# Rita-zi/WavTokenizer

Measured on AMD Instinct MI355X. Metric: audio-seconds/sec encode+decode, 24 kHz 3 s clips, higher is better.
Workload: dtype f32 (split-f16 x3 products)

## Files before the change

### include/wavtokenizer_amd.h

```cpp
#ifndef WAVTOKENIZER_AMD_H
#define WAVTOKENIZER_AMD_H

#include <stddef.h>
#include <stdint.h>

#ifdef __cplusplus
extern "C" {
#endif

typedef enum {
    WT_OK = 0,
    WT_ERR_INVALID = -1,
    WT_ERR_MISSING_TENSOR = -2,
    WT_ERR_SHAPE = -3,
    WT_ERR_HIP = -4,
    WT_ERR_NOT_INITED = -5,
    WT_ERR_RANGE = -6,
    WT_ERR_LSTM_SYNC = -7,
    WT_ERR_INDEX = -8
} wt_status;

enum wt_status_bits {
    WT_STATUS_BIT_LSTM = 1,
    WT_STATUS_BIT_RANGE = 2
};

typedef struct {
    int32_t n_ratios;
    int32_t ratios[8];
    int32_t vq_bins;
    int32_t num_quantizers;
    int32_t input_channels;
    int32_t dim;
    int32_t intermediate_dim;
    int32_t num_layers;
    int32_t adanorm_num_embeddings;
    int32_t n_fft;
    int32_t hop_length;
    int32_t padding_same;
} wt_arch;

typedef struct {
    const char*  name;
    const float* data;
    int64_t      numel;
} wt_tensor;

typedef struct wt_model wt_model;
typedef struct wt_plan  wt_plan;

typedef enum {
    WT_PLAN_ENCODE = 0,
    WT_PLAN_DECODE = 1,
    WT_PLAN_SEANET_DECODER = 2,
    WT_PLAN_HEAD = 3,
    WT_PLAN_UNIT_LSTM = 4
} wt_plan_kind;

enum {
    WT_PLAN_FLAG_KEEP_STAGES = 1,
    WT_PLAN_FLAG_UNFUSED = 16,
    WT_PLAN_FLAG_STEP_LSTM = 4,
    WT_PLAN_FLAG_GRAPH = 8,
    WT_PLAN_FLAG_FP32_GEMM = 2,
    WT_PLAN_FLAG_RANGE_REPORT = 32,
    WT_PLAN_FLAG_MIXED_LENGTH = 64
};

enum wt_range_site {
    WT_SITE_ENCODER = 0,
    WT_SITE_BB_EMBED = 1,
    WT_SITE_RES0 = 2, WT_SITE_RES1 = 3,
    WT_SITE_ATTN = 4,
    WT_SITE_RES2 = 5, WT_SITE_RES3 = 6,
    WT_SITE_CNX0 = 7,
    WT_SITE_HEAD = 40,
    WT_SITE_SEANET_DECODER = 41
};

const char* wt_last_error(void);
const char* wt_version(void);

int  wt_model_create(const wt_arch* arch, const wt_tensor* tensors, int32_t n_tensors, int32_t device,
                     wt_model** out);
void wt_model_destroy(wt_model* m);

size_t wt_model_export_bytes(const wt_model* m);
int  wt_model_export(const wt_model* m, void* buf, size_t n);
int  wt_packed_info(const void* buf, size_t n, wt_arch* arch, int32_t* version, uint64_t* arch_hash);
int  wt_packed_verify(const void* buf, size_t n);
size_t wt_packed_bytes(const void* buf, size_t n);
int  wt_model_create_packed(const void* buf, size_t n, int32_t device, wt_model** out);
int  wt_model_hop(const wt_model* m);
int  wt_model_persistent_lstm(const wt_model* m);
int  wt_device_info(int32_t device, int32_t* compute_units, int32_t* is_gfx950, int32_t* persistent_lstm);
int64_t wt_model_weight_bytes(const wt_model* m);

int    wt_plan_create(const wt_model* m, int32_t kind, int32_t B, int64_t len, int32_t flags, wt_plan** out);
int    wt_plan_create_ex(const wt_model* m, int32_t kind, int32_t B, int64_t len, int32_t flags, uint64_t fp32_sites,
                         wt_plan** out);
void   wt_plan_destroy(wt_plan* p);
size_t wt_plan_workspace_bytes(const wt_plan* p);
int64_t wt_plan_frames(const wt_plan* p);
int    wt_plan_num_launches(const wt_plan* p);
int64_t wt_plan_graph_replays(const wt_plan* p);
int    wt_plan_find_buffer(const wt_plan* p, const char* name, size_t* offset, size_t* numel);
int    wt_plan_buffer_info(const wt_plan* p, const char* name, size_t* offset, size_t* numel, int32_t* format);
int    wt_plan_status(const wt_plan* p, int32_t* bits, int32_t clear);
int    wt_plan_range_sites(const wt_plan* p, uint64_t* sites, int32_t clear);
int    wt_plan_range_report(const wt_plan* p, int32_t index, const char** step, const char** buffer, float* amax);
int    wt_model_status(const wt_model* m, int32_t* bits, int32_t clear);
int    wt_model_split_ok(const wt_model* m);
int    wt_plan_buffer_name(const wt_plan* p, int32_t index, const char** name);

int wt_plan_num_steps(const wt_plan* p);
int wt_plan_step_name(const wt_plan* p, int32_t index, const char** name);
int wt_plan_set_timing(const wt_plan* p, const char* name_substr);
int wt_plan_read_timing(const wt_plan* p, double* total_ms, int64_t* launches, int32_t reset);

int wt_encode(const wt_plan* p, const float* wav, float* features, int64_t* codes, float* emb_out,
              void* workspace, void* stream);

int wt_encode_mixed(const wt_plan* p, const float* wav, const int32_t* lengths, float* features, int64_t* codes, float* emb_out,
                    void* workspace, void* stream);
int64_t wt_plan_min_clip_length(const wt_plan* p);
int wt_sconv_geometry(int64_t T, int32_t k, int32_t stride, int32_t dilation, int32_t out[4]);

int wt_codes_to_features(const wt_model* m, const int64_t* codes, int32_t K, int32_t B, int64_t L,
                         float* features, void* stream);

int wt_decode(const wt_plan* p, const float* features, int32_t bandwidth_id, float* wav_out,
              float* backbone_out, void* workspace, void* stream);

int wt_head(const wt_plan* p, const float* x, float* wav_out, void* workspace, void* stream);

int wt_seanet_decode(const wt_plan* p, const float* features, float* wav_out, void* workspace, void* stream);


int wt_sconv1d(const float* x, const float* w, const float* bias, float* y, int32_t B, int64_t T,
               int32_t Cin, int32_t Cout, int32_t k, int32_t stride, int32_t dilation, int32_t elu_input,
               void* stream);

int wt_linear(const float* x, const float* w, const float* bias, float* y, int64_t M, int32_t N, int32_t K,
              int32_t f16x3, void* workspace, void* stream);

int wt_conv1d_s32(const float* x, const float* w, const float* bias, float* y, int32_t B, int64_t T, int32_t Cin,
                  int32_t Cout, int32_t k, int32_t stride, int32_t zero_same, void* workspace, void* stream);

size_t wt_vq_workspace_bytes(int64_t N, int32_t D, int32_t bins);
int wt_vq_nearest(const float* x, const float* embed, int64_t N, int32_t D, int32_t bins, int64_t* codes_out,
                  void* workspace, void* stream);
int wt_vq_nearest_f32(const float* x, const float* embed, int64_t N, int32_t D, int32_t bins, int64_t* codes_out,
                      void* workspace, void* stream);

typedef struct {
    int32_t size;
    int32_t engine, epi, out, pro, b_is_act;
    int32_t M, N, K;
    int32_t T_in, T_out, Cin, taps, stride, dil, pad_left, pad_mode, Tp;
    int32_t K1, nz, tap_pair, head_kb;
    float alpha;
    int64_t a_bstride, a_rstride, a2_bstride, a2_rstride, w_rstride, c_rstride, r_rstride, zA, zW, zC;
    const float* A;
    const float* A2;
    const float* B;
    const float* bias;
    const float* R;
    const float* gamma;
    float* C;
    float* C2;
    uint32_t* status;
} wt_gemm_desc;
typedef struct {
    int32_t BM, BN, waves_m, waves_n, stages, ks, prod, staged, bias_cache, G, tiles;
} wt_launch_form;
size_t wt_gemm_probe_workspace_bytes(const wt_gemm_desc* d);
int wt_gemm_probe(const wt_gemm_desc* d, wt_launch_form* form, void* workspace, void* stream);

enum { WT_OP_GN_APPLY = 0, WT_OP_GN_STATS = 1, WT_OP_ROWNORM = 2, WT_OP_SOFTMAX = 3, WT_OP_ISTFT_OLA = 4, WT_OP_CONV_FIRST = 5,
       WT_OP_CONV_LAST = 6, WT_OP_TRANSPOSE = 7, WT_OP_CONVTR = 8, WT_OP_ROW_SUMSQ = 9, WT_OP_S32_AMAX = 10 };
enum { WT_OPK_GN_TILE = 1, WT_OPK_GN_CHUNK = 2, WT_OPK_GN_STATS = 3, WT_OPK_ROWNORM = 4, WT_OPK_DWCONV_LN = 5,
       WT_OPK_SOFTMAX_REG = 6, WT_OPK_SOFTMAX_RMW = 7, WT_OPK_ISTFT_OLA = 8, WT_OPK_CONV_FIRST = 9, WT_OPK_CONV_LAST32 = 10,
       WT_OPK_CONV_LAST = 11, WT_OPK_TRANSPOSE = 12, WT_OPK_CONVTR = 13, WT_OPK_ROW_SUMSQ = 14, WT_OPK_S32_AMAX = 15 };
typedef struct {
    int32_t size;
    int32_t op;
    int32_t B, L, C;
    int32_t groups, mode, flag, out_s32;
    int32_t ld, k, stride, Cout, n_fft, hop, Kq;
    float eps;
    int64_t n;
    const void* x;
    const void *p0, *p1, *p2, *p3, *p4, *p5;
    void *y, *y2, *y3;
    uint32_t* status;
} wt_op_desc;
typedef struct {
    int32_t kernel;
    int32_t variant;
    int32_t variant2;
    int32_t grid_x, grid_y, grid_z, block, lds;
} wt_op_form;
int wt_op_probe(const wt_op_desc* d, wt_op_form* form, void* stream);

int wt_resblock(const float* x, const float* wav, const float* e0_w, const float* e0_b, const float* w3, const float* b3,
                const float* w1, const float* b1, const float* ws, const float* bs, float* y, int32_t B, int64_t T,
                int32_t C, int32_t elu_out, int32_t out_s32, int32_t fp32_chain, void* stream);
int wt_resblock_down(const float* wav, const float* e0_w, const float* e0_b, const float* w3, const float* b3, const float* w1,
                     const float* b1, const float* ws, const float* bs, const float* wd, const float* bd, float* y_down,
                     int32_t B, int64_t T, int32_t r, void* stream);

int wt_unit_run(const wt_plan* p, const float* x, float* y, void* workspace, void* stream);

int wt_model_take_bad_codes(const wt_model* m);


typedef struct wt_resampler wt_resampler;
int     wt_resampler_create(int32_t orig_sr, int32_t new_sr, int32_t device, wt_resampler** out);
void    wt_resampler_destroy(wt_resampler* r);
int64_t wt_resampler_out_length(const wt_resampler* r, int64_t T);
int     wt_convert_audio(const wt_resampler* r, const float* wav, int32_t B, int32_t C, int64_t T, float* out, void* stream);

int wt_pcm16(const float* x, int64_t n, float limit, int32_t rescale, int16_t* out, void* workspace, void* stream);

int wt_linear_overlap_add(const float* frames, const float* weight, int32_t n_frames, int64_t rows, int64_t frame_len,
                          int64_t last_len, int64_t stride, float* out, void* stream);

#ifdef __cplusplus
}
#endif
#endif
```

### wavtokenizer_amd/_capi.py

```python
from __future__ import annotations

import ctypes
import os
from ctypes import POINTER, c_char_p, c_float, c_int32, c_int64, c_size_t, c_void_p

_HERE = os.path.dirname(os.path.abspath(__file__))
LIB_PATH = os.environ.get("WAVTOK_HIP_LIB") or os.path.join(_HERE, "libwavtok_hip.so")

EXPORTS = [
    "wt_last_error", "wt_version", "wt_model_create", "wt_model_destroy", "wt_model_export_bytes", "wt_model_export", "wt_packed_info", "wt_packed_verify", "wt_packed_bytes",
    "wt_model_create_packed", "wt_model_hop", "wt_model_weight_bytes",
    "wt_plan_create", "wt_plan_create_ex", "wt_plan_range_sites", "wt_plan_range_report", "wt_model_persistent_lstm", "wt_device_info", "wt_plan_destroy", "wt_plan_workspace_bytes", "wt_plan_frames", "wt_plan_num_launches", "wt_plan_graph_replays",
    "wt_plan_find_buffer", "wt_plan_buffer_info", "wt_plan_buffer_name", "wt_plan_status", "wt_plan_num_steps", "wt_plan_step_name",
    "wt_plan_set_timing", "wt_plan_read_timing", "wt_model_split_ok", "wt_model_status", "wt_model_take_bad_codes", "wt_encode", "wt_codes_to_features",
    "wt_decode", "wt_seanet_decode", "wt_head", "wt_unit_run", "wt_sconv1d", "wt_linear", "wt_conv1d_s32", "wt_vq_workspace_bytes",
    "wt_vq_nearest", "wt_vq_nearest_f32", "wt_resblock", "wt_resblock_down", "wt_gemm_probe_workspace_bytes", "wt_gemm_probe", "wt_op_probe",
    "wt_resampler_create", "wt_resampler_destroy", "wt_resampler_out_length", "wt_convert_audio", "wt_pcm16",
    "wt_linear_overlap_add", "wt_encode_mixed", "wt_plan_min_clip_length", "wt_sconv_geometry",
]

WT_PLAN_ENCODE, WT_PLAN_DECODE, WT_PLAN_SEANET_DECODER, WT_PLAN_HEAD, WT_PLAN_UNIT_LSTM = 0, 1, 2, 3, 4
WT_PLAN_FLAG_KEEP_STAGES = 1
WT_PLAN_FLAG_FP32_GEMM = 2
WT_PLAN_FLAG_STEP_LSTM = 4
WT_PLAN_FLAG_GRAPH = 8
WT_PLAN_FLAG_UNFUSED = 16
WT_PLAN_FLAG_RANGE_REPORT = 32
WT_PLAN_FLAG_MIXED_LENGTH = 64
WT_SITE_ENCODER, WT_SITE_BB_EMBED, WT_SITE_RES0, WT_SITE_RES1, WT_SITE_ATTN, WT_SITE_RES2, WT_SITE_RES3 = 0, 1, 2, 3, 4, 5, 6
WT_SITE_CNX0, WT_SITE_HEAD, WT_SITE_SEANET_DECODER = 7, 40, 41
WT_ERR_INVALID = -1
WT_ERR_RANGE, WT_ERR_LSTM_SYNC, WT_ERR_INDEX = -6, -7, -8
WT_STATUS_BIT_LSTM, WT_STATUS_BIT_RANGE = 1, 2
BUF_S32, BUF_ELU = 1, 2


class WtArch(ctypes.Structure):
    _fields_ = [("n_ratios", c_int32), ("ratios", c_int32 * 8), ("vq_bins", c_int32), ("num_quantizers", c_int32),
                ("input_channels", c_int32), ("dim", c_int32), ("intermediate_dim", c_int32),
                ("num_layers", c_int32), ("adanorm_num_embeddings", c_int32), ("n_fft", c_int32),
                ("hop_length", c_int32), ("padding_same", c_int32)]


class WtTensor(ctypes.Structure):
    _fields_ = [("name", c_char_p), ("data", POINTER(c_float)), ("numel", c_int64)]


class WtGemmDesc(ctypes.Structure):
    _fields_ = ([("size", c_int32), ("engine", c_int32), ("epi", c_int32), ("out", c_int32), ("pro", c_int32), ("b_is_act", c_int32),
                 ("M", c_int32), ("N", c_int32), ("K", c_int32)]
                + [(n, c_int32) for n in ("T_in", "T_out", "Cin", "taps", "stride", "dil", "pad_left", "pad_mode", "Tp",
                                         "K1", "nz", "tap_pair", "head_kb")]
                + [("alpha", c_float)]
                + [(n, c_int64) for n in ("a_bstride", "a_rstride", "a2_bstride", "a2_rstride", "w_rstride", "c_rstride",
                                         "r_rstride", "zA", "zW", "zC")]
                + [(n, c_void_p) for n in ("A", "A2", "B", "bias", "R", "gamma", "C", "C2", "status")])


class WtLaunchForm(ctypes.Structure):
    _fields_ = [(n, c_int32) for n in ("BM", "BN", "waves_m", "waves_n", "stages", "ks", "prod", "staged", "bias_cache", "G", "tiles")]


WT_OP_GN_APPLY, WT_OP_GN_STATS, WT_OP_ROWNORM, WT_OP_SOFTMAX, WT_OP_ISTFT_OLA, WT_OP_CONV_FIRST = 0, 1, 2, 3, 4, 5
WT_OP_CONV_LAST, WT_OP_TRANSPOSE, WT_OP_CONVTR, WT_OP_ROW_SUMSQ, WT_OP_S32_AMAX = 6, 7, 8, 9, 10
WT_OPK_NAMES = {1: "gn_tile", 2: "gn_chunk", 3: "gn_stats", 4: "rownorm", 5: "dwconv_ln", 6: "softmax_reg", 7: "softmax_rmw",
                8: "istft_ola", 9: "conv_first", 10: "conv_last32", 11: "conv_last", 12: "transpose", 13: "convtr",
                14: "row_sumsq", 15: "s32_amax"}


class WtOpDesc(ctypes.Structure):
    _fields_ = ([(n, c_int32) for n in ("size", "op", "B", "L", "C", "groups", "mode", "flag", "out_s32", "ld", "k", "stride",
                                        "Cout", "n_fft", "hop", "Kq")]
                + [("eps", c_float), ("n", c_int64)]
                + [(n, c_void_p) for n in ("x", "p0", "p1", "p2", "p3", "p4", "p5", "y", "y2", "y3", "status")])


class WtOpForm(ctypes.Structure):
    _fields_ = [(n, c_int32) for n in ("kernel", "variant", "variant2", "grid_x", "grid_y", "grid_z", "block", "lds")]


class WavTokError(RuntimeError):
    def __init__(self, msg, status=0):
        super().__init__(msg)
        self.status = status


def _load() -> ctypes.CDLL:
    if not os.path.exists(LIB_PATH):
        raise ImportError(
            f"{LIB_PATH} not found: build the HIP extension first (python -c 'import __graft_entry__ as g; g.build()' "
            "or make -C wavtokenizer_amd/csrc). There is no CPU fallback for the product path.")
    lib = ctypes.CDLL(LIB_PATH)
    if os.environ.get("WAVTOK_HIP_LIB"):
        class _Missing:
            def __init__(self, name):
                self.name, self.argtypes, self.restype = name, None, None

            def __call__(self, *a):
                raise WavTokError(f"{LIB_PATH} has no {self.name}")
        for sym in EXPORTS:
            try:
                getattr(lib, sym)
            except AttributeError:
                setattr(lib, sym, _Missing(sym))
    lib.wt_last_error.restype = c_char_p
    lib.wt_version.restype = c_char_p
    lib.wt_model_create.argtypes = [POINTER(WtArch), POINTER(WtTensor), c_int32, c_int32, POINTER(c_void_p)]
    lib.wt_model_destroy.argtypes = [c_void_p]
    lib.wt_model_destroy.restype = None
    lib.wt_model_export_bytes.argtypes = [c_void_p]
    lib.wt_model_export_bytes.restype = c_size_t
    lib.wt_model_export.argtypes = [c_void_p, c_void_p, c_size_t]
    lib.wt_packed_info.argtypes = [c_void_p, c_size_t, POINTER(WtArch), POINTER(c_int32), POINTER(ctypes.c_uint64)]
    lib.wt_packed_verify.argtypes = [c_void_p, c_size_t]
    lib.wt_packed_bytes.argtypes = [c_void_p, c_size_t]
    lib.wt_packed_bytes.restype = c_size_t
    lib.wt_model_create_packed.argtypes = [c_void_p, c_size_t, c_int32, POINTER(c_void_p)]
    lib.wt_model_hop.argtypes = [c_void_p]
    lib.wt_model_weight_bytes.argtypes = [c_void_p]
    lib.wt_model_weight_bytes.restype = c_int64
    lib.wt_plan_create.argtypes = [c_void_p, c_int32, c_int32, c_int64, c_int32, POINTER(c_void_p)]
    lib.wt_plan_create_ex.argtypes = [c_void_p, c_int32, c_int32, c_int64, c_int32, ctypes.c_uint64, POINTER(c_void_p)]
    lib.wt_plan_range_sites.argtypes = [c_void_p, POINTER(ctypes.c_uint64), c_int32]
    lib.wt_plan_range_report.argtypes = [c_void_p, c_int32, POINTER(c_char_p), POINTER(c_char_p), POINTER(c_float)]
    lib.wt_model_persistent_lstm.argtypes = [c_void_p]
    lib.wt_device_info.argtypes = [c_int32, POINTER(c_int32), POINTER(c_int32), POINTER(c_int32)]
    lib.wt_plan_destroy.argtypes = [c_void_p]
    lib.wt_plan_destroy.restype = None
    lib.wt_plan_workspace_bytes.argtypes = [c_void_p]
    lib.wt_plan_workspace_bytes.restype = c_size_t
    lib.wt_plan_frames.argtypes = [c_void_p]
    lib.wt_plan_frames.restype = c_int64
    lib.wt_plan_num_launches.argtypes = [c_void_p]
    lib.wt_plan_graph_replays.argtypes = [c_void_p]
    lib.wt_plan_graph_replays.restype = c_int64
    lib.wt_plan_find_buffer.argtypes = [c_void_p, c_char_p, POINTER(c_size_t), POINTER(c_size_t)]
    lib.wt_plan_buffer_info.argtypes = [c_void_p, c_char_p, POINTER(c_size_t), POINTER(c_size_t), POINTER(c_int32)]
    lib.wt_plan_status.argtypes = [c_void_p, POINTER(c_int32), c_int32]
    lib.wt_model_split_ok.argtypes = [c_void_p]
    lib.wt_model_status.argtypes = [c_void_p, POINTER(c_int32), c_int32]
    lib.wt_model_take_bad_codes.argtypes = [c_void_p]
    lib.wt_unit_run.argtypes = [c_void_p, c_void_p, c_void_p, c_void_p, c_void_p]
    lib.wt_plan_buffer_name.argtypes = [c_void_p, c_int32, POINTER(c_char_p)]
    lib.wt_plan_num_steps.argtypes = [c_void_p]
    lib.wt_plan_step_name.argtypes = [c_void_p, c_int32, POINTER(c_char_p)]
    lib.wt_plan_set_timing.argtypes = [c_void_p, c_char_p]
    lib.wt_plan_read_timing.argtypes = [c_void_p, POINTER(ctypes.c_double), POINTER(c_int64), c_int32]
    lib.wt_encode.argtypes = [c_void_p, c_void_p, c_void_p, c_void_p, c_void_p, c_void_p, c_void_p]
    lib.wt_encode_mixed.argtypes = [c_void_p, c_void_p, c_void_p, c_void_p, c_void_p, c_void_p, c_void_p, c_void_p]
    lib.wt_plan_min_clip_length.argtypes = [c_void_p]
    lib.wt_plan_min_clip_length.restype = c_int64
    lib.wt_sconv_geometry.argtypes = [c_int64, c_int32, c_int32, c_int32, POINTER(c_int32)]
    lib.wt_codes_to_features.argtypes = [c_void_p, c_void_p, c_int32, c_int32, c_int64, c_void_p, c_void_p]
    lib.wt_decode.argtypes = [c_void_p, c_void_p, c_int32, c_void_p, c_void_p, c_void_p, c_void_p]
    lib.wt_seanet_decode.argtypes = [c_void_p, c_void_p, c_void_p, c_void_p, c_void_p]
    lib.wt_head.argtypes = [c_void_p, c_void_p, c_void_p, c_void_p, c_void_p]
    lib.wt_sconv1d.argtypes = [c_void_p, c_void_p, c_void_p, c_void_p, c_int32, c_int64, c_int32, c_int32, c_int32,
                               c_int32, c_int32, c_int32, c_void_p]
    lib.wt_linear.argtypes = [c_void_p, c_void_p, c_void_p, c_void_p, c_int64, c_int32, c_int32, c_int32, c_void_p, c_void_p]
    lib.wt_conv1d_s32.argtypes = [c_void_p, c_void_p, c_void_p, c_void_p, c_int32, c_int64, c_int32, c_int32, c_int32,
                                  c_int32, c_int32, c_void_p, c_void_p]
    lib.wt_vq_workspace_bytes.argtypes = [c_int64, c_int32, c_int32]
    lib.wt_vq_workspace_bytes.restype = c_size_t
    lib.wt_vq_nearest.argtypes = [c_void_p, c_void_p, c_int64, c_int32, c_int32, c_void_p, c_void_p, c_void_p]
    lib.wt_vq_nearest_f32.argtypes = [c_void_p, c_void_p, c_int64, c_int32, c_int32, c_void_p, c_void_p, c_void_p]
    lib.wt_resblock.argtypes = [c_void_p] * 11 + [c_int32, c_int64, c_int32, c_int32, c_int32, c_int32, c_void_p]
    lib.wt_resblock_down.argtypes = [c_void_p] * 12 + [c_int32, c_int64, c_int32, c_void_p]
    lib.wt_gemm_probe_workspace_bytes.argtypes = [POINTER(WtGemmDesc)]
    lib.wt_gemm_probe_workspace_bytes.restype = c_size_t
    lib.wt_gemm_probe.argtypes = [POINTER(WtGemmDesc), POINTER(WtLaunchForm), c_void_p, c_void_p]
    lib.wt_op_probe.argtypes = [POINTER(WtOpDesc), POINTER(WtOpForm), c_void_p]
    lib.wt_resampler_create.argtypes = [c_int32, c_int32, c_int32, POINTER(c_void_p)]
    lib.wt_resampler_destroy.argtypes = [c_void_p]
    lib.wt_resampler_destroy.restype = None
    lib.wt_resampler_out_length.argtypes = [c_void_p, c_int64]
    lib.wt_resampler_out_length.restype = c_int64
    lib.wt_convert_audio.argtypes = [c_void_p, c_void_p, c_int32, c_int32, c_int64, c_void_p, c_void_p]
    lib.wt_pcm16.argtypes = [c_void_p, c_int64, ctypes.c_float, c_int32, c_void_p, c_void_p, c_void_p]
    lib.wt_linear_overlap_add.argtypes = [c_void_p, c_void_p, c_int32, c_int64, c_int64, c_int64, c_int64, c_void_p, c_void_p]
    return lib


lib = _load()


def check(rc: int, what: str = "") -> None:
    if rc != 0:
        msg = lib.wt_last_error()
        raise WavTokError(f"{what} failed (status {rc}): {msg.decode() if msg else ''}", rc)
```

### wavtokenizer_amd/csrc/common.h

```cpp
#pragma once
#include <hip/hip_runtime.h>
#include <stdint.h>
#include <stdio.h>
#include <stdlib.h>
#include <mutex>
#include <string>

namespace wt {

void set_error(const std::string& msg);

#define WT_HIP_CHECK(expr)                                                                      \
    do {                                                                                        \
        hipError_t _e = (expr);                                                                 \
        if (_e != hipSuccess) {                                                                 \
            ::wt::set_error(std::string(#expr) + ": " + hipGetErrorString(_e));                 \
            return -4;                                                                          \
        }                                                                                       \
    } while (0)

struct PerDeviceOnce {
    std::mutex mu;
    bool seen[64] = {};
    template <class F> int run(F&& f) {
        int d = 0;
        (void)hipGetDevice(&d);
        d &= 63;
        std::lock_guard<std::mutex> g(mu);
        if (seen[d]) return 0;
        if (int rc = f()) return rc;
        seen[d] = true;
        return 0;
    }
};

enum : unsigned { WT_STATUS_LSTM = 1u, WT_STATUS_RANGE = 2u };
enum OpKernel : int {
    OPK_NONE = 0, OPK_GN_TILE, OPK_GN_CHUNK, OPK_GN_STATS, OPK_ROWNORM, OPK_DWCONV_LN, OPK_SOFTMAX_REG, OPK_SOFTMAX_RMW,
    OPK_ISTFT_OLA, OPK_CONV_FIRST, OPK_CONV_LAST32, OPK_CONV_LAST, OPK_TRANSPOSE, OPK_CONVTR, OPK_ROW_SUMSQ, OPK_S32_AMAX
};
struct OpForm {
    int kernel = OPK_NONE;
    int variant = 0;
    int variant2 = 0;
    unsigned grid[3] = {0, 0, 0};
    unsigned block = 0;
    unsigned lds = 0;
};
struct LaunchCtx {
    unsigned* status = nullptr;
    OpForm* form = nullptr;
    unsigned long long* stamp_start = nullptr;
    unsigned long long* stamp_end = nullptr;
    bool stamp_used = false;
};
extern thread_local LaunchCtx g_launch;

int device_cus();

#ifdef WT_LAB
inline const char* lab_env(const char* name) { return getenv(name); }
#else
inline const char* lab_env(const char*) { return nullptr; }
#endif

#if defined(__HIPCC__)
#ifdef WT_NO_RANGE_TRACK
__device__ __forceinline__ float amax1(float m, float) { return m; }
__device__ __forceinline__ float amax4(float m, float, float, float, float) { return m; }
#else
__device__ __forceinline__ float amax1(float m, float v) { return fmaxf(m, fabsf(v)); }
__device__ __forceinline__ float amax4(float m, float a, float b, float c, float d) {
    m = fmaxf(fmaxf(m, fabsf(a)), fabsf(b));
    return fmaxf(fmaxf(m, fabsf(c)), fabsf(d));
}
#endif
__device__ __forceinline__ void split2_f16(float a, float b, unsigned& hi_pk, unsigned& lo_pk) {
    typedef float f32x2_t __attribute__((ext_vector_type(2)));
    typedef _Float16 f16x2_t __attribute__((ext_vector_type(2)));
    const f32x2_t ab = {a, b};
    hi_pk = __builtin_bit_cast(unsigned, __builtin_convertvector(ab, f16x2_t));
    const f32x2_t s = ab * 2048.f;
    const float m = -2048.f;
    asm("v_fma_mixlo_f16 %0, %1, %2, %3 op_sel_hi:[1,0,0]" : "=v"(lo_pk) : "v"(hi_pk), "s"(m), "v"(s[0]));
    asm("v_fma_mixhi_f16 %0, %1, %2, %3 op_sel:[1,0,0] op_sel_hi:[1,0,0]" : "+v"(lo_pk) : "v"(hi_pk), "s"(m), "v"(s[1]));
}
typedef _Float16 wt_f16x4 __attribute__((ext_vector_type(4)));
__device__ __forceinline__ void split4_f16(float a, float b, float c, float d, wt_f16x4& hi, wt_f16x4& lo) {
    typedef unsigned u32x2_t __attribute__((ext_vector_type(2)));
    unsigned h0, l0, h1, l1;
    split2_f16(a, b, h0, l0);
    split2_f16(c, d, h1, l1);
    hi = __builtin_bit_cast(wt_f16x4, (u32x2_t){h0, h1});
    lo = __builtin_bit_cast(wt_f16x4, (u32x2_t){l0, l1});
}
__device__ __forceinline__ float elu_med3(float x) { return __builtin_amdgcn_fmed3f(x, __expf(x) - 1.f, 0.f); }
typedef float wt_f32x4 __attribute__((ext_vector_type(4)));
__device__ __forceinline__ wt_f32x4 elu_med3_x4(wt_f32x4 x) {
    const wt_f32x4 t = x * 1.44269504088896340736f;
    wt_f32x4 e;
#pragma unroll
    for (int i = 0; i < 4; ++i) e[i] = __builtin_amdgcn_exp2f(t[i]);
    e = e - 1.f;
#pragma unroll
    for (int i = 0; i < 4; ++i) e[i] = __builtin_amdgcn_fmed3f(x[i], e[i], 0.f);
    return e;
}
__device__ __forceinline__ void range_report(unsigned* status, float amax) {
    if (status && amax >= 65504.f) __hip_atomic_fetch_or(status, (unsigned)WT_STATUS_RANGE, __ATOMIC_RELAXED, __HIP_MEMORY_SCOPE_AGENT);
}
#endif

struct SConvGeom { int pl, pr_total, Tout, Tp; };
__host__ __device__ inline SConvGeom sconv_geom(long T, int k, int stride, int dil) {
    const int keff = (k - 1) * dil + 1;
    const int pt = keff - stride;
    const long nfr_num = T - keff + pt;
    const long nfr = (nfr_num + stride - 1) / stride + 1;
    const long ideal = (nfr - 1) * stride + (keff - pt);
    const int extra = (int)(ideal - T);
    SConvGeom g;
    const int pr = pt / 2;
    g.pl = pt - pr;
    g.pr_total = pr + extra;
    g.Tout = (int)((T + pt + extra - keff) / stride + 1);
    const int maxpad = g.pl > g.pr_total ? g.pl : g.pr_total;
    g.Tp = T > maxpad ? (int)T : maxpad + 1;
    return g;
}

enum : int {
    GEOM_WORDS = 64, GEOM_VALID = 0, GEOM_T = 1, GEOM_TREAD = 2, GEOM_STAGE0 = 3, GEOM_STAGE_WORDS = 9,
    GEOM_C3 = 0, GEOM_SC = 3, GEOM_DOWN = 6, GEOM_MAX_STAGES = 6
};
inline int geom_final(int n_stages) { return GEOM_STAGE0 + n_stages * GEOM_STAGE_WORDS; }
inline int geom_L(int n_stages) { return geom_final(n_stages) + 3; }

enum Pro : int { PRO_NONE = 0, PRO_ELU = 1 };
enum Epi : int {
    EPI_BIAS = 0,
    EPI_BIAS_RES = 1,
    EPI_BIAS_GELU = 2,
    EPI_BIAS_GAMMA_RES = 3,
    EPI_HEAD = 4,
    EPI_ARGMAX = 6,
    EPI_SCALE = 7,
    EPI_BIAS_ROW = 8,
    EPI_BIAS_RES_ELU = 9,
    EPI_BIAS_ELU = 10
};
enum Out16s : int {
    OUT_F32 = 0,
    OUT_S32 = 1,
    OUT_S32_DUAL_ELU = 2,
    OUT_F32_AND_S32 = 3
};
enum PadMode : int { PAD_ZERO = 0, PAD_REFLECT = 1 };

struct LaunchForm {
    int BM = 0, BN = 0, waves_m = 0, waves_n = 0, stages = 0;
    int ks = 1, prod = 0;
    int staged = 0, bias_cache = 0;
    int G = 0, tiles = 0;
};

struct GemmArgs {
    const float* A = nullptr;
    long a_bstride = 0;
    long a_rstride = 0;
    int T_in = 0, T_out = 0;
    int Cin = 0, taps = 1, stride = 1, dil = 1, pad_left = 0, pad_mode = PAD_ZERO;
    int Tp = 0;
    const float* A2 = nullptr;
    long a2_bstride = 0, a2_rstride = 0;
    int K1 = 0;
    const float* W = nullptr;
    long w_rstride = 0;
    const void* W_hi = nullptr;
    const float* bias = nullptr;
    int M = 0, N = 0, K = 0;
    float* C = nullptr;
    long c_rstride = 0;
    float* C2 = nullptr;
    const float* R = nullptr;
    long r_rstride = 0;
    const float* gamma = nullptr;
    float alpha = 1.f;
    int nz = 1;
    long zA = 0, zW = 0, zC = 0;
    int head_kb = 0;
    const float* vq_xx = nullptr;
    const float* vq_ee = nullptr;
    float* vq_pval = nullptr;
    int*   vq_pidx = nullptr;
    int vq_nparts = 0;
    int group_m = 8;
    int group_n = 0;
    int tap_pair = 0;
    unsigned long long* stamp_start = nullptr;
    unsigned long long* stamp_end = nullptr;
    int stage_epi = 0;
    int stage_off = 0;
    int pc_off = 0;
    float acc_scale = 1.f;
    const float* acc_scale_dev = nullptr;
    unsigned* status = nullptr;
    unsigned long long* dbg_stamps = nullptr;
    LaunchForm* form = nullptr;
};

int gemm_vq_parts(int N);
int check_gemm(const GemmArgs& a, int pro, int epi);
int check_gemm16s(const GemmArgs& a, int epi, int out, const int* mix_geom = nullptr);
int launch_gemm(const GemmArgs& a, int pro, int epi, hipStream_t s);
int launch_gemm16s(const GemmArgs& a, int epi, int out, hipStream_t s, const int* mix_geom = nullptr);
int gemm16s_vq_parts(int N);
int launch_split_s32(const float* x, void* out, long n, hipStream_t s, const float* scale_dev = nullptr);
int launch_unsplit_s32(const void* s32, float* out, long n, float inv_scale, hipStream_t s);
int launch_pow2_scales(const float* a, long na, const float* b, long nb, unsigned* bits2, float* out3, hipStream_t s);

int launch_conv_first(const float* wav, const float* w , const float* bias, float* y, int B, long T,
                      int k, int Cout, hipStream_t s);
int launch_conv_last(const float* x , const float* w , const float* bias, float* y ,
                     int B, long T, int Cin, int k, int elu_in, hipStream_t s);
int launch_transpose(const float* in, float* out, int B, int R, int C, hipStream_t s, int out_s32 = 0);
size_t gn_part_floats(int B, int L, int groups);
int launch_gn_stats(const float* x, const float* gamma, const float* beta, float* scale, float* shift, int B, int L,
                    int C, int groups, float eps, hipStream_t s, float* part = nullptr);
int launch_gn_apply(const float* x, const float* gamma, const float* beta, float* scale, float* shift, float* y,
                    int swish, int B, int L, int C, int groups, float eps, hipStream_t s, int out_s32 = 0, float* part = nullptr);
enum RowNormMode : int { RN_DWCONV = 0, RN_PLAIN = 1, RN_AFFINE_IN = 2 };
int launch_rownorm(int mode, const float* x, float* y, int B, int L, int C, const float* dw_w ,
                   const float* dw_b, const float* in_scale, const float* in_shift, const float* out_scale,
                   const float* out_shift, float eps, hipStream_t s, int out_s32 = 0);
int launch_istft_ola(const float* parts, const float* win, const float* wsq, float* out, int B, int L, int n_fft, int hop,
                     int Kq, int center, hipStream_t s);
int launch_softmax(float* S, int rows, int L, int ld, hipStream_t s, float* P_s32 = nullptr);
int launch_row_sumsq(const float* x, float* out, long rows, int D, hipStream_t s);
int launch_vq_finalize(const float* pval, const int* pidx, int nparts, const float* embed, int64_t* codes,
                       float* feat_ncl, int B, int L, int D, int bins, hipStream_t s);
int launch_codes_to_features(const int64_t* codes, const float* embed, int K, int bins, int B, long L, int D,
                             float* feat_ncl, hipStream_t s, unsigned* bad = nullptr);
int launch_fill_u32(void* p, unsigned value, size_t n_bytes, hipStream_t s);
int launch_plan_guard(const unsigned* status, int nwords, int site0, unsigned* host_status, unsigned* model_status, int64_t* codes,
                      long n_codes, float* f0, long n0, float* f1, long n1, float* f2, long n2, hipStream_t s);
int launch_s32_amax(const void* s32, long numel, unsigned* out_bits, hipStream_t s);
struct LstmArgs {
    const float* xg0;
    const float* W0;
    const float* W1;
    const float* b1;
    float* h0;
    float* h1;
    float* c0;
    float* c1;
    const float* x;
    float* y;
    int B, L, H;
    int elu_out;
    int out_s32;
    int f16x3;
    unsigned* status = nullptr;
};
int launch_lstm_step(const LstmArgs& a, int s, hipStream_t stream);
struct LstmPersistArgs {
    const float* xg0;
    const void* Wp;
    const float* b1;
    const float* x;
    float* y;
    void* hx;
    unsigned* ctl;
    unsigned* status = nullptr;
    int dbg_spin_shift = 0;
    int B, L, H, Bx;
    int elu_out, out_s32;
    int data_flag;
};
size_t lstm_persist_hx_bytes();
size_t lstm_persist_ctl_bytes();
int launch_lstm_persist(const LstmPersistArgs& a, hipStream_t stream);
struct ResblockArgs {
    const float* x;
    const float* wav;
    const float* e0_w;
    const float* e0_b;
    const float* W3;
    const float* b3;
    const float* W1;
    const float* b1;
    const float* Ws;
    const float* bs;
    float* y;
    int B, T, C;
    long x_bstride;
    int elu_out;
    int out_s32;
    int dbg;
    unsigned* status;
    const float* Wd;
    const float* bd;
    float* y_down;
    int R;
};
struct ResblockMix {
    const int* T = nullptr;
    const int* Tread = nullptr;
};
bool resblock_fusable(int C);
int launch_resblock(const ResblockArgs& a, hipStream_t s);
int launch_resblock16(const ResblockArgs& a, hipStream_t s, const ResblockMix* mix = nullptr);
bool resblock16_down_fusable(int C, long T, int r, int k);
int launch_resblock16_down(const ResblockArgs& a, hipStream_t s, const ResblockMix* mix = nullptr);
int launch_mixed_geometry(const int* lengths, int* geom, int B, long Tpad, int tmin, int n_st, const int* kd, const int* rd,
                          int kf, hipStream_t s);
int launch_mixed_pad(const int* geom, int l_word, int64_t* codes, float* feat_ncl, float* emb_ncl, int B, int L, int D,
                     hipStream_t s);
int launch_convtr(const float* x, const float* w , const float* bias, float* y, int B, int Tin,
                  int Cin, int Cout, int k, int stride, int elu_in, hipStream_t s);

}
```

### wavtokenizer_amd/csrc/model.h

```cpp
#pragma once
#include "../../include/wavtokenizer_amd.h"
#include "common.h"

#include <algorithm>
#include <atomic>
#include <climits>
#include <cmath>
#include <cstring>
#include <functional>
#include <map>
#include <memory>
#include <mutex>
#include <string>
#include <vector>

namespace wt {

struct S32Copy {
    const void* p = nullptr;
    float acc_scale = 1.f;
    bool tap_pair = false;
};
struct ConvW {
    float* w = nullptr;
    float* b = nullptr;
    int cout = 0, cin = 0, k = 0;
    S32Copy s32;
};
struct GemmW {
    float* w = nullptr;
    int rows = 0, cols = 0;
    S32Copy s32;
};
struct LstmW {
    GemmW Wih0;
    float* b0 = nullptr;
    float* W0 = nullptr;
    float* W1 = nullptr;
    float* b1 = nullptr;
    float* W0h = nullptr;
    float* W1h = nullptr;
    float* Wp = nullptr;
};
struct ResStage {
    ConvW c3, c1, sc, down;
    ConvW cat;
    int C = 0, r = 0;
};
struct PosRes {
    float *n1w, *n1b, *n2w, *n2b;
    ConvW c1, c2;
};
struct CnxBlock {
    float *dw_w, *dw_b, *ada_s, *ada_h, *b1, *b2, *gamma;
    GemmW W1, W2;
};
struct SeaDecStage {
    float* tr_w = nullptr;
    GemmW tr_wp;
    float* tr_b = nullptr;
    int cin = 0, cout = 0, k = 0, r = 0;
    ConvW c3, c1, sc;
    ConvW cat;
};

}

struct wt_model {
    wt_arch arch{};
    int device = 0;
    int hop = 1;
    int H = 512;
    std::vector<int> enc_ratios;
    std::vector<void*> allocs;
    std::vector<size_t> alloc_bytes;
    int64_t weight_bytes = 0;
    float *e0_w = nullptr, *e0_b = nullptr;
    int e0_k = 7, e0_c = 32;
    std::vector<wt::ResStage> stages;
    wt::LstmW enc_lstm;
    wt::ConvW enc_final;
    wt::GemmW embed;
    float* ee = nullptr;
    wt::ConvW bb_embed;
    wt::PosRes res[4];
    float *at_nw, *at_nb, *at_bqk, *at_bv, *at_bp;
    wt::GemmW at_Wqk, at_Wv, at_Wp;
    float *gn5w, *gn5b, *ada_s, *ada_h;
    std::vector<wt::CnxBlock> cnx;
    float *fln_w, *fln_b;
    wt::GemmW head_W, istft_W;
    float *head_b = nullptr, *wsq = nullptr, *win = nullptr;
    int Kb = 0, Kq = 0, bins_f = 0, R = 0;
    bool has_seadec = false;
    wt::ConvW sd_first;
    wt::LstmW sd_lstm;
    std::vector<wt::SeaDecStage> sd_stages;
    float *sd_last_w = nullptr, *sd_last_b = nullptr;
    bool s32_ok = true;
    bool sd_s32_ok = true;
    float w_amax = 0.f;
    struct LazyF32 { const float* w; const void* s32; int64_t n; float scale; };
    std::vector<LazyF32> lazy_f32;
    mutable std::atomic<bool> f32_stale{false};
    mutable std::mutex f32_mu;
    unsigned* bad_codes_host = nullptr;
    unsigned* bad_codes_dev = nullptr;
    unsigned* status_host = nullptr;
    unsigned* status_dev = nullptr;
    mutable std::atomic<bool> persist_ok{true};
};

namespace wt {

struct TensorMap {
    std::map<std::string, std::pair<const float*, int64_t>> m;
    std::string missing;
    const float* get(const std::string& k, int64_t numel) {
        auto it = m.find(k);
        if (it == m.end()) { if (missing.empty()) missing = k; return nullptr; }
        if (it->second.second != numel) {
            if (missing.empty()) missing = k + " (numel " + std::to_string(it->second.second) + ", expected " + std::to_string(numel) + ")";
            return nullptr;
        }
        return it->second.first;
    }
    bool has(const std::string& k) const { return m.count(k) != 0; }
};

struct RunCtx {
    char* ws;
    hipStream_t stream;
    const float* in_f;
    float* out_f;
    int64_t* codes;
    float* aux;
    int bw_id;
    const int* lengths = nullptr;
};
enum Site : int {
    SITE_ENC = 0,
    SITE_BB_EMBED = 1,
    SITE_RES0 = 2, SITE_RES1 = 3, SITE_ATTN = 4, SITE_RES2 = 5, SITE_RES3 = 6,
    SITE_CNX0 = 7,
    SITE_HEAD = 40,
    SITE_SEADEC = 41,
    SITE_COUNT = 64
};
constexpr int CTL_SITE0 = 16;
constexpr int CTL_WORDS = CTL_SITE0 + SITE_COUNT + 48;

enum BufFmt : int { BUF_F32 = 0, BUF_S32 = 1, BUF_ELU = 2 };
struct BufSpec {
    std::string name;
    size_t bytes = 0, numel = 0, off = 0;
    int first = INT_MAX, last = -1;
    int fmt = BUF_F32;
    bool holds_s32 = false;
};

struct DeviceGuard {
    int prev = -1;
    bool ok = true;
    explicit DeviceGuard(int dev) {
        if (hipGetDevice(&prev) != hipSuccess) prev = -1;
        if (prev != dev) ok = hipSetDevice(dev) == hipSuccess; else prev = -1;
    }
    ~DeviceGuard() { if (prev >= 0) (void)hipSetDevice(prev); }
};

}

struct wt_plan {
    const wt_model* model = nullptr;
    int kind = 0, B = 0, flags = 0;
    int64_t len = 0, L = 0, T = 0;
    uint64_t fp32_sites = 0;
    int whole_site = -1;
    int cur_site = 0;
    long n_codes = 0, n_out = 0, n_aux = 0;
    int build_rc = 0;
    std::vector<wt::BufSpec> bufs;
    std::vector<std::function<int(const wt::RunCtx&)>> steps;
    std::vector<std::string> step_names;
    std::vector<int> step_sites;
    struct RangeEntry { int step, buf; };
    std::vector<RangeEntry> range_entries;
    unsigned* range_dev = nullptr;
    mutable std::vector<float> range_host;
    mutable bool range_fresh = false;
    size_t ws_bytes = 0;
    int n_launches = 0;
    mutable std::string timing_filter;
    mutable std::vector<std::pair<hipEvent_t, hipEvent_t>> ev_pending, ev_free;
    static constexpr int STAMP_SLOTS = 8192;
    mutable unsigned long long* stamps = nullptr;
    mutable int stamp_next = 0;
    mutable double timing_ms = 0.0;
    mutable long timing_n = 0;
    unsigned* status_host = nullptr;
    unsigned* status_dev = nullptr;
    int ctl = -1;
    bool uses_persist = false;
    int mix_geom = -1;
    int64_t min_clip = 0;
    mutable bool graph_persist = false;
    mutable std::mutex mu;
    struct GraphKey {
        const void *ws = nullptr, *in = nullptr, *out = nullptr, *codes = nullptr, *aux = nullptr, *lengths = nullptr;
        int bw = -1;
        bool operator==(const GraphKey& o) const {
            return ws == o.ws && in == o.in && out == o.out && codes == o.codes && aux == o.aux && lengths == o.lengths && bw == o.bw;
        }
    };
    mutable GraphKey graph_key, last_key;
    mutable bool graph_failed = false;
    mutable hipGraphExec_t graph_exec = nullptr;
    mutable hipStream_t cap_stream = nullptr;
    mutable long graph_replays = 0;

    wt_plan() = default;
    wt_plan(const wt_plan&) = delete;
    ~wt_plan() {
        if (status_host) (void)hipHostFree(status_host);
        if (range_dev) (void)hipFree(range_dev);
        if (stamps) (void)hipFree(stamps);
        if (graph_exec) (void)hipGraphExecDestroy(graph_exec);
        if (cap_stream) (void)hipStreamDestroy(cap_stream);
        for (auto& ev : ev_pending) { (void)hipEventDestroy(ev.first); (void)hipEventDestroy(ev.second); }
        for (auto& ev : ev_free) { (void)hipEventDestroy(ev.first); (void)hipEventDestroy(ev.second); }
    }

    int buf(const std::string& name, size_t numel, int fmt = wt::BUF_F32) {
        wt::BufSpec b;
        b.name = name; b.numel = numel; b.bytes = (numel * sizeof(float) + 255) / 256 * 256; b.fmt = fmt;
        bufs.push_back(b);
        return (int)bufs.size() - 1;
    }
    void step(std::initializer_list<int> used, std::function<int(const wt::RunCtx&)> fn, int launches = 1,
              const std::string& name = "") {
        const int s = (int)steps.size();
        std::string nm = name;
        for (int id : used) {
            if (id < 0) continue;
            bufs[id].first = std::min(bufs[id].first, s);
            bufs[id].last = std::max(bufs[id].last, s);
            if (name.empty()) nm = bufs[id].name;
        }
        if (flags & WT_PLAN_FLAG_RANGE_REPORT)
            for (int id : used)
                if (id >= 0 && (bufs[id].fmt & wt::BUF_S32)) range_entries.push_back({s, id});
        steps.push_back(std::move(fn));
        step_names.push_back(nm);
        step_sites.push_back(cur_site);
        n_launches += launches;
    }
    float* ptr(const wt::RunCtx& c, int id) const { return reinterpret_cast<float*>(c.ws + bufs[id].off); }
    void layout() {
        const bool keep = flags & WT_PLAN_FLAG_KEEP_STAGES;
        std::vector<int> order(bufs.size());
        for (size_t i = 0; i < order.size(); ++i) order[i] = (int)i;
        std::stable_sort(order.begin(), order.end(), [&](int x, int y) { return bufs[x].first < bufs[y].first; });
        std::vector<int> placed;
        ws_bytes = 0;
        for (int id : order) {
            wt::BufSpec& b = bufs[id];
            if (b.last < 0) { b.off = 0; continue; }
            if (keep) b.last = INT_MAX;
            size_t off = 0;
            bool moved = true;
            while (moved) {
                moved = false;
                for (int pid : placed) {
                    const wt::BufSpec& q = bufs[pid];
                    const bool live = !(q.last < b.first || b.last < q.first);
                    const bool overlap = off < q.off + q.bytes && q.off < off + b.bytes;
                    if (live && overlap) { off = q.off + q.bytes; moved = true; }
                }
            }
            b.off = off;
            placed.push_back(id);
            ws_bytes = std::max(ws_bytes, off + b.bytes);
        }
        ws_bytes = std::max<size_t>(ws_bytes, 256);
    }
};

namespace wt {

int build_model(wt_model* M, TensorMap& tm);
int build_splits(wt_model* M);
float s32_weight_scale(float amax);
size_t model_export_bytes(const wt_model* M);
int model_export(const wt_model* M, void* buf, size_t n);
int model_import(wt_model* M, const void* buf, size_t n);
int packed_info(const void* buf, size_t n, wt_arch* arch, int32_t* version, uint64_t* arch_hash);
int ensure_f32_weights(const wt_model* M);
size_t packed_bytes(const void* buf, size_t n);
int packed_verify(const void* buf, size_t n);
bool full_chip(int device);
GemmArgs sconv_args(const ConvW& w, int B, long T, int stride, int dil);
GemmArgs zconv_args(const ConvW& w, int B, int L);
GemmArgs linear_args(const float* W, const float* bias, long M, int N, int K);
GemmArgs linear_args(const GemmW& W, const float* bias, long M, int N, int K);
int build_encode(wt_plan* P);
int build_decode(wt_plan* P);
int build_head(wt_plan* P);
int build_seanet_decoder(wt_plan* P);
int build_unit_lstm(wt_plan* P);
void plan_begin(wt_plan* P);
void plan_end(wt_plan* P);
inline long wave_samples(const wt_model* M, long L) {
    return M->arch.padding_same ? L * (long)M->arch.hop_length : (L - 1) * (long)M->arch.hop_length;
}

}
```

### wavtokenizer_amd/csrc/plan.cpp

```cpp
#include "model.h"

namespace wt {

static bool site_fp32(const wt_plan* P, int site) { return (P->fp32_sites >> site) & 1u; }
static bool plan_fp32(const wt_plan* P) {
    if ((P->flags & WT_PLAN_FLAG_FP32_GEMM) || !P->model->s32_ok) return true;
    if (P->whole_site == SITE_SEADEC && !P->model->sd_s32_ok) return true;
    return P->whole_site >= 0 && site_fp32(P, P->whole_site);
}
static bool plan_unfused(const wt_plan* P) { return P->flags & WT_PLAN_FLAG_UNFUSED; }
static bool plan_s32(const wt_plan* P) { return !plan_unfused(P) && !plan_fp32(P); }

static int gemm_auto(const wt_plan* P, const GemmArgs& a, int pro, int epi, hipStream_t s) {
    if (P->model->f32_stale.load()) if (int rc = ensure_f32_weights(P->model)) return rc;
    return launch_gemm(a, pro, epi, s);
}

static void set_s32(GemmArgs& a, const S32Copy& c) {
    a.W_hi = c.p; a.acc_scale = c.acc_scale; a.tap_pair = c.tap_pair ? 1 : 0;
}

static int gemm_s32(const GemmArgs& a, int epi, int out, hipStream_t s, const int* mix = nullptr) {
    if (!a.W_hi) { set_error("internal: no S32 copy of this weight"); return WT_ERR_INVALID; }
    return launch_gemm16s(a, epi, out, s, mix);
}

static int dense(const wt_plan* P, bool s32, const GemmArgs& a, int pro, int epi, int out, hipStream_t s, const int* mix = nullptr) {
    if (mix && !s32) { set_error("internal: a mixed-length conv off the S32 route"); return WT_ERR_INVALID; }
    return s32 ? gemm_s32(a, epi, out, s, mix) : gemm_auto(P, a, pro, epi, s);
}

static int dense_act(const wt_plan* P, bool s32, GemmArgs a, const float* b_op, int epi, int out, hipStream_t s) {
    if (s32) { a.W_hi = b_op; return launch_gemm16s(a, epi, out, s); }
    a.W = b_op;
    return gemm_auto(P, a, PRO_NONE, epi, s);
}

struct GemmBufs {
    int A, A2, C, C2 = -1;
    bool r_is_c = false;
    long x_off = 0;
    int mix_word = -1;
};
static void gemm_step(wt_plan* P, bool s32, const GemmArgs& proto, const GemmBufs& b, int pro, int epi, int out,
                      const std::string& name = "") {
    auto is_s32 = [&](int id) { return (P->bufs[id].fmt & BUF_S32) != 0 || P->bufs[id].holds_s32; };
    const int eff = s32 ? out : OUT_F32;
    const bool c_s32 = eff == OUT_S32 || eff == OUT_S32_DUAL_ELU, dual = eff == OUT_S32_DUAL_ELU || eff == OUT_F32_AND_S32;
    const char* why = nullptr;
    if (dual && b.C2 < 0) why = "a dual output without a second buffer";
    else if (s32 && (!is_s32(b.A) || (b.A2 >= 0 && !is_s32(b.A2)))) why = "an S32 GEMM reads a buffer declared fp32";
    else if ((is_s32(b.C) != c_s32 || (dual && !is_s32(b.C2)))) why = "the output format disagrees with the buffer's declaration";
    if (why && !P->build_rc) {
        set_error("internal: GEMM step into '" + P->bufs[b.C].name + "': " + why);
        P->build_rc = WT_ERR_INVALID;
    }
    const int geom = b.mix_word >= 0 ? P->mix_geom : -1;
    P->step({geom, b.A, b.A2, b.C, b.C2}, [=](const RunCtx& c) {
        GemmArgs a = proto;
        a.A = P->ptr(c, b.A) + b.x_off; a.C = P->ptr(c, b.C);
        if (b.A2 >= 0) a.A2 = P->ptr(c, b.A2);
        if (b.C2 >= 0) a.C2 = P->ptr(c, b.C2);
        if (b.r_is_c) a.R = a.C;
        return dense(P, s32, a, pro, epi, out, c.stream, geom >= 0 ? reinterpret_cast<const int*>(P->ptr(c, geom)) + b.mix_word : nullptr);
    }, 1, name);
}

static GemmBufs in_place(int A, int C) { GemmBufs b{A, -1, C}; b.r_is_c = true; return b; }

static int copy_f32(float* dst, const float* src, size_t numel, hipStream_t s) {
    WT_HIP_CHECK(hipMemcpyAsync(dst, src, numel * sizeof(float), hipMemcpyDeviceToDevice, s));
    return 0;
}
constexpr int CALLER = -1;
static void copy_step(wt_plan* P, int src, int dst, size_t numel, const std::string& name = "") {
    P->step({src, dst}, [=](const RunCtx& c) {
        return copy_f32(dst == CALLER ? c.out_f : P->ptr(c, dst), src == CALLER ? c.in_f : P->ptr(c, src), numel, c.stream);
    }, 1, name);
}


GemmArgs sconv_args(const ConvW& w, int B, long T, int stride, int dil) {
    const SConvGeom g = sconv_geom(T, w.k, stride, dil);
    GemmArgs a;
    a.a_bstride = T * w.cin; a.a_rstride = w.cin;
    a.T_in = (int)T; a.T_out = g.Tout; a.Cin = w.cin; a.taps = w.k; a.stride = stride; a.dil = dil;
    a.pad_left = g.pl; a.pad_mode = PAD_REFLECT; a.Tp = g.Tp;
    a.W = w.w; a.w_rstride = (long)w.k * w.cin; a.bias = w.b;
    a.M = B * g.Tout; a.N = w.cout; a.K = w.k * w.cin;
    a.c_rstride = w.cout;
    set_s32(a, w.s32);
    return a;
}
GemmArgs zconv_args(const ConvW& w, int B, int L) {
    GemmArgs a;
    a.a_bstride = (long)L * w.cin; a.a_rstride = w.cin;
    a.T_in = L; a.T_out = L; a.Cin = w.cin; a.taps = w.k; a.pad_left = (w.k - 1) / 2; a.pad_mode = PAD_ZERO;
    a.W = w.w; a.w_rstride = (long)w.k * w.cin; a.bias = w.b;
    a.M = B * L; a.N = w.cout; a.K = w.k * w.cin; a.c_rstride = w.cout;
    set_s32(a, w.s32);
    return a;
}
GemmArgs linear_args(const float* W, const float* bias, long M, int N, int K) {
    GemmArgs a;
    a.a_bstride = 0; a.a_rstride = K; a.T_in = (int)M; a.T_out = (int)M; a.Cin = K; a.taps = 1;
    a.W = W; a.w_rstride = K; a.bias = bias; a.M = (int)M; a.N = N; a.K = K; a.c_rstride = N;
    return a;
}
GemmArgs linear_args(const GemmW& W, const float* bias, long M, int N, int K) {
    GemmArgs a = linear_args(W.w, bias, M, N, K); set_s32(a, W.s32); return a;
}

static int plan_resblock(wt_plan* P, const ConvW& c3, const ConvW& c1, const ConvW& sc, int B, long T, int xin,
                         const std::string& name, bool elu_out = false, const wt_model* e0 = nullptr, long x_off = 0,
                         long x_bstride = 0, bool out_s32 = false, int mix_word = -1) {
    const int C = sc.cout;
    if (resblock_fusable(C) && !plan_unfused(P)) {
        const int y = P->buf(name, (size_t)B * T * C, (out_s32 && !plan_fp32(P) ? BUF_S32 : BUF_F32) | (elu_out ? BUF_ELU : 0));
        const int geom = mix_word >= 0 ? P->mix_geom : -1;
        P->step({e0 ? -1 : xin, y, geom}, [=](const RunCtx& c) {
            ResblockArgs a{};
            ResblockMix mix;
            if (geom >= 0) mix.T = mix.Tread = reinterpret_cast<const int*>(P->ptr(c, geom)) + mix_word;
            a.x = e0 ? nullptr : P->ptr(c, xin) + x_off;
            a.x_bstride = x_bstride;
            a.wav = e0 ? c.in_f : nullptr;
            a.e0_w = e0 ? e0->e0_w : nullptr; a.e0_b = e0 ? e0->e0_b : nullptr;
            a.W3 = c3.w; a.b3 = c3.b; a.W1 = c1.w; a.b1 = c1.b; a.Ws = sc.w; a.bs = sc.b;
            a.y = P->ptr(c, y); a.B = B; a.T = (int)T; a.C = C; a.elu_out = elu_out ? 1 : 0;
            if (plan_fp32(P)) return launch_resblock(a, c.stream);
            a.out_s32 = out_s32 ? 1 : 0;
            return launch_resblock16(a, c.stream, geom >= 0 ? &mix : nullptr);
        }, 1, "resblock.fused");
        return y;
    }
    const int h = P->buf(name + ".h", (size_t)B * T * (C / 2));
    const int y = P->buf(name, (size_t)B * T * C, elu_out ? BUF_ELU : BUF_F32);
    GemmArgs a3 = sconv_args(c3, B, T, 1, 1), as = sconv_args(sc, B, T, 1, 1), a1 = sconv_args(c1, B, T, 1, 1);
    if (x_bstride) a3.a_bstride = as.a_bstride = x_bstride;
    a1.r_rstride = C;
    GemmBufs bx{xin, -1, h};
    bx.x_off = x_off;
    gemm_step(P, false, a3, bx, PRO_ELU, EPI_BIAS, OUT_F32);
    bx.C = y;
    gemm_step(P, false, as, bx, PRO_NONE, EPI_BIAS, OUT_F32);
    gemm_step(P, false, a1, in_place(h, y), PRO_ELU, elu_out ? EPI_BIAS_RES_ELU : EPI_BIAS_RES, OUT_F32);
    return y;
}

static int plan_lstm(wt_plan* P, const LstmW& w, int B, int L, int H, int xin, const std::string& name,
                     bool elu_out = false, int xin_s32 = -1, bool y_s32 = false) {
    const int xg = P->buf(name + ".xg", (size_t)B * L * 4 * H);
    const int Bp = (B + 63) / 64 * 64;
    const size_t st_numel = (size_t)4 * H * Bp + (size_t)2 * B * H;
    const int st = P->buf(name + ".state", st_numel);
    const int y = P->buf(name, (size_t)B * L * H, (y_s32 ? BUF_S32 : BUF_F32) | (elu_out ? BUF_ELU : 0));
    GemmArgs ax = linear_args(w.Wih0, w.b0, (long)B * L, 4 * H, H);
    ax.T_in = B; ax.T_out = B; ax.a_bstride = H; ax.a_rstride = (long)L * H;
    const int xsrc = xin_s32 >= 0 ? xin_s32 : xin;
    gemm_step(P, xin_s32 >= 0, ax, {xsrc, -1, xg}, PRO_NONE, EPI_BIAS, OUT_F32);
    const bool persist_env = [] { const char* e = lab_env("WT_LSTM_PERSIST"); return !e || e[0] != '0'; }();
    const bool persist = persist_env && !plan_fp32(P) && !(P->flags & WT_PLAN_FLAG_STEP_LSTM) && w.Wp && H == 512 && B <= 128 && L < 65536 &&
                         full_chip(P->model->device);
    if (persist) P->uses_persist = true;
    const size_t hxn = lstm_persist_hx_bytes() / sizeof(float), ctn = lstm_persist_ctl_bytes() / sizeof(float);
    const int hx = persist ? P->buf(name + ".hx", hxn + ctn) : -1;
    P->step({xin, xg, st, hx, y}, [=](const RunCtx& c) {
        if (persist && P->model->persist_ok.load()) {
            float* hb = P->ptr(c, hx);
            if (int rc = launch_fill_u32(hb, 0xFFFFFFFFu, (hxn + ctn) * sizeof(float), c.stream)) return rc;
            LstmPersistArgs pa;
            const int df_trace = [] { const char* e = lab_env("WT_LSTM_TRACE"); return e ? atoi(e) : 0; }();
            pa.data_flag = 1 | (df_trace ? 4 : 0);
            pa.xg0 = P->ptr(c, xg); pa.Wp = w.Wp; pa.b1 = w.b1; pa.x = P->ptr(c, xin); pa.y = P->ptr(c, y);
            pa.hx = hb; pa.ctl = reinterpret_cast<unsigned*>(hb + hxn);
            pa.B = B; pa.L = L; pa.H = H; pa.Bx = (B + 7) / 8; pa.elu_out = elu_out ? 1 : 0; pa.out_s32 = y_s32 ? 1 : 0;
            return launch_lstm_persist(pa, c.stream);
        }
        float* s = P->ptr(c, st);
        if (int rc = launch_fill_u32(s, 0u, (st_numel * sizeof(float) + 15) / 16 * 16, c.stream)) return rc;
        LstmArgs la;
        la.f16x3 = plan_fp32(P) ? 0 : 1;
        la.xg0 = P->ptr(c, xg); la.W0 = la.f16x3 ? w.W0h : w.W0; la.W1 = la.f16x3 ? w.W1h : w.W1; la.b1 = w.b1;
        la.h0 = s; la.h1 = s + (size_t)2 * H * Bp; la.c0 = s + (size_t)4 * H * Bp; la.c1 = la.c0 + (size_t)B * H;
        la.x = P->ptr(c, xin); la.y = P->ptr(c, y); la.B = B; la.L = L; la.H = H; la.elu_out = elu_out ? 1 : 0;
        la.out_s32 = y_s32 ? 1 : 0;
        for (int t = 0; t <= L; ++t)
            if (int rc = launch_lstm_step(la, t, c.stream)) return rc;
        return 0;
    }, L + 2);
    return y;
}

static int plan_resblock_s32(wt_plan* P, const ConvW& c3, const ConvW& sc, const ConvW& cat, int B, long T, int x_raw,
                             int x_elu, const std::string& name, long x_off = 0, long x_bstride = 0, int mix_word = -1) {
    if (!cat.s32.p) { set_error("internal: unfused S32 resblock without an S32 shortcut + conv1 weight"); return -1; }
    const int C = sc.cout;
    const int h = P->buf(name + ".h", (size_t)B * T * (C / 2), BUF_S32 | BUF_ELU);
    GemmArgs a3 = sconv_args(c3, B, T, 1, 1);
    GemmBufs b3{x_elu, -1, h};
    b3.x_off = x_off; b3.mix_word = mix_word >= 0 ? mix_word + GEOM_C3 : -1;
    if (x_bstride) a3.a_bstride = x_bstride;
    gemm_step(P, true, a3, b3, PRO_NONE, EPI_BIAS_ELU, OUT_S32);
    const int o = P->buf(name, (size_t)B * T * C, BUF_S32 | BUF_ELU);
    GemmArgs ac = sconv_args(sc, B, T, 1, 1);
    ac.W = cat.w; ac.w_rstride = cat.cin; ac.bias = cat.b; ac.K = cat.cin; ac.Cin = cat.cin;
    set_s32(ac, cat.s32);
    ac.K1 = C; ac.a2_bstride = T * (C / 2); ac.a2_rstride = C / 2;
    if (x_bstride) ac.a_bstride = x_bstride;
    GemmBufs bc{x_raw, h, o};
    bc.x_off = x_off; bc.mix_word = mix_word >= 0 ? mix_word + GEOM_SC : -1;
    gemm_step(P, true, ac, bc, PRO_NONE, EPI_BIAS_ELU, OUT_S32);
    return o;
}

int build_encode(wt_plan* P) {
    const wt_model* M = P->model;
    const int B = P->B;
    const long T = P->T;
    const bool fold_e0 = !plan_unfused(P) && !M->stages.empty() && M->stages[0].C == 32 &&
                         M->e0_k == 7 && resblock_fusable(32);
    int x = -1;
    if (!fold_e0) {
        x = P->buf("enc.0", (size_t)B * T * M->e0_c);
        const int x0 = x;
        P->step({x0}, [=](const RunCtx& c) {
            return launch_conv_first(c.in_f, M->e0_w, M->e0_b, P->ptr(c, x0), B, T, M->e0_k, M->e0_c, c.stream);
        });
    }
    const bool fuse_elu = !plan_unfused(P);
    const bool s32 = plan_s32(P);
    struct Route { bool fused, down, s32; };
    std::vector<Route> route(M->stages.size());
    for (size_t si = 0; si < route.size(); ++si) {
        const ResStage& st = M->stages[si];
        Route& r = route[si];
        r.fused = resblock_fusable(st.C) && !plan_unfused(P);
        r.s32 = s32 && st.C % 32 == 0 && st.down.s32.p &&
                (r.fused || (si > 0 && route[si - 1].s32 && st.c3.s32.p && st.c1.s32.p && st.sc.s32.p));
        r.down = si == 0 && fold_e0 && r.fused && r.s32 && route.size() > 1 && resblock_fusable(M->stages[1].C) &&
                 st.down.cin == 32 && st.down.cout == 64 && resblock16_down_fusable(st.C, T, st.r, st.down.k);
    }
    const bool lstm_s32 = !route.empty() && route.back().s32 && M->enc_lstm.Wih0.s32.p;
    const bool tail_s32 = lstm_s32 && M->enc_final.s32.p && M->embed.s32.p;
    const bool mixed = P->flags & WT_PLAN_FLAG_MIXED_LENGTH;
    const int n_st = (int)route.size();
    int geom = -1;
    if (mixed) {
        bool ok = s32 && !(P->flags & (WT_PLAN_FLAG_KEEP_STAGES | WT_PLAN_FLAG_RANGE_REPORT)) && tail_s32 &&
                  n_st >= 2 && n_st <= GEOM_MAX_STAGES && route[0].down;
        for (int si = 1; si < n_st && ok; ++si)
            ok = route[si].s32 && (route[si].fused ? M->stages[si].C == 64 : M->stages[si].cat.s32.p != nullptr);
        for (const ResStage& st : M->stages) ok = ok && st.c3.k == 3 && st.sc.k == 1;
        if (!ok) {
            set_error("mixed-length plans run only the shipped split-f16 encoder route: not with WT_PLAN_FLAG_UNFUSED, "
                      "FP32_GEMM, KEEP_STAGES or RANGE_REPORT, an encoder range site on fp32, or weights without S32 copies");
            return WT_ERR_INVALID;
        }
        P->min_clip = 1024;
        if (T < P->min_clip) { set_error("mixed-length plans need a padded length of at least 1024 samples"); return WT_ERR_INVALID; }
        geom = P->mix_geom = P->buf("mix.geom", (size_t)B * GEOM_WORDS);
        std::vector<int> kd, rd;
        for (const ResStage& st : M->stages) { kd.push_back(st.down.k); rd.push_back(st.r); }
        const int kf = M->enc_final.k;
        const int tmin = (int)P->min_clip;
        P->step({geom}, [=](const RunCtx& c) {
            return launch_mixed_geometry(c.lengths, reinterpret_cast<int*>(P->ptr(c, geom)), B, T, tmin, n_st, kd.data(),
                                         rd.data(), kf, c.stream);
        }, 1, "mix.geom");
    }
    auto mix_ptr = [=](const RunCtx& c, int word) { return reinterpret_cast<const int*>(P->ptr(c, geom)) + word; };
    long Tc = T;
    int idx = 1;
    int x_elu = -1;
    int x_s32 = -1;
    for (size_t si = 0; si < route.size(); ++si) {
        const ResStage& st = M->stages[si];
        const Route r = route[si];
        const bool last = si + 1 == route.size();
        GemmArgs ad = sconv_args(st.down, B, Tc, st.r, 1);
        const size_t ynum = (size_t)B * ad.T_out * st.down.cout;
        const std::string out = "enc." + std::to_string(idx + 2);
        if (r.down) {
            const int y = P->buf(out, ynum);
            P->step({-1, y, geom}, [=](const RunCtx& c) {
                ResblockArgs a{};
                ResblockMix mix;
                if (geom >= 0) { mix.T = mix_ptr(c, GEOM_T); mix.Tread = mix_ptr(c, GEOM_TREAD); }
                a.wav = c.in_f; a.e0_w = M->e0_w; a.e0_b = M->e0_b;
                a.W3 = st.c3.w; a.b3 = st.c3.b; a.W1 = st.c1.w; a.b1 = st.c1.b; a.Ws = st.sc.w; a.bs = st.sc.b;
                a.Wd = st.down.w; a.bd = st.down.b; a.y_down = P->ptr(c, y); a.R = st.r;
                a.B = B; a.T = (int)Tc; a.C = st.C;
                return launch_resblock16_down(a, c.stream, geom >= 0 ? &mix : nullptr);
            }, 1, "resblock.fused_down");
            x = y; Tc = ad.T_out; idx += 3;
            continue;
        }
        const std::string name = "enc." + std::to_string(idx);
        const int stage_word = GEOM_STAGE0 + (int)si * GEOM_STAGE_WORDS;
        if (r.fused)
            x = plan_resblock(P, st.c3, st.c1, st.sc, B, Tc, x, name, fuse_elu, (si == 0 && fold_e0) ? M : nullptr, 0, 0, r.s32,
                              mixed ? stage_word + GEOM_C3 : -1);
        else if (r.s32)
            x = plan_resblock_s32(P, st.c3, st.sc, st.cat, B, Tc, x, x_elu, name, 0, 0, mixed ? stage_word : -1);
        else
            x = plan_resblock(P, st.c3, st.c1, st.sc, B, Tc, x, name, fuse_elu);
        if (x < 0) return WT_ERR_INVALID;
        const bool next_s32 = !last && !route[si + 1].fused && route[si + 1].s32;
        const int y = P->buf(out, ynum, next_s32 ? BUF_S32 : BUF_F32);
        const int y2 = (next_s32 || (last && lstm_s32)) ? P->buf(out + ".s32", ynum, BUF_S32 | (next_s32 ? BUF_ELU : 0)) : -1;
        GemmBufs bd{x, -1, y, y2};
        bd.mix_word = mixed ? stage_word + GEOM_DOWN : -1;
        gemm_step(P, r.s32, ad, bd, fuse_elu ? PRO_NONE : PRO_ELU, EPI_BIAS,
                  next_s32 ? OUT_S32_DUAL_ELU : (y2 >= 0 ? OUT_F32_AND_S32 : OUT_F32));
        if (next_s32) x_elu = y2;
        if (last) x_s32 = y2;
        x = y; Tc = ad.T_out; idx += 3;
    }
    const int L = (int)Tc;
    if (L != P->L) { set_error("internal: frame count mismatch"); return WT_ERR_INVALID; }
    P->n_codes = (long)B * L; P->n_out = P->n_aux = (long)B * 512 * L;
    const int H = M->H;
    x = plan_lstm(P, M->enc_lstm, B, L, H, x, "enc." + std::to_string(idx), fuse_elu, x_s32, tail_s32);
    GemmArgs af = sconv_args(M->enc_final, B, L, 1, 1);
    const int emb = P->buf("enc." + std::to_string(idx + 2), (size_t)B * L * 512);
    const int emb_s32 = tail_s32 ? P->buf("enc." + std::to_string(idx + 2) + ".s32", (size_t)B * L * 512, BUF_S32) : -1;
    GemmBufs bf{x, -1, emb, emb_s32};
    bf.mix_word = mixed ? geom_final(n_st) : -1;
    gemm_step(P, tail_s32, af, bf, fuse_elu ? PRO_NONE : PRO_ELU, EPI_BIAS, OUT_F32_AND_S32);
    const int bins = M->arch.vq_bins;
    GemmArgs av = linear_args(M->embed, nullptr, (long)B * L, bins, 512);
    const int np = tail_s32 ? gemm16s_vq_parts(bins) : gemm_vq_parts(bins);
    const int xx = P->buf("vq.xx", (size_t)B * L);
    const int pv = P->buf("vq.pval", (size_t)B * L * np);
    const int pi = P->buf("vq.pidx", (size_t)B * L * np);
    P->step({emb, xx}, [=](const RunCtx& c) { return launch_row_sumsq(P->ptr(c, emb), P->ptr(c, xx), (long)B * L, 512, c.stream); });
    P->step({emb, emb_s32, xx, pv, pi}, [=](const RunCtx& c) {
        GemmArgs a = av; a.A = P->ptr(c, tail_s32 ? emb_s32 : emb);
        a.vq_xx = P->ptr(c, xx); a.vq_ee = M->ee; a.vq_pval = P->ptr(c, pv);
        a.vq_pidx = reinterpret_cast<int*>(P->ptr(c, pi)); a.vq_nparts = np;
        return dense(P, tail_s32, a, PRO_NONE, EPI_ARGMAX, OUT_F32, c.stream);
    }, 1, "vq.argmin");
    P->step({geom, pv, pi, emb}, [=](const RunCtx& c) {
        if (int rc = launch_vq_finalize(P->ptr(c, pv), reinterpret_cast<int*>(P->ptr(c, pi)), np, M->embed.w, c.codes,
                                        c.out_f, B, L, 512, bins, c.stream)) return rc;
        if (c.aux) if (int rc = launch_transpose(P->ptr(c, emb), c.aux, B, L, 512, c.stream)) return rc;
        if (geom >= 0) return launch_mixed_pad(mix_ptr(c, 0), geom_L(n_st), c.codes, c.out_f, c.aux, B, L, 512, c.stream);
        return 0;
    }, mixed ? 3 : 2);
    return 0;
}

static void plan_head(wt_plan* P, int xo, bool s32) {
    const wt_model* M = P->model;
    const wt_arch& ar = M->arch;
    const int B = P->B, L = (int)P->L, D = ar.dim;
    const long Mrows = (long)B * L;
    const int Kb = M->Kb, hop = ar.hop_length;
    const int spec = P->buf("head.spec", (size_t)Mrows * 2 * Kb, s32 ? BUF_S32 : BUF_F32);
    GemmArgs ah = linear_args(M->head_W, M->head_b, Mrows, 2 * Kb, D);
    ah.c_rstride = 2 * Kb; ah.head_kb = Kb;
    gemm_step(P, s32, ah, {xo, -1, spec}, PRO_NONE, EPI_HEAD, OUT_S32, "head.out");
    const int Kq = M->Kq;
    const int parts = P->buf("head.parts", (size_t)4 * Mrows * Kq);
    GemmArgs ai = linear_args(M->istft_W, nullptr, Mrows, Kq, Kq);
    ai.a_rstride = 2 * Kb; ai.zA = Kq;
    ai.zW = (long)Kq * Kq; ai.nz = 4;
    ai.c_rstride = Kq; ai.zC = (long)Mrows * Kq;
    gemm_step(P, s32, ai, {spec, -1, parts}, PRO_NONE, EPI_BIAS, OUT_F32, "head.istft");
    P->step({parts}, [=](const RunCtx& c) {
        return launch_istft_ola(P->ptr(c, parts), M->win, M->wsq, c.out_f, B, L, ar.n_fft, hop, Kq, ar.padding_same ? 0 : 1, c.stream);
    }, 1, "head.ola");
}

int build_decode(wt_plan* P) {
    const wt_model* M = P->model;
    const wt_arch& ar = M->arch;
    const int B = P->B, L = (int)P->L, D = ar.dim, I = ar.intermediate_dim, Cin = ar.input_channels;
    const long Mrows = (long)B * L;
    const int Lp = ((L + 31) / 32) * 32;
    P->n_out = B * wave_samples(M, L); P->n_aux = Mrows * D;
    const bool s32_plan = plan_s32(P) && (Cin % 32 == 0) && (D % 32 == 0) && (I % 32 == 0);
    auto s32_at = [&](int site) { return s32_plan && !site_fp32(P, site); };
    P->cur_site = SITE_BB_EMBED;
    const bool s32_e = s32_at(SITE_BB_EMBED);
    const int x0 = P->buf("bb.in", (size_t)Mrows * Cin, s32_e ? BUF_S32 : BUF_F32);
    P->step({x0}, [=](const RunCtx& c) { return launch_transpose(c.in_f, P->ptr(c, x0), B, Cin, L, c.stream, s32_e); });
    const int x = P->buf("bb.x", (size_t)Mrows * D);
    gemm_step(P, s32_e, zconv_args(M->bb_embed, B, L), {x0, -1, x}, PRO_NONE, EPI_BIAS, OUT_F32);
    const bool keep = P->flags & WT_PLAN_FLAG_KEEP_STAGES;
    auto snapshot = [&](int src, const std::string& name) {
        if (keep) copy_step(P, src, P->buf(name, (size_t)Mrows * D), (size_t)Mrows * D);
    };
    snapshot(x, "bb.embed");
    const int sc = P->buf("bb.gn_scale", (size_t)B * D), sh = P->buf("bb.gn_shift", (size_t)B * D);
    const int gp = P->buf("bb.gn_part", gn_part_floats(B, L, 32));
    const int h1 = P->buf("bb.h1", (size_t)Mrows * D, s32_plan ? BUF_S32 : BUF_F32);
    const int h2 = P->buf("bb.h2", (size_t)Mrows * D);

    auto resnet = [&](const PosRes& r, const std::string& name, int site) {
        P->cur_site = site;
        const bool s32 = s32_at(site);
        P->bufs[h1].fmt = s32 ? BUF_S32 : BUF_F32;
        P->step({x, sc, sh, h1, gp}, [=](const RunCtx& c) {
            return launch_gn_apply(P->ptr(c, x), r.n1w, r.n1b, P->ptr(c, sc), P->ptr(c, sh), P->ptr(c, h1), 1, B, L, D, 32, 1e-6f, c.stream, s32, P->ptr(c, gp));
        }, 1, "res.gn1");
        gemm_step(P, s32, zconv_args(r.c1, B, L), {h1, -1, h2}, PRO_NONE, EPI_BIAS, OUT_F32, "res.conv1");
        P->step({h2, sc, sh, h1, gp}, [=](const RunCtx& c) {
            return launch_gn_apply(P->ptr(c, h2), r.n2w, r.n2b, P->ptr(c, sc), P->ptr(c, sh), P->ptr(c, h1), 1, B, L, D, 32, 1e-6f, c.stream, s32, P->ptr(c, gp));
        }, 1, "res.gn2");
        GemmArgs a2 = zconv_args(r.c2, B, L);
        a2.r_rstride = D;
        gemm_step(P, s32, a2, in_place(h1, x), PRO_NONE, EPI_BIAS_RES, OUT_F32, "res.conv2");
        snapshot(x, name);
    };
    resnet(M->res[0], "bb.pos_net.0", SITE_RES0);
    resnet(M->res[1], "bb.pos_net.1", SITE_RES1);
    {
        P->cur_site = SITE_ATTN;
        const bool s32 = s32_at(SITE_ATTN) && M->at_Wqk.s32.p && M->at_Wv.s32.p && M->at_Wp.s32.p;
        const int fmt = s32 ? BUF_S32 : BUF_F32;
        P->bufs[h1].fmt = fmt;
        const int qk = P->buf("bb.attn.qk", (size_t)Mrows * 2 * D, fmt);
        const int vt = P->buf("bb.attn.vt", (size_t)B * D * Lp, fmt);
        const int S = P->buf("bb.attn.s", (size_t)Mrows * Lp);
        const int Ps = s32 ? P->buf("bb.attn.p", (size_t)Mrows * Lp, BUF_S32) : S;
        const int o = P->buf("bb.attn.o", (size_t)Mrows * D, fmt);
        P->step({x, sc, sh, gp, h1}, [=](const RunCtx& c) {
            return launch_gn_apply(P->ptr(c, x), M->at_nw, M->at_nb, P->ptr(c, sc), P->ptr(c, sh), P->ptr(c, h1), 0, B, L, D, 32, 1e-6f, c.stream, s32, P->ptr(c, gp));
        }, 1, "attn.gn");
        gemm_step(P, s32, linear_args(M->at_Wqk, M->at_bqk, Mrows, 2 * D, D), {h1, -1, qk}, PRO_NONE, EPI_BIAS, OUT_S32, "attn.qk");
        P->step({h1, vt}, [=](const RunCtx& c) {
            if (int rc = launch_fill_u32(P->ptr(c, vt), 0u, (size_t)B * D * Lp * sizeof(float), c.stream)) return rc;
            GemmArgs a = linear_args(nullptr, M->at_bv, D, L, D);
            a.A = s32 ? static_cast<const float*>(M->at_Wv.s32.p) : M->at_Wv.w; a.acc_scale = M->at_Wv.s32.acc_scale; a.zA = 0;
            a.zW = (long)L * D; a.nz = B;
            a.C = P->ptr(c, vt); a.c_rstride = Lp; a.zC = (long)D * Lp;
            return dense_act(P, s32, a, P->ptr(c, h1), EPI_BIAS_ROW, OUT_S32, c.stream);
        }, 2, "attn.vt");
        P->step({qk, S}, [=](const RunCtx& c) {
            GemmArgs a = linear_args(nullptr, nullptr, L, L, D);
            a.A = P->ptr(c, qk); a.a_rstride = 2 * D; a.zA = (long)L * 2 * D;
            a.w_rstride = 2 * D; a.zW = (long)L * 2 * D; a.nz = B;
            a.C = P->ptr(c, S); a.c_rstride = Lp; a.zC = (long)L * Lp;
            a.alpha = (float)std::pow((double)D, -0.5);
            return dense_act(P, s32, a, P->ptr(c, qk) + D, EPI_SCALE, OUT_F32, c.stream);
        }, 1, "attn.s");
        P->step({S, Ps}, [=](const RunCtx& c) { return launch_softmax(P->ptr(c, S), (int)Mrows, L, Lp, c.stream, s32 ? P->ptr(c, Ps) : nullptr); });
        P->step({Ps, vt, o}, [=](const RunCtx& c) {
            GemmArgs a = linear_args(nullptr, nullptr, L, D, Lp);
            a.A = P->ptr(c, Ps); a.zA = (long)L * Lp;
            a.zW = (long)D * Lp; a.nz = B;
            a.C = P->ptr(c, o); a.c_rstride = D; a.zC = (long)L * D;
            return dense_act(P, s32, a, P->ptr(c, vt), EPI_BIAS, OUT_S32, c.stream);
        }, 1, "attn.o");
        GemmArgs ap = linear_args(M->at_Wp, M->at_bp, Mrows, D, D);
        ap.r_rstride = D;
        gemm_step(P, s32, ap, in_place(o, x), PRO_NONE, EPI_BIAS_RES, OUT_F32, "attn.proj");
        snapshot(x, "bb.pos_net.2");
    }
    resnet(M->res[2], "bb.pos_net.3", SITE_RES2);
    resnet(M->res[3], "bb.pos_net.4", SITE_RES3);
    P->cur_site = SITE_CNX0;
    const int xc = P->buf(keep ? "bb.x2" : "bb.norm", (size_t)Mrows * D);
    P->step({x, gp, sc, sh}, [=](const RunCtx& c) {
        return launch_gn_stats(P->ptr(c, x), M->gn5w, M->gn5b, P->ptr(c, sc), P->ptr(c, sh), B, L, D, 32, 1e-6f, c.stream, P->ptr(c, gp));
    });
    P->step({x, sc, sh, xc}, [=](const RunCtx& c) {
        return launch_rownorm(RN_AFFINE_IN, P->ptr(c, x), P->ptr(c, xc), B, L, D, nullptr, nullptr, P->ptr(c, sc),
                              P->ptr(c, sh), M->ada_s + (size_t)c.bw_id * D, M->ada_h + (size_t)c.bw_id * D, 1e-6f, c.stream);
    });
    snapshot(xc, "bb.norm");
    const int nrm = P->buf("bb.cnx.norm", (size_t)Mrows * D, s32_plan ? BUF_S32 : BUF_F32);
    const int mid = P->buf("bb.cnx.mid", (size_t)Mrows * I, s32_plan ? BUF_S32 : BUF_F32);
    for (int i = 0; i < ar.num_layers; ++i) {
        const CnxBlock cb = M->cnx[i];
        P->cur_site = SITE_CNX0 + i;
        const bool s32 = s32_at(SITE_CNX0 + i);
        P->bufs[nrm].fmt = P->bufs[mid].fmt = s32 ? BUF_S32 : BUF_F32;
        P->step({xc, nrm}, [=](const RunCtx& c) {
            return launch_rownorm(RN_DWCONV, P->ptr(c, xc), P->ptr(c, nrm), B, L, D, cb.dw_w, cb.dw_b, nullptr, nullptr,
                                  cb.ada_s + (size_t)c.bw_id * D, cb.ada_h + (size_t)c.bw_id * D, 1e-6f, c.stream, s32);
        });
        gemm_step(P, s32, linear_args(cb.W1, cb.b1, Mrows, I, D), {nrm, -1, mid}, PRO_NONE, EPI_BIAS_GELU, OUT_S32, "cnx.pwconv1");
        GemmArgs a2 = linear_args(cb.W2, cb.b2, Mrows, D, I);
        a2.r_rstride = D; a2.gamma = cb.gamma;
        gemm_step(P, s32, a2, in_place(mid, xc), PRO_NONE, EPI_BIAS_GAMMA_RES, OUT_F32, "cnx.pwconv2");
        if (i == 0 || i == ar.num_layers / 2 - 1 || i == ar.num_layers - 1) snapshot(xc, "bb.convnext." + std::to_string(i));
    }
    P->cur_site = SITE_HEAD;
    const bool s32 = s32_at(SITE_HEAD);
    const int xo = P->buf("bb.out", (size_t)Mrows * D, s32 ? BUF_S32 : BUF_F32);
    P->step({xc, xo}, [=](const RunCtx& c) {
        if (int rc = launch_rownorm(RN_PLAIN, P->ptr(c, xc), P->ptr(c, xo), B, L, D, nullptr, nullptr, nullptr, nullptr,
                                    M->fln_w, M->fln_b, 1e-6f, c.stream, s32)) return rc;
        if (c.aux && s32)
            return launch_rownorm(RN_PLAIN, P->ptr(c, xc), c.aux, B, L, D, nullptr, nullptr, nullptr, nullptr, M->fln_w,
                                  M->fln_b, 1e-6f, c.stream, 0);
        return c.aux ? copy_f32(c.aux, P->ptr(c, xo), (size_t)Mrows * D, c.stream) : 0;
    });
    plan_head(P, xo, s32);
    return 0;
}

int build_head(wt_plan* P) {
    const wt_model* M = P->model;
    const int B = P->B, L = (int)P->L, D = M->arch.dim;
    const long Mrows = (long)B * L;
    const bool s32 = plan_s32(P) && (D % 32 == 0) && M->head_W.s32.p && M->istft_W.s32.p;
    const int xo = P->buf("head.in", (size_t)Mrows * D, s32 ? BUF_S32 : BUF_F32);
    if (s32) P->step({xo}, [=](const RunCtx& c) { return launch_split_s32(c.in_f, P->ptr(c, xo), Mrows * D, c.stream); });
    else copy_step(P, CALLER, xo, (size_t)Mrows * D);
    P->n_out = P->B * wave_samples(M, L);
    plan_head(P, xo, s32);
    return 0;
}

static bool seadec_s32_ok(const wt_plan* P) {
    const wt_model* M = P->model;
    if (!plan_s32(P) || M->sd_stages.empty() || !M->sd_first.s32.p || !M->sd_lstm.Wih0.s32.p) return false;
    for (const SeaDecStage& st : M->sd_stages) {
        if (!st.tr_wp.s32.p || st.cout % 32) return false;
        if (!resblock_fusable(st.cout) && !(st.c3.s32.p && st.c1.s32.p && st.sc.s32.p)) return false;
    }
    return resblock_fusable(M->sd_stages.back().cout);
}

int build_seanet_decoder(wt_plan* P) {
    const wt_model* M = P->model;
    if (!M->has_seadec) { set_error("checkpoint holds no SEANetDecoder weights"); return WT_ERR_MISSING_TENSOR; }
    const int B = P->B, L = (int)P->L, H = M->H;
    P->n_out = (long)B * L * M->hop;
    const bool s32 = seadec_s32_ok(P);
    const bool fuse_elu = !plan_unfused(P);
    const int x0 = P->buf("sdec.in", (size_t)B * L * 512);
    P->step({x0}, [=](const RunCtx& c) { return launch_transpose(c.in_f, P->ptr(c, x0), B, 512, L, c.stream, s32); });
    const int xf = P->buf("sdec.0", (size_t)B * L * H);
    const int xs = s32 ? P->buf("sdec.0.s32", (size_t)B * L * H) : -1;
    P->bufs[x0].holds_s32 = s32;
    if (xs >= 0) P->bufs[xs].holds_s32 = true;
    gemm_step(P, s32, sconv_args(M->sd_first, B, L, 1, 1), {x0, -1, xf, xs}, PRO_NONE, EPI_BIAS, OUT_F32_AND_S32);
    int x = plan_lstm(P, M->sd_lstm, B, L, H, xf, "sdec.1", fuse_elu, xs, s32);
    long Tc = L;
    int di = 2;
    for (size_t si = 0; si < M->sd_stages.size(); ++si) {
        const SeaDecStage st = M->sd_stages[si];
        const long To = Tc * st.r;
        const int xin = x;
        const int Tin = (int)Tc;
        const bool unfused_s32 = s32 && !resblock_fusable(st.cout);
        const bool last = si + 1 == M->sd_stages.size();
        const std::string name = "sdec." + std::to_string(di + 1);
        int y, y2 = -1;
        long y_off = 0, y_bs = 0;
        if (st.tr_wp.w) {
            const int trim_l = (st.k - st.r) - (st.k - st.r) / 2;
            const size_t ynum = (size_t)B * (Tin + 1) * st.r * st.cout;
            y = P->buf(name, ynum);
            if (unfused_s32) { y2 = P->buf(name + ".elu", ynum); P->bufs[y].holds_s32 = P->bufs[y2].holds_s32 = true; }
            y_off = (long)trim_l * st.cout;
            y_bs = (long)(Tin + 1) * st.r * st.cout;
            GemmArgs a;
            a.a_bstride = (long)Tin * st.cin; a.a_rstride = st.cin;
            a.T_in = Tin; a.T_out = Tin + 1; a.Cin = st.cin; a.taps = 2; a.pad_left = 1; a.pad_mode = PAD_ZERO;
            a.W = st.tr_wp.w; a.w_rstride = 2L * st.cin; a.zW = (long)st.cout * 2 * st.cin; a.bias = st.tr_b;
            a.M = B * (Tin + 1); a.N = st.cout; a.K = 2 * st.cin;
            a.c_rstride = (long)st.r * st.cout; a.zC = st.cout; a.nz = st.r;
            set_s32(a, st.tr_wp.s32);
            gemm_step(P, s32, a, {xin, -1, y, y2}, fuse_elu ? PRO_NONE : PRO_ELU, EPI_BIAS, y2 >= 0 ? OUT_S32_DUAL_ELU : OUT_F32, "sdec.convtr");
        } else {
            y = P->buf(name, (size_t)B * To * st.cout);
            P->step({xin, y}, [=](const RunCtx& c) {
                return launch_convtr(P->ptr(c, xin), st.tr_w, st.tr_b, P->ptr(c, y), B, Tin, st.cin, st.cout, st.k, st.r,
                                     fuse_elu ? 0 : 1, c.stream);
            }, 1, "sdec.convtr");
        }
        const std::string rname = "sdec." + std::to_string(di + 2);
        if (unfused_s32)
            x = plan_resblock_s32(P, st.c3, st.sc, st.cat, B, To, y, y2, rname, y_off, y_bs);
        else
            x = plan_resblock(P, st.c3, st.c1, st.sc, B, To, y, rname, fuse_elu, nullptr, y_off, y_bs, s32 && !last);
        if (x < 0) return WT_ERR_INVALID;
        Tc = To; di += 3;
    }
    const int xin = x;
    const long Tf = Tc;
    P->step({xin}, [=](const RunCtx& c) {
        return launch_conv_last(P->ptr(c, xin), M->sd_last_w, M->sd_last_b, c.out_f, B, Tf, 32, 7, fuse_elu ? 0 : 1, c.stream);
    }, 1, "sdec.last");
    return 0;
}


void plan_begin(wt_plan* P) {
    P->ctl = P->buf("ctl", CTL_WORDS);
    const int ctl = P->ctl;
    P->step({ctl}, [=](const RunCtx& c) {
        return launch_fill_u32(P->ptr(c, ctl), 0u, CTL_WORDS * sizeof(unsigned), c.stream);
    }, 1, "ctl.clear");
}

void plan_end(wt_plan* P) {
    const wt_model* M = P->model;
    const int ctl = P->ctl;
    const long nc = P->n_codes, n0 = P->n_out, n1 = P->n_aux;
    P->step({ctl}, [=](const RunCtx& c) {
        return launch_plan_guard(reinterpret_cast<const unsigned*>(P->ptr(c, ctl)), CTL_WORDS, CTL_SITE0, P->status_dev, M->status_dev,
                                 nc ? c.codes : nullptr, nc, c.out_f, n0, n1 ? c.aux : nullptr, n1, nullptr, 0, c.stream);
    }, 1, "guard");
}

int build_unit_lstm(wt_plan* P) {
    const wt_model* M = P->model;
    const int B = P->B, L = (int)P->L, H = M->H;
    const bool s32 = plan_s32(P) && M->enc_lstm.Wih0.s32.p;
    const int x = P->buf("lstm.in", (size_t)B * L * H);
    const int xs = s32 ? P->buf("lstm.in.s32", (size_t)B * L * H, BUF_S32) : -1;
    P->n_out = (long)B * L * 512;
    P->step({x, xs}, [=](const RunCtx& c) {
        if (int rc = copy_f32(P->ptr(c, x), c.in_f, (size_t)B * L * H, c.stream)) return rc;
        return s32 ? launch_split_s32(c.in_f, P->ptr(c, xs), (long)B * L * H, c.stream) : 0;
    }, 2, "lstm.in");
    const int y = plan_lstm(P, M->enc_lstm, B, L, H, x, "lstm.out", false, xs, false);
    copy_step(P, y, CALLER, (size_t)B * L * H, "lstm.copy");
    return 0;
}

}
```

### wavtokenizer_amd/csrc/probe.cpp

```cpp
#include "model.h"

using namespace wt;

extern "C" {

int wt_codes_to_features(const wt_model* m, const int64_t* codes, int32_t K, int32_t B, int64_t L, float* features,
                         void* stream) {
    if (!m || !codes || !features) { set_error("wt_codes_to_features: null argument"); return WT_ERR_INVALID; }
    if (K < 1 || K > m->arch.num_quantizers) { set_error("wt_codes_to_features: K exceeds the number of codebooks"); return WT_ERR_INVALID; }
    DeviceGuard dg(m->device);
    if (!dg.ok) { set_error("hipSetDevice failed"); return WT_ERR_HIP; }
    return launch_codes_to_features(codes, m->embed.w, K, m->arch.vq_bins, B, L, 512, features, static_cast<hipStream_t>(stream),
                                    m->bad_codes_dev);
}

int wt_sconv1d(const float* x, const float* w, const float* bias, float* y, int32_t B, int64_t T, int32_t Cin,
               int32_t Cout, int32_t k, int32_t stride, int32_t dilation, int32_t elu_input, void* stream) {
    ConvW cw; cw.w = const_cast<float*>(w); cw.b = const_cast<float*>(bias); cw.cout = Cout; cw.cin = Cin; cw.k = k;
    GemmArgs a = sconv_args(cw, B, T, stride, dilation);
    a.A = x; a.C = y;
    return launch_gemm(a, elu_input ? PRO_ELU : PRO_NONE, EPI_BIAS, static_cast<hipStream_t>(stream));
}

static int split_pair(const float* w, long nw, const float* x, long nx, char* ws_w, char* ws_x, char* tail, GemmArgs& a,
                      hipStream_t s) {
    unsigned* bits = reinterpret_cast<unsigned*>(tail);
    float* sc = reinterpret_cast<float*>(tail + 16);
    if (int rc = launch_pow2_scales(w, nw, x, nx, bits, sc, s)) return rc;
    if (int rc = launch_split_s32(w, ws_w, nw, s, sc)) return rc;
    if (int rc = launch_split_s32(x, ws_x, nx, s, sc + 1)) return rc;
    a.W_hi = ws_w;
    a.A = reinterpret_cast<const float*>(ws_x);
    a.acc_scale_dev = sc + 2;
    return 0;
}

int wt_linear(const float* x, const float* w, const float* bias, float* y, int64_t M, int32_t N, int32_t K,
              int32_t f16x3, void* workspace, void* stream) {
    if (!x || !w || !y) { set_error("wt_linear: null argument"); return WT_ERR_INVALID; }
    hipStream_t s = static_cast<hipStream_t>(stream);
    GemmArgs a = linear_args(w, bias, M, N, K);
    a.A = x; a.C = y;
    if (!f16x3) return launch_gemm(a, PRO_NONE, EPI_BIAS, s);
    if (!workspace) { set_error("wt_linear: the f16x3 modes need a workspace"); return WT_ERR_INVALID; }
    char* hi = static_cast<char*>(workspace);
    if (f16x3 == 1) { set_error("wt_linear: mode 1 (the in-loop split kernel of round 1) was removed; use 2, 3 or 4"); return WT_ERR_INVALID; }
    char* xs = hi + (size_t)N * K * 4;
    if (int rc = split_pair(w, (long)N * K, x, (long)M * K, hi, xs, xs + (size_t)M * K * 4, a, s)) return rc;
    a.dbg_stamps = reinterpret_cast<unsigned long long*>(xs + (size_t)M * K * 4 + 256);
    if (f16x3 == 4) return launch_gemm16s(a, EPI_BIAS_GELU, OUT_S32, s);
    return launch_gemm16s(a, EPI_BIAS, f16x3 == 3 ? 1 : 0, s);
}

int wt_conv1d_s32(const float* x, const float* w, const float* bias, float* y, int32_t B, int64_t T, int32_t Cin,
                  int32_t Cout, int32_t k, int32_t stride, int32_t zero_same, void* workspace, void* stream) {
    if (!x || !w || !y || !workspace) { set_error("wt_conv1d_s32: null argument"); return WT_ERR_INVALID; }
    hipStream_t s = static_cast<hipStream_t>(stream);
    ConvW cw; cw.w = const_cast<float*>(w); cw.b = const_cast<float*>(bias); cw.cout = Cout; cw.cin = Cin; cw.k = k;
    GemmArgs a = zero_same ? zconv_args(cw, B, (int)T) : sconv_args(cw, B, T, stride, 1);
    char* ws = static_cast<char*>(workspace);
    char* xs = ws + (size_t)Cout * k * Cin * 4;
    if (int rc = split_pair(w, (long)Cout * k * Cin, x, (long)B * T * Cin, ws, xs, xs + (size_t)B * T * Cin * 4, a, s)) return rc;
    a.C = y;
    return launch_gemm16s(a, EPI_BIAS, 0, s);
}

static size_t al256(size_t b) { return (b + 255) / 256 * 256; }

struct ProbeLayout { long nA = 0, nA2 = 0, nB = 0; size_t oA2 = 0, oB = 0, oScale = 0, total = 0; };
static ProbeLayout probe_layout(const wt_gemm_desc& d) {
    ProbeLayout L;
    const long clips = d.M / d.T_out;
    const long a_cols = d.A2 ? d.K1 : d.Cin;
    L.nA = (d.nz - 1) * d.zA + (clips - 1) * d.a_bstride + (long)(d.T_in - 1) * d.a_rstride + a_cols;
    if (d.A2) L.nA2 = (clips - 1) * d.a2_bstride + (long)(d.T_in - 1) * d.a2_rstride + (d.K - d.K1);
    L.nB = (d.nz - 1) * d.zW + (long)(d.N - 1) * d.w_rstride + d.K;
    L.oA2 = al256((size_t)L.nA * 4);
    L.oB = L.oA2 + al256((size_t)L.nA2 * 4);
    L.oScale = L.oB + al256((size_t)L.nB * 4);
    L.total = L.oScale + 256;
    return L;
}
static int probe_args(const wt_gemm_desc* d, char* ws, GemmArgs& a) {
    if (!d || d->size != (int32_t)sizeof(wt_gemm_desc)) { set_error("wt_gemm_probe: descriptor missing or of another size"); return WT_ERR_INVALID; }
    if (d->engine != 0 && d->engine != 1) { set_error("wt_gemm_probe: engine is 0 (gemm16s) or 1 (gemm)"); return WT_ERR_INVALID; }
    if (!d->A || !d->B || !d->C) { set_error("wt_gemm_probe: A, B and C are required"); return WT_ERR_INVALID; }
    if (d->epi == EPI_ARGMAX) { set_error("wt_gemm_probe: the argmax epilogue is reached through wt_vq_nearest"); return WT_ERR_INVALID; }
    if (d->M <= 0 || d->N <= 0 || d->K <= 0 || d->T_out <= 0 || d->T_in <= 0 || d->M % d->T_out || d->nz < 1 || d->taps < 1 ||
        d->stride < 1 || d->dil < 1 || d->pad_left < 0 || (d->pad_mode != PAD_ZERO && d->pad_mode != PAD_REFLECT) ||
        d->a_bstride < 0 || d->a_rstride < 0 || d->a2_bstride < 0 || d->a2_rstride < 0 || d->w_rstride < d->K ||
        d->c_rstride < d->N || d->r_rstride < 0 || d->zA < 0 || d->zW < 0 || d->zC < 0 || (d->nz > 1 && d->zC <= 0)) {
        set_error("wt_gemm_probe: bad extents or strides"); return WT_ERR_INVALID;
    }
    if (d->engine == 1 && (d->out != OUT_F32 || d->A2 || d->tap_pair)) {
        set_error("wt_gemm_probe: gemm.hip writes fp32 and has no second K source or tap pairing"); return WT_ERR_INVALID;
    }
    if (d->engine == 0 && d->pro != PRO_NONE) { set_error("wt_gemm_probe: gemm16s has no operand prologue"); return WT_ERR_INVALID; }
    if (d->tap_pair && (d->taps != 2 * d->stride || d->dil != 1)) { set_error("wt_gemm_probe: tap pairing needs k = 2 * stride, dilation 1"); return WT_ERR_INVALID; }
    if (d->engine == 0 && (!ws || (reinterpret_cast<uintptr_t>(ws) & 255))) { set_error("wt_gemm_probe: gemm16s needs a 256-byte aligned workspace"); return WT_ERR_INVALID; }
    a = GemmArgs{};
    a.a_bstride = d->a_bstride; a.a_rstride = d->a_rstride; a.T_in = d->T_in; a.T_out = d->T_out; a.Cin = d->Cin; a.taps = d->taps;
    a.stride = d->stride; a.dil = d->dil; a.pad_left = d->pad_left; a.pad_mode = d->pad_mode; a.Tp = d->Tp;
    a.a2_bstride = d->a2_bstride; a.a2_rstride = d->a2_rstride; a.K1 = d->K1;
    a.w_rstride = d->w_rstride; a.bias = d->bias; a.M = d->M; a.N = d->N; a.K = d->K;
    a.C = d->C; a.c_rstride = d->c_rstride; a.C2 = d->C2; a.R = d->R; a.r_rstride = d->r_rstride; a.gamma = d->gamma;
    a.alpha = d->alpha; a.nz = d->nz; a.zA = d->zA; a.zW = d->zW; a.zC = d->zC; a.head_kb = d->head_kb; a.tap_pair = d->tap_pair ? 1 : 0;
    if (d->engine == 1) {
        a.A = d->A; a.W = d->B;
        return check_gemm(a, d->pro, d->epi) ? WT_ERR_INVALID : WT_OK;
    }
    const ProbeLayout L = probe_layout(*d);
    a.A = reinterpret_cast<const float*>(ws);
    a.A2 = d->A2 ? reinterpret_cast<const float*>(ws + L.oA2) : nullptr;
    a.W = d->B; a.W_hi = ws + L.oB;
    a.status = reinterpret_cast<unsigned*>(d->status);
    return check_gemm16s(a, d->epi, d->out) ? WT_ERR_INVALID : WT_OK;
}

size_t wt_gemm_probe_workspace_bytes(const wt_gemm_desc* d) {
    if (!d || d->size != (int32_t)sizeof(wt_gemm_desc) || d->engine != 0 || d->M <= 0 || d->T_out <= 0 || d->nz < 1) return 0;
    return probe_layout(*d).total;
}

int wt_gemm_probe(const wt_gemm_desc* d, wt_launch_form* form, void* workspace, void* stream) {
    char* ws = static_cast<char*>(workspace);
    GemmArgs a;
    if (int rc = probe_args(d, ws, a)) return rc;
    hipStream_t s = static_cast<hipStream_t>(stream);
    LaunchForm lf;
    a.form = &lf;
    if (d->engine == 1) {
        if (int rc = launch_gemm(a, d->pro, d->epi, s)) return rc;
    } else {
        const ProbeLayout L = probe_layout(*d);
        float* scale_dev = reinterpret_cast<float*>(ws + L.oScale);
        float scale = 1.f;
        if (!d->b_is_act) {
            std::vector<float> h((size_t)L.nB);
            WT_HIP_CHECK(hipMemcpyAsync(h.data(), d->B, (size_t)L.nB * 4, hipMemcpyDeviceToHost, s));
            WT_HIP_CHECK(hipStreamSynchronize(s));
            float amax = 0.f;
            for (long z = 0; z < d->nz; ++z)
                for (long n = 0; n < d->N; ++n)
                    for (long k = 0; k < d->K; ++k) {
                        const float v = std::fabs(h[(size_t)(z * d->zW + n * d->w_rstride + k)]);
                        if (!(v <= 3.0e38f)) { set_error("wt_gemm_probe: a non-finite weight has no S32 copy"); return WT_ERR_INVALID; }
                        amax = std::max(amax, v);
                    }
            scale = s32_weight_scale(amax);
            uint32_t bits;
            memcpy(&bits, &scale, 4);
            if (int rc = launch_fill_u32(scale_dev, bits, 16, s)) return rc;
            a.acc_scale = 1.f / scale;
        }
        if (int rc = launch_split_s32(d->B, ws + L.oB, L.nB, s, scale != 1.f ? scale_dev : nullptr)) return rc;
        if (int rc = launch_split_s32(d->A, ws, L.nA, s)) return rc;
        if (d->A2) if (int rc = launch_split_s32(d->A2, ws + L.oA2, L.nA2, s)) return rc;
        if (int rc = launch_gemm16s(a, d->epi, d->out, s)) return rc;
    }
    if (form) *form = wt_launch_form{lf.BM, lf.BN, lf.waves_m, lf.waves_n, lf.stages, lf.ks, lf.prod, lf.staged, lf.bias_cache, lf.G, lf.tiles};
    return WT_OK;
}

static int op_probe_check(const wt_op_desc* d) {
    auto bad = [](const char* m) { set_error(std::string("wt_op_probe: ") + m); return (int)WT_ERR_INVALID; };
    if (!d || d->size != (int32_t)sizeof(wt_op_desc)) return bad("descriptor missing or of another size");
    if (d->op < WT_OP_GN_APPLY || d->op > WT_OP_S32_AMAX) return bad("unknown op");
    auto al16 = [](const void* p) { return !(reinterpret_cast<uintptr_t>(p) & 15); };
    const void* ptrs[] = {d->p0, d->p1, d->p2, d->p3, d->p4, d->p5, d->y, d->y2, d->y3};
    for (const void* p : ptrs) if (!al16(p)) return bad("arrays must be 16-byte aligned");
    if (!d->x || (reinterpret_cast<uintptr_t>(d->x) & (d->op == WT_OP_SOFTMAX ? 3 : 15))) return bad("x missing or misaligned");
    if (reinterpret_cast<uintptr_t>(d->status) & 3) return bad("status misaligned");
    const bool shaped = d->op != WT_OP_SOFTMAX && d->op != WT_OP_ROW_SUMSQ && d->op != WT_OP_S32_AMAX;
    if (shaped && (d->B <= 0 || d->L <= 0)) return bad("extents must be positive");
    if (shaped && d->op != WT_OP_CONV_FIRST && d->op != WT_OP_ISTFT_OLA && (d->C <= 0 || (long)d->L * d->C >= (long)INT_MAX)) return bad("extents must be positive (and L * C < 2^31)");
    switch (d->op) {
    case WT_OP_GN_APPLY: case WT_OP_GN_STATS:
        if (!d->p0 || !d->p1 || !d->y2 || !d->y3 || (d->op == WT_OP_GN_APPLY && !d->y)) return bad("null argument");
        if (d->groups <= 0 || d->C % d->groups || d->C / d->groups > 256 || d->B > 65535) return bad("GroupNorm needs C % groups == 0, at most 256 channels per group, B <= 65535");
        break;
    case WT_OP_ROWNORM:
        if (!d->y || !d->p4 || !d->p5) return bad("null argument");
        if (d->mode < RN_DWCONV || d->mode > RN_AFFINE_IN) return bad("rownorm mode is 0, 1 or 2");
        if (d->mode == RN_DWCONV && (!d->p0 || !d->p1)) return bad("null argument");
        if (d->mode == RN_AFFINE_IN && (!d->p2 || !d->p3)) return bad("null argument");
        break;
    case WT_OP_SOFTMAX:
        if (d->n <= 0 || d->n > INT_MAX || d->L <= 0 || d->ld < d->L) return bad("softmax needs rows > 0 and 0 < L <= ld");
        break;
    case WT_OP_ISTFT_OLA:
        if (!d->p0 || !d->p1 || !d->y) return bad("null argument");
        if (d->n_fft <= 0 || d->hop <= 0 || d->n_fft % 4 || d->n_fft % d->hop || (d->n_fft - d->hop) % 2 || d->Kq < d->n_fft / 4 + 1)
            return bad("the ISTFT tail needs n_fft % 4 == 0, n_fft % hop == 0 and Kq > n_fft / 4");
        break;
    case WT_OP_CONV_FIRST:
        if (!d->p0 || !d->p1 || !d->y) return bad("null argument");
        if (d->k <= 0 || d->Cout <= 0 || d->Cout % 4) return bad("conv_first needs k > 0 and Cout % 4 == 0");
        break;
    case WT_OP_CONV_LAST:
        if (!d->p0 || !d->p1 || !d->y) return bad("null argument");
        if (d->k <= 0) return bad("conv_last needs k > 0");
        break;
    case WT_OP_TRANSPOSE:
        if (!d->y) return bad("null argument");
        if (d->B > 65535 || (d->L + 31) / 32 > 65535) return bad("transpose: too many tiles for one launch");
        break;
    case WT_OP_CONVTR:
        if (!d->p0 || !d->p1 || !d->y) return bad("null argument");
        if (d->stride <= 0 || d->k < d->stride || d->Cout <= 0 || d->Cout % 4) return bad("convtr needs k >= stride > 0 and Cout % 4 == 0");
        break;
    case WT_OP_ROW_SUMSQ:
        if (!d->y) return bad("null argument");
        if (d->n <= 0 || d->C <= 0 || d->C % 4) return bad("row_sumsq needs rows > 0 and C % 4 == 0");
        break;
    case WT_OP_S32_AMAX:
        if (!d->y) return bad("null argument");
        if (d->n <= 0 || d->n % 32) return bad("s32_amax needs whole S32 groups of 32 values");
        break;
    }
    return WT_OK;
}

int wt_op_probe(const wt_op_desc* d, wt_op_form* form, void* stream) {
    if (int rc = op_probe_check(d)) return rc;
    hipStream_t s = static_cast<hipStream_t>(stream);
    auto F = [](const void* p) { return static_cast<const float*>(p); };
    auto W = [](void* p) { return static_cast<float*>(p); };
    OpForm lf;
    const LaunchCtx saved = g_launch;
    g_launch.status = reinterpret_cast<unsigned*>(d->status);
    g_launch.form = &lf;
    int rc = 0;
    switch (d->op) {
    case WT_OP_GN_APPLY:
        rc = launch_gn_apply(F(d->x), F(d->p0), F(d->p1), W(d->y2), W(d->y3), W(d->y), d->flag ? 1 : 0, d->B, d->L, d->C, d->groups, d->eps, s,
                             d->out_s32 ? 1 : 0, const_cast<float*>(F(d->p2)));
        break;
    case WT_OP_GN_STATS:
        rc = launch_gn_stats(F(d->x), F(d->p0), F(d->p1), W(d->y2), W(d->y3), d->B, d->L, d->C, d->groups, d->eps, s, const_cast<float*>(F(d->p2)));
        break;
    case WT_OP_ROWNORM:
        rc = launch_rownorm(d->mode, F(d->x), W(d->y), d->B, d->L, d->C, F(d->p0), F(d->p1), F(d->p2), F(d->p3), F(d->p4), F(d->p5), d->eps, s,
                            d->out_s32 ? 1 : 0);
        break;
    case WT_OP_SOFTMAX:
        rc = launch_softmax(const_cast<float*>(F(d->x)), (int)d->n, d->L, d->ld, s, W(d->y));
        break;
    case WT_OP_ISTFT_OLA:
        rc = launch_istft_ola(F(d->x), F(d->p0), F(d->p1), W(d->y), d->B, d->L, d->n_fft, d->hop, d->Kq, d->flag ? 1 : 0, s);
        break;
    case WT_OP_CONV_FIRST:
        rc = launch_conv_first(F(d->x), F(d->p0), F(d->p1), W(d->y), d->B, d->L, d->k, d->Cout, s);
        break;
    case WT_OP_CONV_LAST:
        rc = launch_conv_last(F(d->x), F(d->p0), F(d->p1), W(d->y), d->B, d->L, d->C, d->k, d->flag ? 1 : 0, s);
        break;
    case WT_OP_TRANSPOSE:
        rc = launch_transpose(F(d->x), W(d->y), d->B, d->L, d->C, s, d->out_s32 ? 1 : 0);
        break;
    case WT_OP_CONVTR:
        rc = launch_convtr(F(d->x), F(d->p0), F(d->p1), W(d->y), d->B, d->L, d->C, d->Cout, d->k, d->stride, d->flag ? 1 : 0, s);
        break;
    case WT_OP_ROW_SUMSQ:
        rc = launch_row_sumsq(F(d->x), W(d->y), d->n, d->C, s);
        break;
    case WT_OP_S32_AMAX:
        rc = launch_s32_amax(d->x, d->n, static_cast<unsigned*>(d->y), s);
        break;
    }
    g_launch = saved;
    if (rc) return rc;
    if (form) *form = wt_op_form{lf.kernel, lf.variant, lf.variant2, (int32_t)lf.grid[0], (int32_t)lf.grid[1], (int32_t)lf.grid[2], (int32_t)lf.block, (int32_t)lf.lds};
    return WT_OK;
}

size_t wt_vq_workspace_bytes(int64_t N, int32_t D, int32_t bins) {
    const size_t np = std::max(gemm_vq_parts(bins), gemm16s_vq_parts(bins));
    return al256((size_t)N * D * 4) + al256((size_t)bins * D * 4) + al256((size_t)N * sizeof(float)) +
           2 * al256((size_t)N * np * sizeof(float)) + al256((size_t)bins * sizeof(float)) + 512;
}

static int vq_nearest(const float* x, const float* embed, int64_t N, int32_t D, int32_t bins, int64_t* codes_out,
                      void* workspace, void* stream, bool s32) {
    if (!x || !embed || !codes_out || !workspace) { set_error("wt_vq_nearest: null argument"); return WT_ERR_INVALID; }
    if (s32 && (D % 32)) { set_error("wt_vq_nearest: the split-f16 kernel needs D % 32 == 0"); return WT_ERR_INVALID; }
    hipStream_t s = static_cast<hipStream_t>(stream);
    const int np = s32 ? gemm16s_vq_parts(bins) : gemm_vq_parts(bins);
    char* ws = static_cast<char*>(workspace);
    char* xs = ws; ws += al256((size_t)N * D * 4);
    char* es = ws; ws += al256((size_t)bins * D * 4);
    float* xx = reinterpret_cast<float*>(ws); ws += al256((size_t)N * sizeof(float));
    float* pv = reinterpret_cast<float*>(ws); ws += al256((size_t)N * np * sizeof(float));
    int* pi = reinterpret_cast<int*>(ws); ws += al256((size_t)N * np * sizeof(float));
    float* ee = reinterpret_cast<float*>(ws); ws += al256((size_t)bins * sizeof(float));
    if (int rc = launch_row_sumsq(x, xx, N, D, s)) return rc;
    if (int rc = launch_row_sumsq(embed, ee, bins, D, s)) return rc;
    GemmArgs a = linear_args(embed, nullptr, N, bins, D);
    a.A = x; a.vq_xx = xx; a.vq_ee = ee; a.vq_pval = pv; a.vq_pidx = pi; a.vq_nparts = np;
    if (s32) {
        if (int rc = split_pair(embed, (long)bins * D, x, (long)N * D, es, xs, ws, a, s)) return rc;
        if (int rc = launch_gemm16s(a, EPI_ARGMAX, OUT_F32, s)) return rc;
    } else {
        if (int rc = launch_gemm(a, PRO_NONE, EPI_ARGMAX, s)) return rc;
    }
    for (int64_t r0 = 0; r0 < N; r0 += 8192) {
        const int n = (int)std::min<int64_t>(8192, N - r0);
        if (int rc = launch_vq_finalize(pv + r0 * np, pi + r0 * np, np, embed, codes_out + r0, nullptr, 1, n, D, bins, s)) return rc;
    }
    return WT_OK;
}
int wt_vq_nearest(const float* x, const float* embed, int64_t N, int32_t D, int32_t bins, int64_t* codes_out,
                  void* workspace, void* stream) {
    return vq_nearest(x, embed, N, D, bins, codes_out, workspace, stream, true);
}
int wt_vq_nearest_f32(const float* x, const float* embed, int64_t N, int32_t D, int32_t bins, int64_t* codes_out,
                      void* workspace, void* stream) {
    return vq_nearest(x, embed, N, D, bins, codes_out, workspace, stream, false);
}

int wt_resblock(const float* x, const float* wav, const float* e0_w, const float* e0_b, const float* w3, const float* b3,
                const float* w1, const float* b1, const float* ws, const float* bs, float* y, int32_t B, int64_t T,
                int32_t C, int32_t elu_out, int32_t out_s32, int32_t fp32_chain, void* stream) {
    if ((!x && !wav) || !w3 || !b3 || !w1 || !b1 || !ws || !bs || !y) { set_error("wt_resblock: null argument"); return WT_ERR_INVALID; }
    if (wav && (!e0_w || !e0_b)) { set_error("wt_resblock: the folded first conv needs its weights"); return WT_ERR_INVALID; }
    if (B < 1 || T < 1 || (long)B * T >= (long)INT_MAX) { set_error("wt_resblock: bad shape"); return WT_ERR_INVALID; }
    if (fp32_chain && out_s32) { set_error("wt_resblock: the fp32 kernel writes fp32"); return WT_ERR_INVALID; }
    ResblockArgs a{};
    a.x = wav ? nullptr : x; a.wav = wav; a.e0_w = e0_w; a.e0_b = e0_b;
    a.W3 = w3; a.b3 = b3; a.W1 = w1; a.b1 = b1; a.Ws = ws; a.bs = bs;
    a.y = y; a.B = B; a.T = (int)T; a.C = C; a.elu_out = elu_out ? 1 : 0; a.out_s32 = out_s32 ? 1 : 0;
    hipStream_t s = static_cast<hipStream_t>(stream);
    return fp32_chain ? launch_resblock(a, s) : launch_resblock16(a, s);
}

int wt_resblock_down(const float* wav, const float* e0_w, const float* e0_b, const float* w3, const float* b3, const float* w1,
                     const float* b1, const float* ws, const float* bs, const float* wd, const float* bd, float* y_down,
                     int32_t B, int64_t T, int32_t r, void* stream) {
    if (!wav || !e0_w || !e0_b || !w3 || !b3 || !w1 || !b1 || !ws || !bs || !wd || !bd || !y_down) {
        set_error("wt_resblock_down: null argument"); return WT_ERR_INVALID;
    }
    if (B < 1 || T < 1 || (long)B * T >= (long)INT_MAX) { set_error("wt_resblock_down: bad shape"); return WT_ERR_INVALID; }
    if (!resblock16_down_fusable(32, T, r, 2 * r)) {
        set_error("wt_resblock_down: needs stride 2 or 4 and T >= 1024"); return WT_ERR_INVALID;
    }
    ResblockArgs a{};
    a.wav = wav; a.e0_w = e0_w; a.e0_b = e0_b; a.W3 = w3; a.b3 = b3; a.W1 = w1; a.b1 = b1; a.Ws = ws; a.bs = bs;
    a.Wd = wd; a.bd = bd; a.y_down = y_down; a.R = r; a.B = B; a.T = (int)T; a.C = 32;
    return launch_resblock16_down(a, static_cast<hipStream_t>(stream));
}


}
```

### wavtokenizer_amd/csrc/weights.cpp

```cpp
#include "model.h"

namespace wt {

static int upload(wt_model* M, const std::vector<float>& h, float** out) {
    void* d = nullptr;
    size_t bytes = std::max<size_t>(h.size(), 4) * sizeof(float);
    WT_HIP_CHECK(hipMalloc(&d, bytes));
    M->allocs.push_back(d);
    M->alloc_bytes.push_back(bytes);
    WT_HIP_CHECK(hipMemcpy(d, h.data(), h.size() * sizeof(float), hipMemcpyHostToDevice));
    M->weight_bytes += (int64_t)h.size() * sizeof(float);
    *out = static_cast<float*>(d);
    return 0;
}
static int upload_raw(wt_model* M, const float* src, int64_t n, float** out) {
    std::vector<float> h(src, src + n);
    return upload(M, h, out);
}

static std::vector<float> fold_wn(const float* g, const float* v, int d0, int64_t inner) {
    std::vector<float> w((size_t)d0 * inner);
    for (int o = 0; o < d0; ++o) {
        double ss = 0.0;
        for (int64_t i = 0; i < inner; ++i) { double x = v[o * inner + i]; ss += x * x; }
        const double sc = (double)g[o] / std::sqrt(ss);
        for (int64_t i = 0; i < inner; ++i) w[o * inner + i] = (float)(sc * (double)v[o * inner + i]);
    }
    return w;
}

static std::vector<float> repack_ock(const std::vector<float>& w, int cout, int cin, int k) {
    std::vector<float> o(w.size());
    for (int a = 0; a < cout; ++a)
        for (int c = 0; c < cin; ++c)
            for (int j = 0; j < k; ++j) o[((size_t)a * k + j) * cin + c] = w[((size_t)a * cin + c) * k + j];
    return o;
}

static int load_wn_conv(wt_model* M, TensorMap& tm, const std::string& prefix, int cout, int cin, int k, ConvW* out) {
    const float* g = tm.get(prefix + ".weight_g", cout);
    const float* v = tm.get(prefix + ".weight_v", (int64_t)cout * cin * k);
    const float* b = tm.get(prefix + ".bias", cout);
    if (!g || !v || !b) return WT_ERR_MISSING_TENSOR;
    std::vector<float> w = repack_ock(fold_wn(g, v, cout, (int64_t)cin * k), cout, cin, k);
    out->cout = cout; out->cin = cin; out->k = k;
    if (int rc = upload(M, w, &out->w)) return rc;
    return upload_raw(M, b, cout, &out->b);
}

static int load_plain_conv(wt_model* M, TensorMap& tm, const std::string& prefix, int cout, int cin, int k, ConvW* out) {
    const float* w = tm.get(prefix + ".weight", (int64_t)cout * cin * k);
    const float* b = tm.get(prefix + ".bias", cout);
    if (!w || !b) return WT_ERR_MISSING_TENSOR;
    std::vector<float> wv(w, w + (int64_t)cout * cin * k);
    std::vector<float> p = repack_ock(wv, cout, cin, k);
    out->cout = cout; out->cin = cin; out->k = k;
    if (int rc = upload(M, p, &out->w)) return rc;
    return upload_raw(M, b, cout, &out->b);
}

static int load_vec(wt_model* M, TensorMap& tm, const std::string& key, int64_t n, float** out) {
    const float* p = tm.get(key, n);
    if (!p) return WT_ERR_MISSING_TENSOR;
    return upload_raw(M, p, n, out);
}
static int upload_gemm(wt_model* M, const std::vector<float>& h, int rows, int cols, GemmW* out) {
    out->rows = rows; out->cols = cols; return upload(M, h, &out->w);
}
static int load_gemm(wt_model* M, TensorMap& tm, const std::string& key, int rows, int cols, GemmW* out) {
    out->rows = rows; out->cols = cols; return load_vec(M, tm, key, (int64_t)rows * cols, &out->w);
}

static int load_lstm(wt_model* M, TensorMap& tm, const std::string& prefix, int H, LstmW* out, bool* split_ok) {
    const float* wih0 = tm.get(prefix + ".lstm.weight_ih_l0", 4LL * H * H);
    const float* whh0 = tm.get(prefix + ".lstm.weight_hh_l0", 4LL * H * H);
    const float* bih0 = tm.get(prefix + ".lstm.bias_ih_l0", 4LL * H);
    const float* bhh0 = tm.get(prefix + ".lstm.bias_hh_l0", 4LL * H);
    const float* wih1 = tm.get(prefix + ".lstm.weight_ih_l1", 4LL * H * H);
    const float* whh1 = tm.get(prefix + ".lstm.weight_hh_l1", 4LL * H * H);
    const float* bih1 = tm.get(prefix + ".lstm.bias_ih_l1", 4LL * H);
    const float* bhh1 = tm.get(prefix + ".lstm.bias_hh_l1", 4LL * H);
    if (!wih0 || !whh0 || !bih0 || !bhh0 || !wih1 || !whh1 || !bih1 || !bhh1) return WT_ERR_MISSING_TENSOR;
    std::vector<float> Wih0((size_t)4 * H * H), W0((size_t)4 * H * H), W1((size_t)4 * H * 2 * H), b0(4 * H), b1(4 * H);
    auto put = [&](std::vector<float>& dst, size_t prow, int Ktot, int k, float v) {
        const size_t blk = prow / 16, li = prow % 16;
        const int S = k / 16, e = (k % 16) / 4, lk = k % 4;
        dst[blk * 16 * Ktot + (size_t)S * 256 + (size_t)(lk * 16 + li) * 4 + e] = v;
    };
    std::vector<_Float16> W0h((size_t)4 * H * H * 2), W1h((size_t)4 * H * 2 * H * 2);
    auto put16 = [&](std::vector<_Float16>& dst, size_t prow, int Ktot, int k, float v) {
        const size_t blk = prow / 16, li = prow % 16;
        const int P = k / 32, r = k % 32, pp = (r / 16) * 4 + (r % 16) / 4, lk = r % 4;
        const size_t base = blk * 16 * Ktot * 2 + (size_t)P * 1024 + (size_t)(lk * 16 + li) * 8 + pp;
        const _Float16 h = (_Float16)v;
        dst[base] = h;
        dst[base + 512] = (_Float16)((v - (float)h) * 2048.f);
    };
    std::vector<_Float16> Wp(H == 512 ? (size_t)3 * 2048 * 512 * 2 : 0);
    auto putp = [&](int role, size_t prow, int k, float v) {
        if (Wp.empty()) return;
        const size_t wg = prow / 64, tile = (prow % 64) / 16, li = prow % 16;
        const int blk = k / 32, lk = (k % 32) / 8, pp = k % 8;
        const size_t base = ((((size_t)role * 32 + wg) * 4 + tile) * 16 + blk) * 2 * 64 * 8 + (size_t)(lk * 16 + li) * 8 + pp;
        const _Float16 h = (_Float16)v;
        Wp[base] = h;
        Wp[base + 64 * 8] = (_Float16)((v - (float)h) * 2048.f);
    };
    for (const float* wsrc : {whh0, wih1, whh1})
        for (size_t i = 0; i < (size_t)4 * H * H; ++i)
            if (!(std::fabs(wsrc[i]) < 65504.f)) *split_ok = false;
    for (int g = 0; g < 4; ++g)
        for (int j = 0; j < H; ++j) {
            const size_t src = (size_t)g * H + j;
            const size_t dst = (size_t)(j / 4) * 16 + g * 4 + (j % 4);
            std::memcpy(&Wih0[dst * H], &wih0[src * H], H * sizeof(float));
            for (int k = 0; k < H; ++k) {
                put(W0, dst, H, k, whh0[src * H + k]);
                put(W1, dst, 2 * H, k, wih1[src * H + k]);
                put(W1, dst, 2 * H, H + k, whh1[src * H + k]);
                put16(W0h, dst, H, k, whh0[src * H + k]);
                put16(W1h, dst, 2 * H, k, wih1[src * H + k]);
                put16(W1h, dst, 2 * H, H + k, whh1[src * H + k]);
                putp(0, dst, k, whh0[src * H + k]);
                putp(1, dst, k, wih1[src * H + k]);
                putp(2, dst, k, whh1[src * H + k]);
            }
            b0[dst] = bih0[src] + bhh0[src];
            b1[dst] = bih1[src] + bhh1[src];
        }
    if (int rc = upload_gemm(M, Wih0, 4 * H, H, &out->Wih0)) return rc;
    if (int rc = upload(M, b0, &out->b0)) return rc;
    if (int rc = upload(M, W0, &out->W0)) return rc;
    if (int rc = upload(M, W1, &out->W1)) return rc;
    {
        std::vector<float> t0(W0.size()), t1(W1.size());
        std::memcpy(t0.data(), W0h.data(), t0.size() * sizeof(float));
        std::memcpy(t1.data(), W1h.data(), t1.size() * sizeof(float));
        if (int rc = upload(M, t0, &out->W0h)) return rc;
        if (int rc = upload(M, t1, &out->W1h)) return rc;
        if (!Wp.empty()) {
            std::vector<float> tp(Wp.size() / 2);
            std::memcpy(tp.data(), Wp.data(), tp.size() * sizeof(float));
            if (int rc = upload(M, tp, &out->Wp)) return rc;
        }
    }
    return upload(M, b1, &out->b1);
}

static int build_cat(wt_model* M, const ConvW& sc, const ConvW& c1, ConvW* cat) {
    if (sc.k != 1 || c1.k != 1 || sc.cout != c1.cout) return 0;
    const int C = sc.cout, K1 = sc.cin, K2 = c1.cin;
    std::vector<float> ws((size_t)C * K1), w1((size_t)C * K2), bs(C), b1(C), w((size_t)C * (K1 + K2)), b(C);
    WT_HIP_CHECK(hipMemcpy(ws.data(), sc.w, ws.size() * sizeof(float), hipMemcpyDeviceToHost));
    WT_HIP_CHECK(hipMemcpy(w1.data(), c1.w, w1.size() * sizeof(float), hipMemcpyDeviceToHost));
    WT_HIP_CHECK(hipMemcpy(bs.data(), sc.b, bs.size() * sizeof(float), hipMemcpyDeviceToHost));
    WT_HIP_CHECK(hipMemcpy(b1.data(), c1.b, b1.size() * sizeof(float), hipMemcpyDeviceToHost));
    for (int n = 0; n < C; ++n) {
        std::memcpy(&w[(size_t)n * (K1 + K2)], &ws[(size_t)n * K1], K1 * sizeof(float));
        std::memcpy(&w[(size_t)n * (K1 + K2) + K1], &w1[(size_t)n * K2], K2 * sizeof(float));
        b[n] = bs[n] + b1[n];
    }
    if (int rc = upload(M, w, &cat->w)) return rc;
    if (int rc = upload(M, b, &cat->b)) return rc;
    cat->cout = C; cat->cin = K1 + K2; cat->k = 1;
    return 0;
}

static const char* ENC = "feature_extractor.encodec.encoder.model.";
static const char* DEC = "feature_extractor.encodec.decoder.model.";
static const char* VQK = "feature_extractor.encodec.quantizer.vq.layers.0._codebook.";

int build_model(wt_model* M, TensorMap& tm) {
    const wt_arch& a = M->arch;
    const int nf = 32, H = 512;
    M->H = H;
    {
        const float* g = tm.get(std::string(ENC) + "0.conv.conv.weight_g", nf);
        const float* v = tm.get(std::string(ENC) + "0.conv.conv.weight_v", (int64_t)nf * 7);
        const float* b = tm.get(std::string(ENC) + "0.conv.conv.bias", nf);
        if (!g || !v || !b) return WT_ERR_MISSING_TENSOR;
        std::vector<float> w = fold_wn(g, v, nf, 7);
        std::vector<float> p((size_t)7 * nf);
        for (int c = 0; c < nf; ++c)
            for (int j = 0; j < 7; ++j) p[(size_t)j * nf + c] = w[(size_t)c * 7 + j];
        if (int rc = upload(M, p, &M->e0_w)) return rc;
        if (int rc = upload_raw(M, b, nf, &M->e0_b)) return rc;
    }
    int idx = 1, mult = 1;
    for (int r : M->enc_ratios) {
        ResStage st;
        st.C = mult * nf; st.r = r;
        const std::string p = std::string(ENC) + std::to_string(idx);
        if (int rc = load_wn_conv(M, tm, p + ".block.1.conv.conv", st.C / 2, st.C, 3, &st.c3)) return rc;
        if (int rc = load_wn_conv(M, tm, p + ".block.3.conv.conv", st.C, st.C / 2, 1, &st.c1)) return rc;
        if (int rc = load_wn_conv(M, tm, p + ".shortcut.conv.conv", st.C, st.C, 1, &st.sc)) return rc;
        if (int rc = load_wn_conv(M, tm, std::string(ENC) + std::to_string(idx + 2) + ".conv.conv", 2 * st.C, st.C, 2 * r, &st.down)) return rc;
        if (!resblock_fusable(st.C)) if (int rc = build_cat(M, st.sc, st.c1, &st.cat)) return rc;
        M->stages.push_back(st);
        idx += 3; mult *= 2;
    }
    if (mult * nf != H) { set_error("encoder width after the last ratio must be 512"); return WT_ERR_INVALID; }
    if (int rc = load_lstm(M, tm, std::string(ENC) + std::to_string(idx), H, &M->enc_lstm, &M->s32_ok)) return rc;
    if (int rc = load_wn_conv(M, tm, std::string(ENC) + std::to_string(idx + 2) + ".conv.conv", 512, H, 7, &M->enc_final)) return rc;

    {
        const float* inited = tm.get(std::string(VQK) + "inited", 1);
        const float* e = tm.get(std::string(VQK) + "embed", (int64_t)a.vq_bins * 512);
        if (!inited || !e) return WT_ERR_MISSING_TENSOR;
        if (inited[0] != 1.0f) {
            set_error("codebook buffer `inited` is not 1: the reference would run k-means on the first forward (core_vq.py:140-151)");
            return WT_ERR_NOT_INITED;
        }
        std::vector<float> all((size_t)a.num_quantizers * a.vq_bins * 512);
        std::memcpy(all.data(), e, (size_t)a.vq_bins * 512 * sizeof(float));
        for (int q = 1; q < a.num_quantizers; ++q) {
            const std::string pq = "feature_extractor.encodec.quantizer.vq.layers." + std::to_string(q) + "._codebook.";
            const float* eq = tm.get(pq + "embed", (int64_t)a.vq_bins * 512);
            if (!eq) return WT_ERR_MISSING_TENSOR;
            std::memcpy(all.data() + (size_t)q * a.vq_bins * 512, eq, (size_t)a.vq_bins * 512 * sizeof(float));
        }
        M->embed.rows = a.vq_bins; M->embed.cols = 512;
        if (int rc = upload(M, all, &M->embed.w)) return rc;
        std::vector<float> ee(a.vq_bins);
        for (int n = 0; n < a.vq_bins; ++n) {
            float s = 0.f;
            for (int c = 0; c < 512; ++c) s += e[(size_t)n * 512 + c] * e[(size_t)n * 512 + c];
            ee[n] = s;
        }
        if (int rc = upload(M, ee, &M->ee)) return rc;
    }

    const int D = a.dim, I = a.intermediate_dim, A = a.adanorm_num_embeddings;
    if (int rc = load_plain_conv(M, tm, "backbone.embed", D, a.input_channels, 7, &M->bb_embed)) return rc;
    const int ridx[4] = {0, 1, 3, 4};
    for (int i = 0; i < 4; ++i) {
        const std::string p = "backbone.pos_net." + std::to_string(ridx[i]);
        PosRes& r = M->res[i];
        if (int rc = load_vec(M, tm, p + ".norm1.weight", D, &r.n1w)) return rc;
        if (int rc = load_vec(M, tm, p + ".norm1.bias", D, &r.n1b)) return rc;
        if (int rc = load_vec(M, tm, p + ".norm2.weight", D, &r.n2w)) return rc;
        if (int rc = load_vec(M, tm, p + ".norm2.bias", D, &r.n2b)) return rc;
        if (int rc = load_plain_conv(M, tm, p + ".conv1", D, D, 3, &r.c1)) return rc;
        if (int rc = load_plain_conv(M, tm, p + ".conv2", D, D, 3, &r.c2)) return rc;
    }
    {
        const std::string p = "backbone.pos_net.2";
        if (int rc = load_vec(M, tm, p + ".norm.weight", D, &M->at_nw)) return rc;
        if (int rc = load_vec(M, tm, p + ".norm.bias", D, &M->at_nb)) return rc;
        const float* wq = tm.get(p + ".q.weight", (int64_t)D * D);
        const float* wk = tm.get(p + ".k.weight", (int64_t)D * D);
        const float* bq = tm.get(p + ".q.bias", D);
        const float* bk = tm.get(p + ".k.bias", D);
        if (!wq || !wk || !bq || !bk) return WT_ERR_MISSING_TENSOR;
        std::vector<float> wqk((size_t)2 * D * D), bqk(2 * D);
        std::memcpy(&wqk[0], wq, (size_t)D * D * sizeof(float));
        std::memcpy(&wqk[(size_t)D * D], wk, (size_t)D * D * sizeof(float));
        std::memcpy(&bqk[0], bq, D * sizeof(float));
        std::memcpy(&bqk[D], bk, D * sizeof(float));
        if (int rc = upload_gemm(M, wqk, 2 * D, D, &M->at_Wqk)) return rc;
        if (int rc = upload(M, bqk, &M->at_bqk)) return rc;
        if (int rc = load_gemm(M, tm, p + ".v.weight", D, D, &M->at_Wv)) return rc;
        if (int rc = load_vec(M, tm, p + ".v.bias", D, &M->at_bv)) return rc;
        if (int rc = load_gemm(M, tm, p + ".proj_out.weight", D, D, &M->at_Wp)) return rc;
        if (int rc = load_vec(M, tm, p + ".proj_out.bias", D, &M->at_bp)) return rc;
    }
    if (int rc = load_vec(M, tm, "backbone.pos_net.5.weight", D, &M->gn5w)) return rc;
    if (int rc = load_vec(M, tm, "backbone.pos_net.5.bias", D, &M->gn5b)) return rc;
    if (A <= 0) { set_error("only the AdaLayerNorm (adanorm_num_embeddings > 0) backbone is implemented"); return WT_ERR_INVALID; }
    if (int rc = load_vec(M, tm, "backbone.norm.scale.weight", (int64_t)A * D, &M->ada_s)) return rc;
    if (int rc = load_vec(M, tm, "backbone.norm.shift.weight", (int64_t)A * D, &M->ada_h)) return rc;
    for (int i = 0; i < a.num_layers; ++i) {
        const std::string p = "backbone.convnext." + std::to_string(i);
        CnxBlock c;
        const float* dw = tm.get(p + ".dwconv.weight", (int64_t)D * 7);
        if (!dw) return WT_ERR_MISSING_TENSOR;
        std::vector<float> dwp((size_t)7 * D);
        for (int ch = 0; ch < D; ++ch)
            for (int j = 0; j < 7; ++j) dwp[(size_t)j * D + ch] = dw[(size_t)ch * 7 + j];
        if (int rc = upload(M, dwp, &c.dw_w)) return rc;
        if (int rc = load_vec(M, tm, p + ".dwconv.bias", D, &c.dw_b)) return rc;
        if (int rc = load_vec(M, tm, p + ".norm.scale.weight", (int64_t)A * D, &c.ada_s)) return rc;
        if (int rc = load_vec(M, tm, p + ".norm.shift.weight", (int64_t)A * D, &c.ada_h)) return rc;
        if (int rc = load_gemm(M, tm, p + ".pwconv1.weight", I, D, &c.W1)) return rc;
        if (int rc = load_vec(M, tm, p + ".pwconv1.bias", I, &c.b1)) return rc;
        if (int rc = load_gemm(M, tm, p + ".pwconv2.weight", D, I, &c.W2)) return rc;
        if (int rc = load_vec(M, tm, p + ".pwconv2.bias", D, &c.b2)) return rc;
        if (int rc = load_vec(M, tm, p + ".gamma", D, &c.gamma)) return rc;
        M->cnx.push_back(c);
    }
    if (int rc = load_vec(M, tm, "backbone.final_layer_norm.weight", D, &M->fln_w)) return rc;
    if (int rc = load_vec(M, tm, "backbone.final_layer_norm.bias", D, &M->fln_b)) return rc;

    {
        const int N = a.n_fft, hop = a.hop_length;
        if (N % hop != 0 || N % 2 != 0 || (N - hop) % 2 != 0) {
            set_error("ISTFT kernel needs n_fft to be an even multiple of hop_length"); return WT_ERR_INVALID;
        }
        if (N % 4 != 0) { set_error("ISTFT kernel needs n_fft % 4 == 0"); return WT_ERR_INVALID; }
        const int bins = N / 2 + 1;
        const int Q = N / 4;
        const int Kq = ((Q + 1 + 31) / 32) * 32;
        const int Kb = 2 * Kq;
        const int R = N / hop;
        M->Kb = Kb; M->Kq = Kq; M->bins_f = bins; M->R = R;
        const float* w = tm.get("head.out.weight", (int64_t)(N + 2) * D);
        const float* b = tm.get("head.out.bias", N + 2);
        const float* win = tm.get("head.istft.window", N);
        if (!w || !b || !win) return WT_ERR_MISSING_TENSOR;
        auto slot_bin = [&](int s) { int f = s < Kq ? 2 * s : 2 * (s - Kq) + 1; return f <= N / 2 && (s < Kq || s - Kq < Q) ? f : -1; };
        std::vector<float> wp((size_t)2 * Kb * D, 0.f), bp((size_t)2 * Kb, 0.f);
        for (int sl = 0; sl < Kb; ++sl) {
            const int f = slot_bin(sl);
            if (f < 0) continue;
            const size_t pm = (size_t)(sl / 16) * 32 + (sl % 16), pp = pm + 16;
            std::memcpy(&wp[pm * D], &w[(size_t)f * D], D * sizeof(float));
            std::memcpy(&wp[pp * D], &w[(size_t)(bins + f) * D], D * sizeof(float));
            bp[pm] = b[f];
            bp[pp] = b[bins + f];
        }
        if (int rc = upload_gemm(M, wp, 2 * Kb, D, &M->head_W)) return rc;
        if (int rc = upload(M, bp, &M->head_b)) return rc;
        std::vector<float> basis((size_t)4 * Kq * Kq, 0.f);
        const double two_pi = 6.283185307179586476925286766559;
        for (int n = 0; n <= Q; ++n)
            for (int g = 0; g <= Q; ++g) {
                const int fe = 2 * g, fo = 2 * g + 1;
                const bool edge = (fe == 0) || (fe == N / 2);
                const double ce = (edge ? 1.0 : 2.0) / (double)N, co = 2.0 / (double)N;
                const double the = two_pi * (double)(((long)fe * n) % N) / (double)N;
                const double tho = two_pi * (double)(((long)fo * n) % N) / (double)N;
                basis[((size_t)0 * Kq + n) * Kq + g] = (float)(ce * std::cos(the));
                basis[((size_t)2 * Kq + n) * Kq + g] = edge ? 0.f : (float)(ce * std::sin(the));
                if (g < Q) {
                    basis[((size_t)1 * Kq + n) * Kq + g] = (float)(co * std::cos(tho));
                    basis[((size_t)3 * Kq + n) * Kq + g] = (float)(co * std::sin(tho));
                }
            }
        if (int rc = upload_gemm(M, basis, 4 * Kq, Kq, &M->istft_W)) return rc;
        if (int rc = upload_raw(M, win, N, &M->win)) return rc;
        std::vector<float> wsq(N);
        for (int n = 0; n < N; ++n) wsq[n] = win[n] * win[n];
        if (int rc = upload(M, wsq, &M->wsq)) return rc;
    }

    M->has_seadec = tm.has(std::string(DEC) + "0.conv.conv.weight_v");
    if (M->has_seadec) {
        int m2 = 1 << a.n_ratios;
        if (int rc = load_wn_conv(M, tm, std::string(DEC) + "0.conv.conv", m2 * nf, 512, 7, &M->sd_first)) return rc;
        if (int rc = load_lstm(M, tm, std::string(DEC) + "1", H, &M->sd_lstm, &M->sd_s32_ok)) return rc;
        int di = 2;
        for (int i = 0; i < a.n_ratios; ++i) {
            const int r = a.ratios[i];
            SeaDecStage st;
            st.cin = m2 * nf; st.cout = st.cin / 2; st.k = 2 * r; st.r = r;
            const std::string p = std::string(DEC) + std::to_string(di + 1) + ".convtr.convtr";
            const float* g = tm.get(p + ".weight_g", st.cin);
            const float* v = tm.get(p + ".weight_v", (int64_t)st.cin * st.cout * st.k);
            const float* b = tm.get(p + ".bias", st.cout);
            if (!g || !v || !b) return WT_ERR_MISSING_TENSOR;
            std::vector<float> w = fold_wn(g, v, st.cin, (int64_t)st.cout * st.k);
            std::vector<float> pk((size_t)st.k * st.cin * st.cout);
            for (int ci = 0; ci < st.cin; ++ci)
                for (int co = 0; co < st.cout; ++co)
                    for (int j = 0; j < st.k; ++j)
                        pk[((size_t)j * st.cin + ci) * st.cout + co] = w[((size_t)ci * st.cout + co) * st.k + j];
            if (int rc = upload(M, pk, &st.tr_w)) return rc;
            if (st.k == 2 * r) {
                std::vector<float> pp((size_t)r * st.cout * 2 * st.cin);
                for (int ph = 0; ph < r; ++ph)
                    for (int co = 0; co < st.cout; ++co)
                        for (int ci = 0; ci < st.cin; ++ci) {
                            pp[(((size_t)ph * st.cout + co) * 2 + 0) * st.cin + ci] = w[((size_t)ci * st.cout + co) * st.k + ph + r];
                            pp[(((size_t)ph * st.cout + co) * 2 + 1) * st.cin + ci] = w[((size_t)ci * st.cout + co) * st.k + ph];
                        }
                if (int rc = upload_gemm(M, pp, r * st.cout, 2 * st.cin, &st.tr_wp)) return rc;
            }
            if (int rc = upload_raw(M, b, st.cout, &st.tr_b)) return rc;
            const std::string rp = std::string(DEC) + std::to_string(di + 2);
            const int h = st.cout;
            if (int rc = load_wn_conv(M, tm, rp + ".block.1.conv.conv", h / 2, h, 3, &st.c3)) return rc;
            if (int rc = load_wn_conv(M, tm, rp + ".block.3.conv.conv", h, h / 2, 1, &st.c1)) return rc;
            if (int rc = load_wn_conv(M, tm, rp + ".shortcut.conv.conv", h, h, 1, &st.sc)) return rc;
            if (!resblock_fusable(h)) if (int rc = build_cat(M, st.sc, st.c1, &st.cat)) return rc;
            M->sd_stages.push_back(st);
            di += 3; m2 /= 2;
        }
        const std::string p = std::string(DEC) + std::to_string(di + 1) + ".conv.conv";
        const float* g = tm.get(p + ".weight_g", 1);
        const float* v = tm.get(p + ".weight_v", (int64_t)nf * 7);
        const float* b = tm.get(p + ".bias", 1);
        if (!g || !v || !b) return WT_ERR_MISSING_TENSOR;
        std::vector<float> w = fold_wn(g, v, 1, (int64_t)nf * 7);
        std::vector<float> pk((size_t)7 * nf);
        for (int c = 0; c < nf; ++c)
            for (int j = 0; j < 7; ++j) pk[(size_t)j * nf + c] = w[(size_t)c * 7 + j];
        if (int rc = upload(M, pk, &M->sd_last_w)) return rc;
        if (int rc = upload_raw(M, b, 1, &M->sd_last_b)) return rc;
    }
    return 0;
}

float s32_weight_scale(float amax) {
    if (!(amax > 0.f) || (amax >= 0x1p-6f && amax < 0x1p12f)) return 1.f;
    int e = 0;
    (void)std::frexp(amax, &e);
    return std::ldexp(1.f, 1 - e);
}
static int add_s32(wt_model* M, const float* w, long n, S32Copy* out, bool* split_ok = nullptr, bool gemm_only = false) {
    if (!w || n <= 0 || (n % 32)) return 0;
    if (!split_ok) split_ok = &M->s32_ok;
    std::vector<float> h((size_t)n);
    WT_HIP_CHECK(hipMemcpy(h.data(), w, (size_t)n * sizeof(float), hipMemcpyDeviceToHost));
    float amax = 0.f;
    bool finite = true;
    for (long i = 0; i < n; ++i) {
        const float v = std::fabs(h[i]);
        if (!(v <= 3.0e38f)) finite = false;
        else amax = std::max(amax, v);
    }
    if (!finite) *split_ok = false;
    M->w_amax = std::max(M->w_amax, amax);
    const float scale = finite ? s32_weight_scale(amax) : 1.f;
    float* scale_dev = nullptr;
    if (scale != 1.f) {
        if (int rc = upload(M, std::vector<float>{scale}, &scale_dev)) return rc;
        out->acc_scale = 1.f / scale;
    }
    void* d = nullptr;
    WT_HIP_CHECK(hipMalloc(&d, (size_t)n * 4));
    M->allocs.push_back(d);
    M->alloc_bytes.push_back((size_t)n * 4);
    M->weight_bytes += n * 4;
    if (int rc = launch_split_s32(w, d, n, nullptr, scale_dev)) return rc;
    out->p = d;
    if (gemm_only && finite) M->lazy_f32.push_back({w, d, (int64_t)n, scale});
    return 0;
}

int build_splits(wt_model* M) {
    auto conv32 = [&](ConvW& c, bool gemm_only = true) { return (c.cin % 32) ? 0 : add_s32(M, c.w, (long)c.cout * c.k * c.cin, &c.s32, nullptr, gemm_only); };
    auto gemm32 = [&](GemmW& g, bool* split_ok = nullptr, bool gemm_only = true) { return add_s32(M, g.w, (long)g.rows * g.cols, &g.s32, split_ok, gemm_only); };
    auto conv32sd = [&](ConvW& c) { return (c.cin % 32) ? 0 : add_s32(M, c.w, (long)c.cout * c.k * c.cin, &c.s32, &M->sd_s32_ok, true); };
    for (ResStage& st : M->stages) {
        if (st.down.cin % 32 == 0 && st.down.k == 2 * st.r && st.down.k <= 32) {
            const long n = (long)st.down.cout * st.down.k * st.down.cin;
            std::vector<float> h((size_t)n), pk((size_t)n);
            WT_HIP_CHECK(hipMemcpy(h.data(), st.down.w, (size_t)n * sizeof(float), hipMemcpyDeviceToHost));
            for (int co = 0; co < st.down.cout; ++co)
                for (int q = 0; q < st.down.k; ++q) {
                    const int tap = (q >> 1) + (q & 1) * st.r;
                    std::memcpy(&pk[((size_t)co * st.down.k + q) * st.down.cin], &h[((size_t)co * st.down.k + tap) * st.down.cin],
                                st.down.cin * sizeof(float));
                }
            float* dpk = nullptr;
            if (int rc = upload(M, pk, &dpk)) return rc;
            if (int rc = add_s32(M, dpk, n, &st.down.s32)) return rc;
            M->lazy_f32.push_back({dpk, nullptr, (int64_t)n, 1.f});
            st.down.s32.tap_pair = true;
        } else
        if (int rc = conv32(st.down, false)) return rc;
        const bool fused = resblock_fusable(st.C);
        if (int rc = conv32(st.c3, !fused)) return rc;
        if (int rc = conv32(st.c1, !fused)) return rc;
        if (int rc = conv32(st.sc, !fused)) return rc;
        if (st.cat.w) if (int rc = conv32(st.cat)) return rc;
    }
    if (int rc = gemm32(M->enc_lstm.Wih0)) return rc;
    if (int rc = conv32(M->enc_final)) return rc;
    if (int rc = gemm32(M->embed, nullptr, false)) return rc;
    if (int rc = conv32(M->bb_embed)) return rc;
    for (int i = 0; i < 4; ++i) {
        if (int rc = conv32(M->res[i].c1)) return rc;
        if (int rc = conv32(M->res[i].c2)) return rc;
    }
    for (CnxBlock& c : M->cnx) {
        if (int rc = gemm32(c.W1)) return rc;
        if (int rc = gemm32(c.W2)) return rc;
    }
    if (int rc = gemm32(M->head_W)) return rc;
    if (int rc = gemm32(M->istft_W)) return rc;
    if (int rc = gemm32(M->at_Wqk)) return rc;
    if (int rc = gemm32(M->at_Wv)) return rc;
    if (int rc = gemm32(M->at_Wp)) return rc;
    if (M->has_seadec) {
        if (int rc = conv32sd(M->sd_first)) return rc;
        if (int rc = gemm32(M->sd_lstm.Wih0, &M->sd_s32_ok)) return rc;
        for (SeaDecStage& st : M->sd_stages) {
            if (st.tr_wp.w && st.cin % 16 == 0) if (int rc = gemm32(st.tr_wp, &M->sd_s32_ok)) return rc;
            if (resblock_fusable(st.cout)) continue;
            if (int rc = conv32sd(st.sc)) return rc;
            if (int rc = conv32sd(st.c3)) return rc;
            if (int rc = conv32sd(st.c1)) return rc;
            if (st.cat.w) if (int rc = conv32sd(st.cat)) return rc;
        }
    }
    WT_HIP_CHECK(hipDeviceSynchronize());
    return 0;
}


static constexpr uint32_t PACK_MAGIC = 0x4b505457u;
static constexpr int32_t PACK_VERSION = 7;

static uint64_t arch_hash_of(const wt_arch& a) {
    uint64_t h = 1469598103934665603ull;
    auto mix = [&](const void* p, size_t n) { for (size_t i = 0; i < n; ++i) { h ^= static_cast<const unsigned char*>(p)[i]; h *= 1099511628211ull; } };
    mix(&a, sizeof(a));
    mix(&PACK_VERSION, sizeof(PACK_VERSION));
    return h;
}

struct Archive {
    bool saving;
    std::vector<char>* out = nullptr;
    const char* in = nullptr;
    size_t pos = 0, n = 0;
    bool ok = true;
    const std::map<const void*, int>* index = nullptr;
    const std::vector<void*>* allocs = nullptr;
    const std::vector<size_t>* alloc_bytes = nullptr;
    void raw(void* p, size_t bytes) {
        if (saving) { const char* c = static_cast<const char*>(p); out->insert(out->end(), c, c + bytes); }
        else { if (!ok || bytes > n - pos) { ok = false; std::memset(p, 0, bytes); return; } std::memcpy(p, in + pos, bytes); pos += bytes; }
    }
    int32_t count(size_t have, int32_t limit) {
        int32_t c = (int32_t)have;
        pod(c);
        if (!saving && (c < 0 || c > limit)) { ok = false; c = 0; }
        return c;
    }
    template <class T> void pod(T& v) { raw(&v, sizeof(T)); }
    template <class T> void ptr(T*& p) {
        int32_t idx = -1;
        int64_t off = 0;
        if (saving && p) {
            auto it = index->upper_bound(static_cast<const void*>(p));
            if (it == index->begin()) { ok = false; }
            else { --it; idx = it->second; off = reinterpret_cast<const char*>(p) - static_cast<const char*>(it->first); }
        }
        pod(idx); pod(off);
        if (!saving) {
            if (idx < 0) p = nullptr;
            else if (!ok || idx >= (int)allocs->size() || off < 0 || (size_t)off >= (*alloc_bytes)[idx]) { ok = false; p = nullptr; }
            else p = reinterpret_cast<T*>(static_cast<char*>((*allocs)[idx]) + off);
        }
    }
    void s32(S32Copy& s) { ptr(s.p); pod(s.acc_scale); pod(s.tap_pair); }
    void conv(ConvW& c) { ptr(c.w); ptr(c.b); pod(c.cout); pod(c.cin); pod(c.k); s32(c.s32); }
    void gemm(GemmW& g) { ptr(g.w); pod(g.rows); pod(g.cols); s32(g.s32); }
    void lstm(LstmW& l) { gemm(l.Wih0); ptr(l.b0); ptr(l.W0); ptr(l.W1); ptr(l.b1); ptr(l.W0h); ptr(l.W1h); ptr(l.Wp); }
};

static void archive_model(Archive& ar, wt_model* M) {
    ar.pod(M->hop); ar.pod(M->H); ar.pod(M->weight_bytes); ar.pod(M->s32_ok); ar.pod(M->sd_s32_ok); ar.pod(M->w_amax);
    int32_t n = ar.count(M->enc_ratios.size(), 8);
    M->enc_ratios.resize(n);
    for (int& r : M->enc_ratios) ar.pod(r);
    ar.ptr(M->e0_w); ar.ptr(M->e0_b); ar.pod(M->e0_k); ar.pod(M->e0_c);
    n = ar.count(M->stages.size(), 8); M->stages.resize(n);
    for (ResStage& st : M->stages) { ar.conv(st.c3); ar.conv(st.c1); ar.conv(st.sc); ar.conv(st.down); ar.conv(st.cat); ar.pod(st.C); ar.pod(st.r); }
    ar.lstm(M->enc_lstm); ar.conv(M->enc_final); ar.gemm(M->embed); ar.ptr(M->ee);
    ar.conv(M->bb_embed);
    for (PosRes& r : M->res) { ar.ptr(r.n1w); ar.ptr(r.n1b); ar.ptr(r.n2w); ar.ptr(r.n2b); ar.conv(r.c1); ar.conv(r.c2); }
    ar.ptr(M->at_nw); ar.ptr(M->at_nb); ar.gemm(M->at_Wqk); ar.ptr(M->at_bqk); ar.gemm(M->at_Wv); ar.ptr(M->at_bv); ar.gemm(M->at_Wp); ar.ptr(M->at_bp);
    ar.ptr(M->gn5w); ar.ptr(M->gn5b); ar.ptr(M->ada_s); ar.ptr(M->ada_h);
    n = ar.count(M->cnx.size(), 64); M->cnx.resize(n);
    for (CnxBlock& c : M->cnx) { ar.ptr(c.dw_w); ar.ptr(c.dw_b); ar.ptr(c.ada_s); ar.ptr(c.ada_h); ar.gemm(c.W1); ar.ptr(c.b1); ar.gemm(c.W2); ar.ptr(c.b2); ar.ptr(c.gamma); }
    ar.ptr(M->fln_w); ar.ptr(M->fln_b); ar.gemm(M->head_W); ar.ptr(M->head_b);
    ar.pod(M->Kb); ar.pod(M->Kq); ar.pod(M->bins_f); ar.pod(M->R);
    ar.gemm(M->istft_W); ar.ptr(M->wsq); ar.ptr(M->win);
    ar.pod(M->has_seadec); ar.conv(M->sd_first); ar.lstm(M->sd_lstm);
    n = ar.count(M->sd_stages.size(), 8); M->sd_stages.resize(n);
    for (SeaDecStage& st : M->sd_stages) {
        ar.ptr(st.tr_w); ar.gemm(st.tr_wp); ar.ptr(st.tr_b); ar.pod(st.cin); ar.pod(st.cout); ar.pod(st.k); ar.pod(st.r);
        ar.conv(st.c3); ar.conv(st.c1); ar.conv(st.sc); ar.conv(st.cat);
    }
    ar.ptr(M->sd_last_w); ar.ptr(M->sd_last_b);
    n = ar.count(M->lazy_f32.size(), 1 << 12); M->lazy_f32.resize(n);
    for (wt_model::LazyF32& z : M->lazy_f32) { ar.ptr(z.w); ar.ptr(z.s32); ar.pod(z.n); ar.pod(z.scale); }
}

struct PackHeader {
    uint32_t magic;
    int32_t version;
    wt_arch arch;
    uint64_t arch_hash;
    uint64_t n_allocs, struct_bytes, payload_bytes;
    uint64_t body_hash;
};

static uint64_t body_hash_of(const char* p, size_t n) {
    uint64_t h[4] = {0x9e3779b97f4a7c15ull, 0xc2b2ae3d27d4eb4full, 0x165667b19e3779f9ull, 0x27d4eb2f165667c5ull};
    const uint64_t K = 0x100000001b3ull * 0x9e3779b1ull | 1ull;
    size_t i = 0;
    for (; i + 32 <= n; i += 32) {
        uint64_t w[4];
        std::memcpy(w, p + i, 32);
        for (int l = 0; l < 4; ++l) { h[l] = (h[l] ^ w[l]) * K; h[l] ^= h[l] >> 29; }
    }
    for (; i < n; ++i) { h[0] = (h[0] ^ (unsigned char)p[i]) * K; h[0] ^= h[0] >> 29; }
    h[0] = (h[0] ^ (uint64_t)n) * K;
    return (h[0] ^ (h[1] * 3) ^ (h[2] * 5) ^ (h[3] * 7)) * K;
}

static constexpr uint64_t PACK_NOT_STORED = 1ull << 63;

static std::vector<bool> lazy_allocs(const wt_model* M) {
    std::vector<bool> lazy(M->allocs.size(), false);
    for (const wt_model::LazyF32& z : M->lazy_f32)
        for (size_t i = 0; i < M->allocs.size(); ++i)
            if (M->allocs[i] == static_cast<const void*>(z.w)) lazy[i] = true;
    return lazy;
}

size_t model_export_bytes(const wt_model* M) {
    size_t total = sizeof(PackHeader) + M->allocs.size() * sizeof(uint64_t) + (1u << 17);
    const std::vector<bool> lazy = lazy_allocs(M);
    for (size_t i = 0; i < M->allocs.size(); ++i) if (!lazy[i]) total += (M->alloc_bytes[i] + 255) / 256 * 256;
    return total + 256;
}

int model_export(const wt_model* Mc, void* buf, size_t n) {
    wt_model* M = const_cast<wt_model*>(Mc);
    std::map<const void*, int> index;
    for (size_t i = 0; i < M->allocs.size(); ++i) index[M->allocs[i]] = (int)i;
    std::vector<char> st;
    Archive ar;
    ar.saving = true; ar.out = &st; ar.index = &index;
    archive_model(ar, M);
    if (!ar.ok) { set_error("wt_model_export: a model pointer lies outside the model's allocations"); return WT_ERR_INVALID; }
    PackHeader h{};
    h.magic = PACK_MAGIC; h.version = PACK_VERSION; h.arch = M->arch; h.arch_hash = arch_hash_of(M->arch);
    h.n_allocs = M->allocs.size(); h.struct_bytes = st.size();
    if (M->f32_stale.load()) if (int rc = ensure_f32_weights(M)) return rc;
    const std::vector<bool> lazy = lazy_allocs(M);
    size_t pos = sizeof(PackHeader) + M->allocs.size() * sizeof(uint64_t) + st.size();
    pos = (pos + 255) / 256 * 256;
    const size_t payload0 = pos;
    for (size_t i = 0; i < M->allocs.size(); ++i) if (!lazy[i]) pos += (M->alloc_bytes[i] + 255) / 256 * 256;
    h.payload_bytes = pos - payload0;
    if (pos > n) { set_error("wt_model_export: buffer too small (wt_model_export_bytes)"); return WT_ERR_INVALID; }
    char* o = static_cast<char*>(buf);
    std::memset(o, 0, payload0);
    for (size_t i = 0; i < M->allocs.size(); ++i) { uint64_t b = M->alloc_bytes[i] | (lazy[i] ? PACK_NOT_STORED : 0); std::memcpy(o + sizeof(h) + i * 8, &b, 8); }
    std::memcpy(o + sizeof(h) + M->allocs.size() * 8, st.data(), st.size());
    pos = payload0;
    WT_HIP_CHECK(hipDeviceSynchronize());
    for (size_t i = 0; i < M->allocs.size(); ++i) {
        if (lazy[i]) continue;
        const size_t b = M->alloc_bytes[i], padded = (b + 255) / 256 * 256;
        WT_HIP_CHECK(hipMemcpy(o + pos, M->allocs[i], b, hipMemcpyDeviceToHost));
        std::memset(o + pos + b, 0, padded - b);
        pos += padded;
    }
    h.body_hash = body_hash_of(o + sizeof(h), pos - sizeof(h));
    std::memcpy(o, &h, sizeof(h));
    return (int)0;
}

int packed_info(const void* buf, size_t n, wt_arch* arch, int32_t* version, uint64_t* arch_hash) {
    if (!buf || n < sizeof(PackHeader)) { set_error("packed image: too short"); return WT_ERR_INVALID; }
    PackHeader h;
    std::memcpy(&h, buf, sizeof(h));
    if (h.magic != PACK_MAGIC) { set_error("packed image: bad magic (not a wavtokenizer_amd packed file)"); return WT_ERR_INVALID; }
    if (version) *version = h.version;
    if (arch) *arch = h.arch;
    if (arch_hash) *arch_hash = h.arch_hash;
    if (h.version != PACK_VERSION) { set_error("packed image: layout version " + std::to_string(h.version) + ", this library reads " + std::to_string(PACK_VERSION)); return WT_ERR_INVALID; }
    if (h.arch_hash != arch_hash_of(h.arch)) { set_error("packed image: architecture hash mismatch (corrupt header)"); return WT_ERR_INVALID; }
    size_t left = n - sizeof(PackHeader);
    if (h.n_allocs > (1u << 16) || h.n_allocs * 8 > left) { set_error("packed image: truncated (allocation table)"); return WT_ERR_INVALID; }
    left -= h.n_allocs * 8;
    if (h.struct_bytes > (1u << 24) || h.struct_bytes > left) { set_error("packed image: truncated (model section)"); return WT_ERR_INVALID; }
    const size_t head = sizeof(PackHeader) + h.n_allocs * 8 + h.struct_bytes, head_pad = (head + 255) / 256 * 256;
    if (head_pad > n || h.payload_bytes > n - head_pad) { set_error("packed image: truncated (payload)"); return WT_ERR_INVALID; }
    return WT_OK;
}

size_t packed_bytes(const void* buf, size_t n) {
    if (packed_info(buf, n, nullptr, nullptr, nullptr)) return 0;
    PackHeader h;
    std::memcpy(&h, buf, sizeof(h));
    return (sizeof(PackHeader) + h.n_allocs * 8 + h.struct_bytes + 255) / 256 * 256 + h.payload_bytes;
}

int packed_verify(const void* buf, size_t n) {
    if (int rc = packed_info(buf, n, nullptr, nullptr, nullptr)) return rc;
    PackHeader h;
    std::memcpy(&h, buf, sizeof(h));
    const char* in = static_cast<const char*>(buf);
    const size_t head_pad = (sizeof(PackHeader) + h.n_allocs * 8 + h.struct_bytes + 255) / 256 * 256;
    size_t pos = head_pad;
    for (size_t i = 0; i < h.n_allocs; ++i) {
        uint64_t b;
        std::memcpy(&b, in + sizeof(h) + i * 8, 8);
        if (b & PACK_NOT_STORED) {
            if ((b & ~PACK_NOT_STORED) == 0 || (b & ~PACK_NOT_STORED) > (1ull << 32)) { set_error("packed image: bad size of an unstored array"); return WT_ERR_INVALID; }
            continue;
        }
        if (b == 0 || b > n - pos || (b + 255) / 256 * 256 > n - pos) { set_error("packed image: allocation table does not fit the payload"); return WT_ERR_INVALID; }
        pos += (b + 255) / 256 * 256;
    }
    if (pos - head_pad != h.payload_bytes) { set_error("packed image: allocation table and payload size disagree"); return WT_ERR_INVALID; }
    if (body_hash_of(in + sizeof(h), pos - sizeof(h)) != h.body_hash) { set_error("packed image: content hash mismatch (corrupt file)"); return WT_ERR_INVALID; }
    return WT_OK;
}

static int validate_imported(const wt_model* M) {
    const wt_arch& a = M->arch;
    auto fits = [&](const void* p, size_t bytes) {
        if (!p) return false;
        const char* c = static_cast<const char*>(p);
        for (size_t i = 0; i < M->allocs.size(); ++i) {
            const char* base = static_cast<const char*>(M->allocs[i]);
            if (c >= base && c < base + M->alloc_bytes[i]) return bytes <= (size_t)(base + M->alloc_bytes[i] - c);
        }
        return false;
    };
    auto bad = [](const char* what) { set_error(std::string("packed image: ") + what + " does not match the architecture in its header"); return WT_ERR_INVALID; };
    auto copy_ok = [&](const S32Copy& s, size_t bytes, bool pair_ok) {
        return (!s.p || fits(s.p, bytes)) && s.acc_scale > 0.f && std::isfinite(s.acc_scale) && (pair_ok || !s.tap_pair);
    };
    auto conv_ok = [&](const ConvW& c, int cout, int cin, int k, bool pair_ok = false) {
        const size_t bytes = (size_t)cout * cin * k * 4;
        return c.cout == cout && c.cin == cin && c.k == k && fits(c.w, bytes) && fits(c.b, (size_t)cout * 4) && copy_ok(c.s32, bytes, pair_ok);
    };
    auto gemm_ok = [&](const GemmW& g, int rows, int cols) {
        const size_t bytes = (size_t)rows * cols * 4;
        return g.rows == rows && g.cols == cols && fits(g.w, bytes) && copy_ok(g.s32, bytes, false);
    };
    auto lstm_ok = [&](const LstmW& l, int H) {
        const size_t hh = (size_t)4 * H * H * 4;
        return gemm_ok(l.Wih0, 4 * H, H) && fits(l.b0, (size_t)16 * H) && fits(l.W0, hh) && fits(l.W1, 2 * hh) && fits(l.b1, (size_t)16 * H) &&
               (!l.W0h || fits(l.W0h, hh)) && (!l.W1h || fits(l.W1h, 2 * hh)) &&
               (!l.Wp || fits(l.Wp, (size_t)3 * 32 * 4 * 16 * 2 * 64 * 16));
    };
    const int nf = 32, H = 512, D = a.dim, I = a.intermediate_dim;
    if (a.n_ratios < 1 || a.n_ratios > 8 || a.num_quantizers < 1 || a.num_quantizers > 32 || a.input_channels != 512 || D % 256 || I % 32 || a.num_layers < 1 || a.num_layers > 32 ||
        a.adanorm_num_embeddings < 1 || a.vq_bins < 1 || a.n_fft < 4 || a.hop_length < 1) return bad("the architecture itself");
    int hop = 1;
    for (int i = 0; i < a.n_ratios; ++i) { if (a.ratios[i] < 1 || a.ratios[i] > 64) return bad("a ratio"); hop *= a.ratios[i]; }
    if (M->hop != hop || M->H != H || (int)M->enc_ratios.size() != a.n_ratios || (int)M->stages.size() != a.n_ratios) return bad("the encoder's shape");
    if (M->e0_k != 7 || M->e0_c != nf || !fits(M->e0_w, 7 * nf * 4) || !fits(M->e0_b, nf * 4)) return bad("the first conv");
    int mult = 1;
    for (int i = 0; i < a.n_ratios; ++i) {
        const ResStage& st = M->stages[i];
        const int r = a.ratios[a.n_ratios - 1 - i], C = mult * nf;
        if (M->enc_ratios[i] != r || st.C != C || st.r != r || !conv_ok(st.c3, C / 2, C, 3) || !conv_ok(st.c1, C, C / 2, 1) || !conv_ok(st.sc, C, C, 1) ||
            !conv_ok(st.down, 2 * C, C, 2 * r, true)) return bad("an encoder stage");
        if ((st.cat.w || st.cat.s32.p) && !conv_ok(st.cat, C, C + C / 2, 1)) return bad("a fused shortcut weight");
        mult *= 2;
    }
    if (mult * nf != H || !lstm_ok(M->enc_lstm, H) || !conv_ok(M->enc_final, 512, H, 7)) return bad("the encoder tail");
    if (!gemm_ok(M->embed, a.vq_bins, 512) || !fits(M->embed.w, (size_t)a.num_quantizers * a.vq_bins * 512 * 4) || !fits(M->ee, (size_t)a.vq_bins * 4)) return bad("the codebook");
    if (!conv_ok(M->bb_embed, D, 512, 7)) return bad("backbone.embed");
    for (const PosRes& r : M->res)
        if (!fits(r.n1w, D * 4) || !fits(r.n1b, D * 4) || !fits(r.n2w, D * 4) || !fits(r.n2b, D * 4) || !conv_ok(r.c1, D, D, 3) || !conv_ok(r.c2, D, D, 3)) return bad("a pos_net block");
    if (!fits(M->at_nw, D * 4) || !fits(M->at_nb, D * 4) || !gemm_ok(M->at_Wqk, 2 * D, D) || !fits(M->at_bqk, 2 * D * 4) || !gemm_ok(M->at_Wv, D, D) ||
        !fits(M->at_bv, D * 4) || !gemm_ok(M->at_Wp, D, D) || !fits(M->at_bp, D * 4)) return bad("the attention block");
    const size_t ada = (size_t)a.adanorm_num_embeddings * D * 4;
    if (!fits(M->gn5w, D * 4) || !fits(M->gn5b, D * 4) || !fits(M->ada_s, ada) || !fits(M->ada_h, ada)) return bad("backbone.norm");
    if ((int)M->cnx.size() != a.num_layers) return bad("the ConvNeXt block count");
    for (const CnxBlock& c : M->cnx)
        if (!fits(c.dw_w, (size_t)7 * D * 4) || !fits(c.dw_b, D * 4) || !fits(c.ada_s, ada) || !fits(c.ada_h, ada) || !gemm_ok(c.W1, I, D) || !fits(c.b1, I * 4) ||
            !gemm_ok(c.W2, D, I) || !fits(c.b2, D * 4) || !fits(c.gamma, D * 4)) return bad("a ConvNeXt block");
    const int N = a.n_fft;
    if (N % 4 || N % a.hop_length) return bad("n_fft / hop_length");
    const int Kq = ((N / 4 + 1 + 31) / 32) * 32, Kb = 2 * Kq;
    if (M->Kq != Kq || M->Kb != Kb || M->bins_f != N / 2 + 1 || M->R != N / a.hop_length) return bad("the ISTFT head's shape");
    if (!fits(M->fln_w, D * 4) || !fits(M->fln_b, D * 4) || !gemm_ok(M->head_W, 2 * Kb, D) || !fits(M->head_b, (size_t)2 * Kb * 4) ||
        !gemm_ok(M->istft_W, 4 * Kq, Kq) || !fits(M->win, (size_t)N * 4) || !fits(M->wsq, (size_t)N * 4)) return bad("the ISTFT head");
    if (M->has_seadec) {
        if ((int)M->sd_stages.size() != a.n_ratios || !conv_ok(M->sd_first, (1 << a.n_ratios) * nf, 512, 7) || !lstm_ok(M->sd_lstm, H)) return bad("the SEANetDecoder");
        int m2 = 1 << a.n_ratios;
        for (int i = 0; i < a.n_ratios; ++i) {
            const SeaDecStage& st = M->sd_stages[i];
            const int r = a.ratios[i], cin = m2 * nf, h = cin / 2;
            if (st.cin != cin || st.cout != h || st.k != 2 * r || st.r != r || !fits(st.tr_w, (size_t)2 * r * cin * h * 4) || ((st.tr_wp.w || st.tr_wp.s32.p) && !gemm_ok(st.tr_wp, r * h, 2 * cin)) ||
                !fits(st.tr_b, h * 4) || !conv_ok(st.c3, h / 2, h, 3) || !conv_ok(st.c1, h, h / 2, 1) || !conv_ok(st.sc, h, h, 1)) return bad("a SEANetDecoder stage");
            if ((st.cat.w || st.cat.s32.p) && !conv_ok(st.cat, h, h + h / 2, 1)) return bad("a SEANetDecoder fused shortcut");
            m2 /= 2;
        }
        if (!fits(M->sd_last_w, 7 * nf * 4) || !fits(M->sd_last_b, 4)) return bad("the SEANetDecoder's last conv");
    }
    return WT_OK;
}

int model_import(wt_model* M, const void* buf, size_t n) {
    PackHeader h;
    if (int rc = packed_verify(buf, n)) return rc;
    std::memcpy(&h, buf, sizeof(h));
    M->arch = h.arch;
    const char* in = static_cast<const char*>(buf);
    size_t pos = (sizeof(PackHeader) + h.n_allocs * 8 + h.struct_bytes + 255) / 256 * 256;
    for (size_t i = 0; i < h.n_allocs; ++i) {
        uint64_t b;
        std::memcpy(&b, in + sizeof(h) + i * 8, 8);
        const bool stored = !(b & PACK_NOT_STORED);
        b &= ~PACK_NOT_STORED;
        const size_t padded = (b + 255) / 256 * 256;
        if (stored && pos + padded > n) { set_error("packed image: truncated payload"); return WT_ERR_INVALID; }
        void* d = nullptr;
        WT_HIP_CHECK(hipMalloc(&d, b));
        M->allocs.push_back(d);
        M->alloc_bytes.push_back(b);
        if (stored) {
            WT_HIP_CHECK(hipMemcpy(d, in + pos, b, hipMemcpyHostToDevice));
            pos += padded;
        } else {
            M->f32_stale.store(true);
        }
    }
    Archive ar;
    ar.saving = false; ar.in = in + sizeof(h) + h.n_allocs * 8; ar.n = h.struct_bytes; ar.allocs = &M->allocs; ar.alloc_bytes = &M->alloc_bytes;
    archive_model(ar, M);
    if (!ar.ok || ar.pos != ar.n) { set_error("packed image: model section does not match this library's layout"); return WT_ERR_INVALID; }
    for (const wt_model::LazyF32& z : M->lazy_f32) {
        size_t iw = M->allocs.size(), is = M->allocs.size();
        for (size_t i = 0; i < M->allocs.size(); ++i) {
            if (M->allocs[i] == static_cast<const void*>(z.w)) iw = i;
            if (z.s32 && M->allocs[i] == z.s32) is = i;
        }
        if (iw == M->allocs.size() || z.n <= 0 || (z.n % 32) || (size_t)z.n * 4 > M->alloc_bytes[iw] ||
            (z.s32 && (is == M->allocs.size() || (size_t)z.n * 4 > M->alloc_bytes[is])) || !(z.scale > 0.f) || !std::isfinite(z.scale)) {
            set_error("packed image: bad entry in the list of unstored fp32 arrays"); return WT_ERR_INVALID;
        }
    }
    return validate_imported(M);
}

int ensure_f32_weights(const wt_model* M) {
    std::lock_guard<std::mutex> lock(M->f32_mu);
    if (!M->f32_stale.load()) return WT_OK;
    for (const wt_model::LazyF32& z : M->lazy_f32) {
        if (!z.s32) continue;
        if (int rc = launch_unsplit_s32(z.s32, const_cast<float*>(z.w), (long)z.n, 1.f / z.scale, nullptr)) return rc;
    }
    WT_HIP_CHECK(hipDeviceSynchronize());
    M->f32_stale.store(false);
    return WT_OK;
}

}
```

Measured before the change: 38950.

## Fuse attention QKV projection and add single-kernel attention core

Concatenates the Q, K and V weights into one QKV GEMM and replaces the separate V-transpose GEMM, score GEMM, softmax and PV GEMM with a single HIP kernel. The kernel computes scores, softmax and the output per 32-query block using split-f16 MFMA products in LDS, for D=768 and L<=128. This removes several launches, a buffer fill and the intermediate round-trips to global memory. In exchange it stores extra packed QKV weights, bumps the pack version, and recomputes V staging in every query-block workgroup.

```diff
diff --git a/include/wavtokenizer_amd.h b/include/wavtokenizer_amd.h
--- a/include/wavtokenizer_amd.h
+++ b/include/wavtokenizer_amd.h
@@ -178,10 +178,12 @@
 int wt_gemm_probe(const wt_gemm_desc* d, wt_launch_form* form, void* workspace, void* stream);
 
 enum { WT_OP_GN_APPLY = 0, WT_OP_GN_STATS = 1, WT_OP_ROWNORM = 2, WT_OP_SOFTMAX = 3, WT_OP_ISTFT_OLA = 4, WT_OP_CONV_FIRST = 5,
-       WT_OP_CONV_LAST = 6, WT_OP_TRANSPOSE = 7, WT_OP_CONVTR = 8, WT_OP_ROW_SUMSQ = 9, WT_OP_S32_AMAX = 10 };
+       WT_OP_CONV_LAST = 6, WT_OP_TRANSPOSE = 7, WT_OP_CONVTR = 8, WT_OP_ROW_SUMSQ = 9, WT_OP_S32_AMAX = 10,
+       WT_OP_ATTN_CORE = 12 };
 enum { WT_OPK_GN_TILE = 1, WT_OPK_GN_CHUNK = 2, WT_OPK_GN_STATS = 3, WT_OPK_ROWNORM = 4, WT_OPK_DWCONV_LN = 5,
        WT_OPK_SOFTMAX_REG = 6, WT_OPK_SOFTMAX_RMW = 7, WT_OPK_ISTFT_OLA = 8, WT_OPK_CONV_FIRST = 9, WT_OPK_CONV_LAST32 = 10,
-       WT_OPK_CONV_LAST = 11, WT_OPK_TRANSPOSE = 12, WT_OPK_CONVTR = 13, WT_OPK_ROW_SUMSQ = 14, WT_OPK_S32_AMAX = 15 };
+       WT_OPK_CONV_LAST = 11, WT_OPK_TRANSPOSE = 12, WT_OPK_CONVTR = 13, WT_OPK_ROW_SUMSQ = 14, WT_OPK_S32_AMAX = 15,
+       WT_OPK_ATTN_CORE = 16 };
 typedef struct {
     int32_t size;
     int32_t op;
diff --git a/wavtokenizer_amd/_capi.py b/wavtokenizer_amd/_capi.py
--- a/wavtokenizer_amd/_capi.py
+++ b/wavtokenizer_amd/_capi.py
@@ -63,9 +63,10 @@
 
 WT_OP_GN_APPLY, WT_OP_GN_STATS, WT_OP_ROWNORM, WT_OP_SOFTMAX, WT_OP_ISTFT_OLA, WT_OP_CONV_FIRST = 0, 1, 2, 3, 4, 5
 WT_OP_CONV_LAST, WT_OP_TRANSPOSE, WT_OP_CONVTR, WT_OP_ROW_SUMSQ, WT_OP_S32_AMAX = 6, 7, 8, 9, 10
+WT_OP_ATTN_CORE = 12
 WT_OPK_NAMES = {1: "gn_tile", 2: "gn_chunk", 3: "gn_stats", 4: "rownorm", 5: "dwconv_ln", 6: "softmax_reg", 7: "softmax_rmw",
                 8: "istft_ola", 9: "conv_first", 10: "conv_last32", 11: "conv_last", 12: "transpose", 13: "convtr",
-                14: "row_sumsq", 15: "s32_amax"}
+                14: "row_sumsq", 15: "s32_amax", 16: "attn_core"}
 
 
 class WtOpDesc(ctypes.Structure):
diff --git a/wavtokenizer_amd/csrc/attn_core.hip b/wavtokenizer_amd/csrc/attn_core.hip
--- /dev/null
+++ b/wavtokenizer_amd/csrc/attn_core.hip
@@ -0,0 +1,282 @@
+#include "common.h"
+#include <cmath>
+
+namespace wt {
+
+typedef float f32x4 __attribute__((ext_vector_type(4)));
+typedef _Float16 f16x8 __attribute__((ext_vector_type(8)));
+
+namespace {
+
+constexpr int AC_D = 768;
+constexpr int AC_G = AC_D / 32;
+constexpr int AC_ROWB = 3 * AC_D * 4;
+constexpr int AC_QB = 32;
+constexpr int AC_LMAX = 128;
+constexpr int AC_CH = 128;
+constexpr int AC_PITCH = 528;
+constexpr int AC_QPITCH = AC_G * 128 + 16;
+constexpr int AC_VT = 0, AC_Q = 0, AC_P = AC_QB * AC_QPITCH, AC_S = AC_P + AC_QB * AC_PITCH;
+constexpr int AC_KPITCH = 144, AC_KW = AC_S + AC_QB * AC_PITCH;
+constexpr int AC_LDS = AC_KW + 4 * 32 * AC_KPITCH;
+static_assert(AC_CH * AC_PITCH <= AC_P, "the V^T chunk must fit the region it shares with the q block");
+constexpr int AC_PF = 8;
+
+__device__ __forceinline__ float ac_wave_sum(float v) {
+#pragma unroll
+    for (int off = 32; off >= 1; off >>= 1) v += __shfl_xor(v, off, 64);
+    return v;
+}
+__device__ __forceinline__ float ac_wave_max(float v) {
+#pragma unroll
+    for (int off = 32; off >= 1; off >>= 1) v = fmaxf(v, __shfl_xor(v, off, 64));
+    return v;
+}
+__device__ __forceinline__ f16x8 ld16(const char* p) { return *reinterpret_cast<const f16x8*>(p); }
+
+struct KRows { f16x8 r[4]; };
+
+}
+
+__global__ __launch_bounds__(256) void attn_core_kernel(const char* __restrict__ qkv, char* __restrict__ o, int B, int L,
+                                                        float scale, unsigned* __restrict__ status) {
+    extern __shared__ __attribute__((aligned(16))) char ac_smem[];
+    char* const Vt = ac_smem + AC_VT;
+    char* const Ql = ac_smem + AC_Q;
+    char* const Pl = ac_smem + AC_P;
+    char* const Sl = ac_smem + AC_S;
+    const int tid = threadIdx.x, lane = tid & 63;
+    const int wave = __builtin_amdgcn_readfirstlane(tid >> 6);
+    const int nqb = (L + AC_QB - 1) / AC_QB, Lp = nqb * AC_QB, nks = Lp / 32;
+    const int slot = blockIdx.x >> 3;
+    const int qb = slot % nqb, clip = (slot / nqb) * 8 + (blockIdx.x & 7);
+    if (clip >= B) return;
+    const int q0 = qb * AC_QB;
+    const char* const base = qkv + (size_t)clip * L * AC_ROWB;
+    const int li = lane & 15, kq = lane >> 4;
+
+    auto load_v = [&](int chunk, f16x8 (&vr)[2][8]) {
+#pragma unroll
+        for (int i = 0; i < 2; ++i) {
+            const int t = tid + 256 * i;
+            const int piece = t & 7, kg = (t >> 8) * 8 + ((t >> 3) & 7), grp = (t >> 6) & 3;
+            const char* p = base + (2 * AC_G + chunk * (AC_CH / 32) + grp) * 128 + piece * 16;
+#pragma unroll
+            for (int r = 0; r < 8; ++r) vr[i][r] = ld16(p + (size_t)min(kg * 8 + r, L - 1) * AC_ROWB);
+        }
+    };
+    auto store_v = [&](const f16x8 (&vr)[2][8]) {
+#pragma unroll
+        for (int i = 0; i < 2; ++i) {
+            const int t = tid + 256 * i;
+            const int piece = t & 7, kg = (t >> 8) * 8 + ((t >> 3) & 7), grp = (t >> 6) & 3;
+            if (kg * 8 >= Lp) continue;
+            char* dst = Vt + (grp * 32 + (piece & 3) * 8) * AC_PITCH + (piece >> 2) * 256 + ((kg + piece) & 15) * 16;
+            f16x8 z[8];
+#pragma unroll
+            for (int r = 0; r < 8; ++r) z[r] = kg * 8 + r < L ? vr[i][r] : (f16x8)(_Float16)0;
+#pragma unroll
+            for (int j = 0; j < 8; ++j) {
+                f16x8 tr;
+#pragma unroll
+                for (int r = 0; r < 8; ++r) tr[r] = z[r][j];
+                *reinterpret_cast<f16x8*>(dst + j * AC_PITCH) = tr;
+            }
+        }
+    };
+
+    const bool s_wave = wave * 32 < Lp;
+    char* const Kw = ac_smem + AC_KW + wave * (32 * AC_KPITCH);
+    const char* kp[4];
+#pragma unroll
+    for (int i = 0; i < 4; ++i) kp[i] = base + (size_t)min(wave * 32 + i * 8 + (lane >> 3), L - 1) * AC_ROWB + AC_G * 128 + (lane & 7) * 16;
+    auto load_k = [&](int s, KRows& f) {
+#pragma unroll
+        for (int i = 0; i < 4; ++i) f.r[i] = ld16(kp[i] + s * 128);
+    };
+    KRows f[AC_PF + 1];
+    {
+        constexpr int PIECES = AC_G * 8;
+        f16x8 qr[AC_QB * PIECES / 256];
+#pragma unroll
+        for (int i = 0; i < AC_QB * PIECES / 256; ++i) {
+            const int p = tid + 256 * i, row = p / PIECES, col = p - row * PIECES;
+            qr[i] = ld16(base + (size_t)min(q0 + row, L - 1) * AC_ROWB + col * 16);
+        }
+        if (s_wave) {
+#pragma unroll
+            for (int s = 0; s < AC_PF; ++s) load_k(s, f[s]);
+        }
+#pragma unroll
+        for (int i = 0; i < AC_QB * PIECES / 256; ++i) {
+            const int p = tid + 256 * i, row = p / PIECES, col = p - row * PIECES;
+            *reinterpret_cast<f16x8*>(Ql + row * AC_QPITCH + col * 16) = qr[i];
+        }
+    }
+    __syncthreads();
+    if (s_wave) {
+        f32x4 am[2][2], ac[2][2];
+#pragma unroll
+        for (int n = 0; n < 2; ++n)
+#pragma unroll
+            for (int m = 0; m < 2; ++m) am[n][m] = ac[n][m] = (f32x4){0.f, 0.f, 0.f, 0.f};
+#pragma unroll
+        for (int s = 0; s < AC_G; ++s) {
+            if (s + AC_PF < AC_G) load_k(s + AC_PF, f[(s + AC_PF) % (AC_PF + 1)]);
+            const KRows& c = f[s % (AC_PF + 1)];
+#pragma unroll
+            for (int i = 0; i < 4; ++i) *reinterpret_cast<f16x8*>(Kw + (i * 8 + (lane >> 3)) * AC_KPITCH + (lane & 7) * 16) = c.r[i];
+            f16x8 kh[2], kl[2], qh[2], ql[2];
+#pragma unroll
+            for (int n = 0; n < 2; ++n) {
+                const char* p = Kw + (n * 16 + li) * AC_KPITCH + kq * 16;
+                kh[n] = ld16(p); kl[n] = ld16(p + 64);
+            }
+#pragma unroll
+            for (int m = 0; m < 2; ++m) {
+                const char* p = Ql + (m * 16 + li) * AC_QPITCH + s * 128 + kq * 16;
+                qh[m] = ld16(p); ql[m] = ld16(p + 64);
+            }
+#pragma unroll
+            for (int n = 0; n < 2; ++n)
+#pragma unroll
+                for (int m = 0; m < 2; ++m) {
+                    am[n][m] = __builtin_amdgcn_mfma_f32_16x16x32_f16(kh[n], qh[m], am[n][m], 0, 0, 0);
+                    ac[n][m] = __builtin_amdgcn_mfma_f32_16x16x32_f16(kl[n], qh[m], ac[n][m], 0, 0, 0);
+                    ac[n][m] = __builtin_amdgcn_mfma_f32_16x16x32_f16(kh[n], ql[m], ac[n][m], 0, 0, 0);
+                }
+        }
+#pragma unroll
+        for (int n = 0; n < 2; ++n)
+#pragma unroll
+            for (int m = 0; m < 2; ++m) {
+                f32x4 v;
+#pragma unroll
+                for (int e = 0; e < 4; ++e) v[e] = scale * fmaf(ac[n][m][e], 1.f / 2048.f, am[n][m][e]);
+                *reinterpret_cast<f32x4*>(Sl + (m * 16 + li) * AC_PITCH + (wave * 32 + n * 16 + 4 * kq) * 4) = v;
+            }
+    }
+    f16x8 vr0[2][8], vr1[2][8];
+    load_v(0, vr0);
+    load_v(1, vr1);
+    __syncthreads();
+
+#pragma unroll 1
+    for (int i = 0; i < AC_QB / 4; ++i) {
+        const int r = wave * (AC_QB / 4) + i;
+        const int j = 4 * lane;
+        f32x4 v = j < Lp ? *reinterpret_cast<const f32x4*>(Sl + r * AC_PITCH + j * 4) : (f32x4){0.f, 0.f, 0.f, 0.f};
+        float mx = -INFINITY;
+#pragma unroll
+        for (int e = 0; e < 4; ++e) {
+            if (j + e >= L) v[e] = -INFINITY;
+            mx = fmaxf(mx, v[e]);
+        }
+        mx = ac_wave_max(mx);
+        float sum = 0.f;
+#pragma unroll
+        for (int e = 0; e < 4; ++e) {
+            const float ex = j + e < L ? expf(v[e] - mx) : 0.f;
+            v[e] = ex;
+            sum += ex;
+        }
+        sum = ac_wave_sum(sum);
+        if (j < Lp) {
+            f32x4 p;
+#pragma unroll
+            for (int e = 0; e < 4; ++e) p[e] = j + e < L ? v[e] / sum : 0.f;
+            wt_f16x4 hi, lo;
+            split4_f16(p[0], p[1], p[2], p[3], hi, lo);
+            char* dst = Pl + r * AC_PITCH + (j >> 5) * 128 + (j & 31) * 2;
+            *reinterpret_cast<wt_f16x4*>(dst) = hi;
+            *reinterpret_cast<wt_f16x4*>(dst + 64) = lo;
+        }
+    }
+    __syncthreads();
+
+    f16x8 ph[4][2], pl[4][2];
+#pragma unroll
+    for (int s = 0; s < AC_LMAX / 32; ++s)
+#pragma unroll
+        for (int m = 0; m < 2; ++m) {
+            const char* p = Pl + (m * 16 + li) * AC_PITCH + (s < nks ? s : 0) * 128 + kq * 16;
+            ph[s][m] = ld16(p);
+            pl[s][m] = ld16(p + 64);
+        }
+    float amax = 0.f;
+    auto do_chunk = [&](int chunk, f16x8 (&vr)[2][8]) {
+        store_v(vr);
+        __syncthreads();
+        if (chunk + 2 < AC_D / AC_CH) load_v(chunk + 2, vr);
+        f32x4 am[2][2], ac[2][2];
+#pragma unroll
+        for (int n = 0; n < 2; ++n)
+#pragma unroll
+            for (int m = 0; m < 2; ++m) am[n][m] = ac[n][m] = (f32x4){0.f, 0.f, 0.f, 0.f};
+#pragma unroll
+        for (int s = 0; s < AC_LMAX / 32; ++s) {
+            if (s >= nks) break;
+#pragma unroll
+            for (int n = 0; n < 2; ++n) {
+                const char* p = Vt + (wave * 32 + n * 16 + li) * AC_PITCH;
+                const int cq = (2 * n + (li >> 3)) & 3;
+                const f16x8 vh = ld16(p + ((4 * s + kq + cq) & 15) * 16), vl = ld16(p + 256 + ((4 * s + kq + cq + 4) & 15) * 16);
+#pragma unroll
+                for (int m = 0; m < 2; ++m) {
+                    am[n][m] = __builtin_amdgcn_mfma_f32_16x16x32_f16(vh, ph[s][m], am[n][m], 0, 0, 0);
+                    ac[n][m] = __builtin_amdgcn_mfma_f32_16x16x32_f16(vl, ph[s][m], ac[n][m], 0, 0, 0);
+                    ac[n][m] = __builtin_amdgcn_mfma_f32_16x16x32_f16(vh, pl[s][m], ac[n][m], 0, 0, 0);
+                }
+            }
+        }
+#pragma unroll
+        for (int m = 0; m < 2; ++m) {
+            const int qrow = q0 + m * 16 + li;
+            if (qrow >= L) continue;
+            char* orow = o + ((size_t)clip * L + qrow) * (AC_D * 4);
+#pragma unroll
+            for (int n = 0; n < 2; ++n) {
+                const int ch = chunk * AC_CH + wave * 32 + n * 16 + 4 * kq;
+                f32x4 v;
+#pragma unroll
+                for (int e = 0; e < 4; ++e) v[e] = fmaf(ac[n][m][e], 1.f / 2048.f, am[n][m][e]);
+                amax = amax4(amax, v[0], v[1], v[2], v[3]);
+                wt_f16x4 hi, lo;
+                split4_f16(v[0], v[1], v[2], v[3], hi, lo);
+                char* dst = orow + (ch >> 5) * 128 + (ch & 31) * 2;
+                *reinterpret_cast<wt_f16x4*>(dst) = hi;
+                *reinterpret_cast<wt_f16x4*>(dst + 64) = lo;
+            }
+        }
+        __syncthreads();
+    };
+#pragma unroll 1
+    for (int chunk = 0; chunk < AC_D / AC_CH; chunk += 2) {
+        do_chunk(chunk, vr0);
+        do_chunk(chunk + 1, vr1);
+    }
+    range_report(status, amax);
+}
+
+bool attn_core_supported(int L, int D) { return D == AC_D && L >= 1 && L <= AC_LMAX; }
+
+int launch_attn_core(const float* qkv, float* o, int B, int L, int D, hipStream_t s) {
+    if (!attn_core_supported(L, D) || B < 1) { set_error("attn_core: needs D = 768, 1 <= L <= 128 and B >= 1"); return -1; }
+    if ((reinterpret_cast<uintptr_t>(qkv) | reinterpret_cast<uintptr_t>(o)) & 15) { set_error("attn_core: buffers must be 16-byte aligned"); return -1; }
+    if ((long)B * ((L + AC_QB - 1) / AC_QB) > (1L << 24)) { set_error("attn_core: too many clips for one launch"); return -1; }
+    static PerDeviceOnce attr_once;
+    if (int rc = attr_once.run([] {
+            WT_HIP_CHECK(hipFuncSetAttribute(reinterpret_cast<const void*>(attn_core_kernel), hipFuncAttributeMaxDynamicSharedMemorySize, AC_LDS));
+            return 0;
+        })) return rc;
+    const int nqb = (L + AC_QB - 1) / AC_QB;
+    const dim3 grid((unsigned)(nqb * ((B + 7) / 8 * 8))), block(256);
+    if (OpForm* f = g_launch.form) *f = OpForm{OPK_ATTN_CORE, nqb, 0, {grid.x, 1, 1}, 256, (unsigned)AC_LDS};
+    const float scale = (float)std::pow((double)D, -0.5);
+    hipLaunchKernelGGL(attn_core_kernel, grid, block, AC_LDS, s, reinterpret_cast<const char*>(qkv), reinterpret_cast<char*>(o), B, L, scale,
+                       g_launch.status);
+    WT_HIP_CHECK(hipGetLastError());
+    return 0;
+}
+
+}
diff --git a/wavtokenizer_amd/csrc/common.h b/wavtokenizer_amd/csrc/common.h
--- a/wavtokenizer_amd/csrc/common.h
+++ b/wavtokenizer_amd/csrc/common.h
@@ -37,7 +37,7 @@
 enum : unsigned { WT_STATUS_LSTM = 1u, WT_STATUS_RANGE = 2u };
 enum OpKernel : int {
     OPK_NONE = 0, OPK_GN_TILE, OPK_GN_CHUNK, OPK_GN_STATS, OPK_ROWNORM, OPK_DWCONV_LN, OPK_SOFTMAX_REG, OPK_SOFTMAX_RMW,
-    OPK_ISTFT_OLA, OPK_CONV_FIRST, OPK_CONV_LAST32, OPK_CONV_LAST, OPK_TRANSPOSE, OPK_CONVTR, OPK_ROW_SUMSQ, OPK_S32_AMAX
+    OPK_ISTFT_OLA, OPK_CONV_FIRST, OPK_CONV_LAST32, OPK_CONV_LAST, OPK_TRANSPOSE, OPK_CONVTR, OPK_ROW_SUMSQ, OPK_S32_AMAX, OPK_ATTN_CORE
 };
 struct OpForm {
     int kernel = OPK_NONE;
@@ -236,6 +236,8 @@
 int launch_istft_ola(const float* parts, const float* win, const float* wsq, float* out, int B, int L, int n_fft, int hop,
                      int Kq, int center, hipStream_t s);
 int launch_softmax(float* S, int rows, int L, int ld, hipStream_t s, float* P_s32 = nullptr);
+bool attn_core_supported(int L, int D);
+int launch_attn_core(const float* qkv, float* o, int B, int L, int D, hipStream_t s);
 int launch_row_sumsq(const float* x, float* out, long rows, int D, hipStream_t s);
 int launch_vq_finalize(const float* pval, const int* pidx, int nparts, const float* embed, int64_t* codes,
                        float* feat_ncl, int B, int L, int D, int bins, hipStream_t s);
diff --git a/wavtokenizer_amd/csrc/model.h b/wavtokenizer_amd/csrc/model.h
--- a/wavtokenizer_amd/csrc/model.h
+++ b/wavtokenizer_amd/csrc/model.h
@@ -84,8 +84,9 @@
     float* ee = nullptr;
     wt::ConvW bb_embed;
     wt::PosRes res[4];
-    float *at_nw, *at_nb, *at_bqk, *at_bv, *at_bp;
+    float *at_nw, *at_nb, *at_bqk, *at_bv, *at_bp, *at_bqkv;
     wt::GemmW at_Wqk, at_Wv, at_Wp;
+    wt::GemmW at_Wqkv;
     float *gn5w, *gn5b, *ada_s, *ada_h;
     std::vector<wt::CnxBlock> cnx;
     float *fln_w, *fln_b;
diff --git a/wavtokenizer_amd/csrc/plan.cpp b/wavtokenizer_amd/csrc/plan.cpp
--- a/wavtokenizer_amd/csrc/plan.cpp
+++ b/wavtokenizer_amd/csrc/plan.cpp
@@ -421,39 +421,55 @@
         const bool s32 = s32_at(SITE_ATTN) && M->at_Wqk.s32.p && M->at_Wv.s32.p && M->at_Wp.s32.p;
         const int fmt = s32 ? BUF_S32 : BUF_F32;
         P->bufs[h1].fmt = fmt;
-        const int qk = P->buf("bb.attn.qk", (size_t)Mrows * 2 * D, fmt);
-        const int vt = P->buf("bb.attn.vt", (size_t)B * D * Lp, fmt);
-        const int S = P->buf("bb.attn.s", (size_t)Mrows * Lp);
-        const int Ps = s32 ? P->buf("bb.attn.p", (size_t)Mrows * Lp, BUF_S32) : S;
-        const int o = P->buf("bb.attn.o", (size_t)Mrows * D, fmt);
-        P->step({x, sc, sh, gp, h1}, [=](const RunCtx& c) {
-            return launch_gn_apply(P->ptr(c, x), M->at_nw, M->at_nb, P->ptr(c, sc), P->ptr(c, sh), P->ptr(c, h1), 0, B, L, D, 32, 1e-6f, c.stream, s32, P->ptr(c, gp));
-        }, 1, "attn.gn");
-        gemm_step(P, s32, linear_args(M->at_Wqk, M->at_bqk, Mrows, 2 * D, D), {h1, -1, qk}, PRO_NONE, EPI_BIAS, OUT_S32, "attn.qk");
-        P->step({h1, vt}, [=](const RunCtx& c) {
-            if (int rc = launch_fill_u32(P->ptr(c, vt), 0u, (size_t)B * D * Lp * sizeof(float), c.stream)) return rc;
-            GemmArgs a = linear_args(nullptr, M->at_bv, D, L, D);
-            a.A = s32 ? static_cast<const float*>(M->at_Wv.s32.p) : M->at_Wv.w; a.acc_scale = M->at_Wv.s32.acc_scale; a.zA = 0;
-            a.zW = (long)L * D; a.nz = B;
-            a.C = P->ptr(c, vt); a.c_rstride = Lp; a.zC = (long)D * Lp;
-            return dense_act(P, s32, a, P->ptr(c, h1), EPI_BIAS_ROW, OUT_S32, c.stream);
-        }, 2, "attn.vt");
-        P->step({qk, S}, [=](const RunCtx& c) {
-            GemmArgs a = linear_args(nullptr, nullptr, L, L, D);
-            a.A = P->ptr(c, qk); a.a_rstride = 2 * D; a.zA = (long)L * 2 * D;
-            a.w_rstride = 2 * D; a.zW = (long)L * 2 * D; a.nz = B;
-            a.C = P->ptr(c, S); a.c_rstride = Lp; a.zC = (long)L * Lp;
-            a.alpha = (float)std::pow((double)D, -0.5);
-            return dense_act(P, s32, a, P->ptr(c, qk) + D, EPI_SCALE, OUT_F32, c.stream);
-        }, 1, "attn.s");
-        P->step({S, Ps}, [=](const RunCtx& c) { return launch_softmax(P->ptr(c, S), (int)Mrows, L, Lp, c.stream, s32 ? P->ptr(c, Ps) : nullptr); });
-        P->step({Ps, vt, o}, [=](const RunCtx& c) {
-            GemmArgs a = linear_args(nullptr, nullptr, L, D, Lp);
-            a.A = P->ptr(c, Ps); a.zA = (long)L * Lp;
-            a.zW = (long)D * Lp; a.nz = B;
-            a.C = P->ptr(c, o); a.c_rstride = D; a.zC = (long)L * D;
-            return dense_act(P, s32, a, P->ptr(c, vt), EPI_BIAS, OUT_S32, c.stream);
-        }, 1, "attn.o");
+        const bool core_env = [] { const char* e = lab_env("WT_ATTN_CORE"); return !e || e[0] != '0'; }();
+        const bool core = s32 && core_env && M->at_Wqkv.s32.p && attn_core_supported(L, D);
+        int o = -1;
+        auto gn_step = [&] {
+            P->step({x, sc, sh, gp, h1}, [=](const RunCtx& c) {
+                return launch_gn_apply(P->ptr(c, x), M->at_nw, M->at_nb, P->ptr(c, sc), P->ptr(c, sh), P->ptr(c, h1), 0, B, L, D, 32, 1e-6f, c.stream, s32, P->ptr(c, gp));
+            }, 1, "attn.gn");
+        };
+        if (core) {
+            const int qkv = P->buf("bb.attn.qkv", (size_t)Mrows * 3 * D, BUF_S32);
+            o = P->buf("bb.attn.o", (size_t)Mrows * D, BUF_S32);
+            gn_step();
+            gemm_step(P, true, linear_args(M->at_Wqkv, M->at_bqkv, Mrows, 3 * D, D), {h1, -1, qkv}, PRO_NONE, EPI_BIAS, OUT_S32, "attn.qkv");
+            P->step({qkv, o}, [=](const RunCtx& c) {
+                return launch_attn_core(P->ptr(c, qkv), P->ptr(c, o), B, L, D, c.stream);
+            }, 1, "attn.core");
+        } else {
+            const int qk = P->buf("bb.attn.qk", (size_t)Mrows * 2 * D, fmt);
+            const int vt = P->buf("bb.attn.vt", (size_t)B * D * Lp, fmt);
+            const int S = P->buf("bb.attn.s", (size_t)Mrows * Lp);
+            const int Ps = s32 ? P->buf("bb.attn.p", (size_t)Mrows * Lp, BUF_S32) : S;
+            o = P->buf("bb.attn.o", (size_t)Mrows * D, fmt);
+            gn_step();
+            gemm_step(P, s32, linear_args(M->at_Wqk, M->at_bqk, Mrows, 2 * D, D), {h1, -1, qk}, PRO_NONE, EPI_BIAS, OUT_S32, "attn.qk");
+            P->step({h1, vt}, [=](const RunCtx& c) {
+                if (int rc = launch_fill_u32(P->ptr(c, vt), 0u, (size_t)B * D * Lp * sizeof(float), c.stream)) return rc;
+                GemmArgs a = linear_args(nullptr, M->at_bv, D, L, D);
+                a.A = s32 ? static_cast<const float*>(M->at_Wv.s32.p) : M->at_Wv.w; a.acc_scale = M->at_Wv.s32.acc_scale; a.zA = 0;
+                a.zW = (long)L * D; a.nz = B;
+                a.C = P->ptr(c, vt); a.c_rstride = Lp; a.zC = (long)D * Lp;
+                return dense_act(P, s32, a, P->ptr(c, h1), EPI_BIAS_ROW, OUT_S32, c.stream);
+            }, 2, "attn.vt");
+            P->step({qk, S}, [=](const RunCtx& c) {
+                GemmArgs a = linear_args(nullptr, nullptr, L, L, D);
+                a.A = P->ptr(c, qk); a.a_rstride = 2 * D; a.zA = (long)L * 2 * D;
+                a.w_rstride = 2 * D; a.zW = (long)L * 2 * D; a.nz = B;
+                a.C = P->ptr(c, S); a.c_rstride = Lp; a.zC = (long)L * Lp;
+                a.alpha = (float)std::pow((double)D, -0.5);
+                return dense_act(P, s32, a, P->ptr(c, qk) + D, EPI_SCALE, OUT_F32, c.stream);
+            }, 1, "attn.s");
+            P->step({S, Ps}, [=](const RunCtx& c) { return launch_softmax(P->ptr(c, S), (int)Mrows, L, Lp, c.stream, s32 ? P->ptr(c, Ps) : nullptr); });
+            P->step({Ps, vt, o}, [=](const RunCtx& c) {
+                GemmArgs a = linear_args(nullptr, nullptr, L, D, Lp);
+                a.A = P->ptr(c, Ps); a.zA = (long)L * Lp;
+                a.zW = (long)D * Lp; a.nz = B;
+                a.C = P->ptr(c, o); a.c_rstride = D; a.zC = (long)L * D;
+                return dense_act(P, s32, a, P->ptr(c, vt), EPI_BIAS, OUT_S32, c.stream);
+            }, 1, "attn.o");
+        }
         GemmArgs ap = linear_args(M->at_Wp, M->at_bp, Mrows, D, D);
         ap.r_rstride = D;
         gemm_step(P, s32, ap, in_place(o, x), PRO_NONE, EPI_BIAS_RES, OUT_F32, "attn.proj");
diff --git a/wavtokenizer_amd/csrc/probe.cpp b/wavtokenizer_amd/csrc/probe.cpp
--- a/wavtokenizer_amd/csrc/probe.cpp
+++ b/wavtokenizer_amd/csrc/probe.cpp
@@ -165,7 +165,7 @@
 static int op_probe_check(const wt_op_desc* d) {
     auto bad = [](const char* m) { set_error(std::string("wt_op_probe: ") + m); return (int)WT_ERR_INVALID; };
     if (!d || d->size != (int32_t)sizeof(wt_op_desc)) return bad("descriptor missing or of another size");
-    if (d->op < WT_OP_GN_APPLY || d->op > WT_OP_S32_AMAX) return bad("unknown op");
+    if (d->op < WT_OP_GN_APPLY || d->op > WT_OP_ATTN_CORE || d->op == WT_OP_S32_AMAX + 1) return bad("unknown op");
     auto al16 = [](const void* p) { return !(reinterpret_cast<uintptr_t>(p) & 15); };
     const void* ptrs[] = {d->p0, d->p1, d->p2, d->p3, d->p4, d->p5, d->y, d->y2, d->y3};
     for (const void* p : ptrs) if (!al16(p)) return bad("arrays must be 16-byte aligned");
@@ -217,6 +217,10 @@
         if (!d->y) return bad("null argument");
         if (d->n <= 0 || d->n % 32) return bad("s32_amax needs whole S32 groups of 32 values");
         break;
+    case WT_OP_ATTN_CORE:
+        if (!d->y) return bad("null argument");
+        if (!attn_core_supported(d->L, d->C)) return bad("attn_core needs C = 768 and L <= 128");
+        break;
     }
     return WT_OK;
 }
@@ -266,6 +270,9 @@
         break;
     case WT_OP_S32_AMAX:
         rc = launch_s32_amax(d->x, d->n, static_cast<unsigned*>(d->y), s);
+        break;
+    case WT_OP_ATTN_CORE:
+        rc = launch_attn_core(F(d->x), W(d->y), d->B, d->L, d->C, s);
         break;
     }
     g_launch = saved;
diff --git a/wavtokenizer_amd/csrc/weights.cpp b/wavtokenizer_amd/csrc/weights.cpp
--- a/wavtokenizer_amd/csrc/weights.cpp
+++ b/wavtokenizer_amd/csrc/weights.cpp
@@ -261,6 +261,16 @@
         if (int rc = upload(M, bqk, &M->at_bqk)) return rc;
         if (int rc = load_gemm(M, tm, p + ".v.weight", D, D, &M->at_Wv)) return rc;
         if (int rc = load_vec(M, tm, p + ".v.bias", D, &M->at_bv)) return rc;
+        const float* wv = tm.get(p + ".v.weight", (int64_t)D * D);
+        const float* bv = tm.get(p + ".v.bias", D);
+        if (!wv || !bv) return WT_ERR_MISSING_TENSOR;
+        std::vector<float> wqkv((size_t)3 * D * D), bqkv(3 * D);
+        std::memcpy(&wqkv[0], wqk.data(), (size_t)2 * D * D * sizeof(float));
+        std::memcpy(&wqkv[(size_t)2 * D * D], wv, (size_t)D * D * sizeof(float));
+        std::memcpy(&bqkv[0], bqk.data(), 2 * D * sizeof(float));
+        std::memcpy(&bqkv[2 * D], bv, D * sizeof(float));
+        if (int rc = upload_gemm(M, wqkv, 3 * D, D, &M->at_Wqkv)) return rc;
+        if (int rc = upload(M, bqkv, &M->at_bqkv)) return rc;
         if (int rc = load_gemm(M, tm, p + ".proj_out.weight", D, D, &M->at_Wp)) return rc;
         if (int rc = load_vec(M, tm, p + ".proj_out.bias", D, &M->at_bp)) return rc;
     }
@@ -481,6 +491,7 @@
     if (int rc = gemm32(M->istft_W)) return rc;
     if (int rc = gemm32(M->at_Wqk)) return rc;
     if (int rc = gemm32(M->at_Wv)) return rc;
+    if (int rc = gemm32(M->at_Wqkv)) return rc;
     if (int rc = gemm32(M->at_Wp)) return rc;
     if (M->has_seadec) {
         if (int rc = conv32sd(M->sd_first)) return rc;
@@ -500,7 +511,7 @@
 
 
 static constexpr uint32_t PACK_MAGIC = 0x4b505457u;
-static constexpr int32_t PACK_VERSION = 7;
+static constexpr int32_t PACK_VERSION = 8;
 
 static uint64_t arch_hash_of(const wt_arch& a) {
     uint64_t h = 1469598103934665603ull;
@@ -563,6 +574,7 @@
     ar.conv(M->bb_embed);
     for (PosRes& r : M->res) { ar.ptr(r.n1w); ar.ptr(r.n1b); ar.ptr(r.n2w); ar.ptr(r.n2b); ar.conv(r.c1); ar.conv(r.c2); }
     ar.ptr(M->at_nw); ar.ptr(M->at_nb); ar.gemm(M->at_Wqk); ar.ptr(M->at_bqk); ar.gemm(M->at_Wv); ar.ptr(M->at_bv); ar.gemm(M->at_Wp); ar.ptr(M->at_bp);
+    ar.gemm(M->at_Wqkv); ar.ptr(M->at_bqkv);
     ar.ptr(M->gn5w); ar.ptr(M->gn5b); ar.ptr(M->ada_s); ar.ptr(M->ada_h);
     n = ar.count(M->cnx.size(), 64); M->cnx.resize(n);
     for (CnxBlock& c : M->cnx) { ar.ptr(c.dw_w); ar.ptr(c.dw_b); ar.ptr(c.ada_s); ar.ptr(c.ada_h); ar.gemm(c.W1); ar.ptr(c.b1); ar.gemm(c.W2); ar.ptr(c.b2); ar.ptr(c.gamma); }
@@ -757,7 +769,8 @@
     for (const PosRes& r : M->res)
         if (!fits(r.n1w, D * 4) || !fits(r.n1b, D * 4) || !fits(r.n2w, D * 4) || !fits(r.n2b, D * 4) || !conv_ok(r.c1, D, D, 3) || !conv_ok(r.c2, D, D, 3)) return bad("a pos_net block");
     if (!fits(M->at_nw, D * 4) || !fits(M->at_nb, D * 4) || !gemm_ok(M->at_Wqk, 2 * D, D) || !fits(M->at_bqk, 2 * D * 4) || !gemm_ok(M->at_Wv, D, D) ||
-        !fits(M->at_bv, D * 4) || !gemm_ok(M->at_Wp, D, D) || !fits(M->at_bp, D * 4)) return bad("the attention block");
+        !fits(M->at_bv, D * 4) || !gemm_ok(M->at_Wp, D, D) || !fits(M->at_bp, D * 4) || !gemm_ok(M->at_Wqkv, 3 * D, D) ||
+        !fits(M->at_bqkv, 3 * D * 4)) return bad("the attention block");
     const size_t ada = (size_t)a.adanorm_num_embeddings * D * 4;
     if (!fits(M->gn5w, D * 4) || !fits(M->gn5b, D * 4) || !fits(M->ada_s, ada) || !fits(M->ada_h, ada)) return bad("backbone.norm");
     if ((int)M->cnx.size() != a.num_layers) return bad("the ConvNeXt block count");
```

Result: no change. 39050 (median of 6 runs) (+0.3%).
